# manhofer/Line3Dpp

Measured on AMD Instinct MI355X. Metric: M segment-pair scores/sec, higher is better.
Workload: dtype f64

## Files before the change

### include/l3dpp_hip.h

```cpp
#ifndef L3DPP_HIP_H_
#define L3DPP_HIP_H_

#include <stdint.h>

#ifdef __cplusplus
extern "C" {
#endif


typedef struct l3d_match {
    uint32_t src_camID_, src_segID_, tgt_camID_, tgt_segID_;
    float overlap_score_, score3D_;
    float depth_p1_, depth_p2_, depth_q1_, depth_q2_;
} l3d_match;

typedef struct l3d_segment2d { uint32_t camID_, segID_; } l3d_segment2d;

typedef struct l3d_segment3d {
    double P1[3], P2[3], dir[3];
    float length_;
    uint32_t valid_;
} l3d_segment3d;

typedef struct l3d_cledge { int32_t i_, j_; float w_; } l3d_cledge;

typedef struct l3d_float4 { float x, y, z, w; } l3d_float4;

typedef struct l3d_slot {
    uint32_t tgt_seg;
    float overlap;
    float depth_p1, depth_p2, depth_q1, depth_q2;
    float score3D;
    uint32_t flags;
} l3d_slot;

typedef enum l3d_status {
    L3D_OK = 0,
    L3D_ERR_ARG = -1,
    L3D_ERR_IMAGE_SMALL = -2,
    L3D_ERR_ID_IN_USE = -3,
    L3D_ERR_NO_NEIGHBORS = -4,
    L3D_ERR_NO_SEGMENTS = -5,
    L3D_ERR_NO_VIEWS = -6,
    L3D_ERR_STATE = -7,
    L3D_ERR_HIP = -8,
    L3D_ERR_LIMIT = -9,
    L3D_ERR_RETRY = -10,
    L3D_ERR_IO = -11
} l3d_status;

typedef struct l3d_ctx l3d_ctx;

typedef struct l3d_match_params {
    float sigma_position;
    float sigma_angle;
    uint32_t num_neighbors;
    float epipolar_overlap;
    int32_t kNN;
    float const_regularization_depth;
} l3d_match_params;

const char* l3d_last_error(void);
const char* l3d_build_info(void);
uint64_t l3d_trim_cache(void);


l3d_ctx* l3d_create(int device, void* stream);
void l3d_destroy(l3d_ctx*);

int l3d_add_view(l3d_ctx*, uint32_t camID, const float* segs4, uint32_t M, const double K[9],
                 const double R[9], const double t[3], uint32_t width, uint32_t height,
                 float median_depth, const uint32_t* neighbors, uint32_t n_neighbors);

int l3d_add_view_worldpoints(l3d_ctx*, uint32_t camID, const float* segs4, uint32_t M, const double K[9],
                             const double R[9], const double t[3], uint32_t width, uint32_t height,
                             float median_depth, const uint32_t* worldpoints, uint32_t n_worldpoints);
int l3d_get_visual_neighbors(l3d_ctx*, uint32_t camID, uint32_t* out, uint32_t cap, uint32_t* n);
int l3d_neighbors_from_worldpoints(uint32_t n_views, const uint32_t* cam_ids, const double* K9, const double* R9,
                                   const double* t3, const uint64_t* wp_offsets, const uint32_t* worldpoints,
                                   uint32_t num_neighbors, uint64_t* nb_offsets, uint32_t* neighbors, uint64_t cap);

typedef struct l3d_nvm l3d_nvm;
typedef struct l3d_nvm_camera {
    const char* filename;
    float focal, distortion;
    float median_depth;
    uint32_t n_worldpoints;
    double R[9], t[3], C[3];
} l3d_nvm_camera;
int l3d_nvm_open(const char* path, l3d_nvm** out);
uint32_t l3d_nvm_num_cameras(const l3d_nvm*);
int l3d_nvm_get_camera(const l3d_nvm*, uint32_t index, l3d_nvm_camera* out);
int l3d_nvm_get_worldpoints(const l3d_nvm*, uint32_t index, uint32_t* out, uint32_t cap);
void l3d_nvm_close(l3d_nvm*);
void l3d_nvm_intrinsics(float focal, uint32_t width, uint32_t height, double K[9]);
typedef struct l3d_sfm l3d_sfm;
typedef struct l3d_sfm_image {
    uint32_t id, camera;
    uint32_t width, height;
    const char* name;
    float focal;
    float median_depth;
    uint32_t n_worldpoints;
    double K[9];
    double R[9], t[3], C[3];
    double radial[3], tangential[2];
} l3d_sfm_image;
int l3d_sfm_open_colmap(const char* folder, l3d_sfm** out);
int l3d_sfm_open_bundler(const char* bundle_file, l3d_sfm** out);
uint32_t l3d_sfm_num_images(const l3d_sfm*);
int l3d_sfm_get_image(const l3d_sfm*, uint32_t index, l3d_sfm_image* out);
int l3d_sfm_get_worldpoints(const l3d_sfm*, uint32_t index, uint32_t* out, uint32_t cap);
void l3d_sfm_close(l3d_sfm*);
struct l3d_camera_model;
int l3d_sfm_get_camera_model(const l3d_sfm*, uint32_t index, struct l3d_camera_model* out);
const char* l3d_sfm_get_camera_params(const l3d_sfm*, uint32_t index, double* params, uint32_t cap, uint32_t* n);
int l3d_segment_cache_name(uint32_t camID, uint32_t width, uint32_t height, uint32_t max_segments, char* out, uint32_t cap);
int l3d_read_segment_cache(const char* path, float* segs4 , uint32_t cap, uint32_t* n);
int l3d_write_segment_cache(const char* path, const float* segs4, uint32_t n);

typedef struct l3d_image {
    const uint8_t* data;
    uint32_t cols, rows, channels, row_stride;
} l3d_image;
typedef struct l3d_detect_options {
    const char* output_folder;
    int32_t load_segments;
    int32_t max_image_width;
    uint32_t max_line_segments;
} l3d_detect_options;
typedef struct l3d_detect_stats {
    uint32_t width, height;
    uint32_t raw_segments;
    uint32_t segments;
    uint32_t from_cache;
    uint32_t seeds;
    uint32_t nfa_evals;
    uint32_t reserved;
    double max_grad;
} l3d_detect_stats;
int l3d_detect_segments(l3d_ctx*, uint32_t n_images, const l3d_image* images, int max_image_width,
                        uint32_t max_segments, uint32_t* counts);
int l3d_detect_view_segments(l3d_ctx*, uint32_t n_images, const uint32_t* camIDs, const l3d_image* images,
                             const l3d_detect_options* opts, uint32_t* counts);
int l3d_get_detected_segments(l3d_ctx*, float* segs4 , uint64_t cap, uint64_t* n);
int l3d_get_detect_stats(l3d_ctx*, l3d_detect_stats* out, uint32_t cap, uint32_t* n);
int l3d_add_view_image(l3d_ctx*, uint32_t camID, const l3d_image* image, const l3d_detect_options* opts,
                       const double K[9], const double R[9], const double t[3], float median_depth,
                       const uint32_t* neighbors, uint32_t n_neighbors, uint32_t* n_segments);
int l3d_add_view_image_worldpoints(l3d_ctx*, uint32_t camID, const l3d_image* image, const l3d_detect_options* opts,
                                   const double K[9], const double R[9], const double t[3], float median_depth,
                                   const uint32_t* worldpoints, uint32_t n_worldpoints, uint32_t* n_segments);

typedef struct l3d_distortion { double K[9]; double radial[3]; double tangential[2]; } l3d_distortion;
int l3d_undistort_images(l3d_ctx*, uint32_t n_images, const l3d_image* in, const l3d_distortion* dist,
                         uint8_t* const* out);
enum { L3D_CAM_NONE = 0, L3D_CAM_FULL_OPENCV = 1, L3D_CAM_OPENCV_FISHEYE = 2, L3D_CAM_SIMPLE_RADIAL_FISHEYE = 3,
       L3D_CAM_RADIAL_FISHEYE = 4, L3D_CAM_FOV = 5 };
typedef struct l3d_camera_model {
    uint32_t model;
    uint32_t reserved;
    double K[9];
    double params[8];
    double K_new[9];
} l3d_camera_model;
int l3d_undistort_images_model(l3d_ctx*, uint32_t n_images, const l3d_image* in, const l3d_camera_model* cams,
                               uint8_t* const* out);

int l3d_match_images(l3d_ctx*, const l3d_match_params*);

int l3d_match_begin(l3d_ctx*, const l3d_match_params*);
int l3d_num_pairs(l3d_ctx*, uint32_t* n);
int l3d_get_pairs(l3d_ctx*, uint32_t* src_cam, uint32_t* tgt_cam, uint64_t* slot_offset );
int l3d_match_pairs(l3d_ctx*, uint32_t first, uint32_t count);
int l3d_slot_buffer(l3d_ctx*, void** dev_ptr, uint64_t* n_slots);
int l3d_get_fresh_hyp(l3d_ctx*, float* out, uint64_t n);
int l3d_slots_exchanged(l3d_ctx*);
int l3d_slot_index_buffer(l3d_ctx*, void** dev_ptr, uint64_t* n_slots);
int l3d_pack_slot_indices(l3d_ctx*, uint32_t first, uint32_t count);
int l3d_expand_slot_indices(l3d_ctx*, uint32_t first, uint32_t count);
int l3d_match_finish(l3d_ctx*);
int l3d_lists_shard(l3d_ctx*, uint32_t rank, uint32_t world, void* slab_ptr[4], uint64_t slab_bytes[4], void* full_ptr[4]);
int l3d_lists_shard_views(l3d_ctx*, uint32_t rank, uint32_t world, uint32_t view0, uint32_t view1, void* slab_ptr[4],
                          uint64_t slab_bytes[4], void* full_ptr[4]);
int l3d_tail_shard_count(l3d_ctx*, uint32_t counts[2]);
int l3d_shard_options(l3d_ctx*, uint32_t first_needed_rank, int exchanges_stream_ordered);
int l3d_tail_shard_layout(l3d_ctx*, uint32_t world, const uint32_t* counts_all, const uint32_t* view_bounds, void* base_ptr[9],
                          uint64_t elt_bytes[9], uint64_t* first, uint64_t* count);
int l3d_tail_shard_commit(l3d_ctx*);
int l3d_affinity_shard_begin(l3d_ctx*, uint32_t rank, uint32_t world, void** simv, uint64_t* first, uint64_t* count);
int l3d_affinity_shard_finish(l3d_ctx*);
int l3d_affinity_shard_abort(l3d_ctx*);
int l3d_plan_shards(uint32_t n_views, uint32_t n_pairs, const uint32_t* pair_src_view, const uint64_t* pair_cost,
                    uint32_t world, uint32_t* view_bounds, uint32_t* pair_bounds);
int l3d_match_abort(l3d_ctx*);

int l3d_compute_affinity(l3d_ctx*);

int l3d_reconstruct_3d_lines(l3d_ctx*, uint32_t visibility_t, int perform_diffusion, float collinearity_t,
                             int use_CERES, uint32_t max_iter_CERES);
int l3d_num_3d_lines(l3d_ctx*, uint32_t* n_lines, uint32_t* n_segments, uint32_t* n_residuals);
typedef struct l3d_line_opt_summary {
    uint32_t lines_bundled;
    uint32_t lines_constant;
    uint32_t lines_dropped;
    uint32_t stop_gradient, stop_function, stop_parameter, stop_max_iter;
    uint32_t stop_other;
    uint32_t max_iterations;
    uint32_t residuals;
    uint32_t lines_wide;
    uint32_t max_residuals;
    double cost_before, cost_after;
    float kernel_ms;
    uint32_t reserved;
} l3d_line_opt_summary;
int l3d_line_opt_stats(l3d_ctx*, l3d_line_opt_summary* out);
int l3d_get_3d_lines(l3d_ctx*, uint32_t* seg_offsets, l3d_segment3d* segments, uint32_t* res_offsets,
                     l3d_segment2d* residuals, l3d_segment3d* cluster_lines, uint32_t* reference_views);

int l3d_synchronize(l3d_ctx*);


int l3d_pair_tests(l3d_ctx*, uint64_t* n);
int l3d_get_matches(l3d_ctx*, uint32_t camID, l3d_match* out, uint64_t cap, uint32_t* seg_offsets,
                    uint64_t* n);
int l3d_get_pair_slots(l3d_ctx*, uint32_t pair_index, l3d_slot* out, uint64_t cap, uint32_t* Ms,
                       uint32_t* K);
int l3d_num_best(l3d_ctx*, uint32_t* n);
int l3d_get_best(l3d_ctx*, l3d_segment2d* seg2d, l3d_segment3d* seg3d, l3d_match* best);
int l3d_view_info(l3d_ctx*, uint32_t camID, float* k, float* median_depth);
int l3d_translation(l3d_ctx*, double t[3]);
int l3d_num_affinity(l3d_ctx*, uint32_t* n_edges, uint32_t* n_rows);
int l3d_get_affinity(l3d_ctx*, l3d_cledge* edges, l3d_segment2d* local2global, float* med_scene_depth_lines);
int l3d_get_sparse_matrix(l3d_ctx*, int sort_by_row, l3d_float4* entries, int32_t* start_indices);

int l3d_principal_direction(const double S9[9], double dir3[3]);
int l3d_line_to_cayley(const double P1[3], const double P2[3], double x[4]);
int l3d_cayley_to_segment(const double x[4], const double P1_old[3], const double P2_old[3], double P1[3], double P2[3]);
int l3d_line_opt_eval(int device, uint32_t n, const double x[4], const double* obs, const double* cams, double* cost,
                      double* residuals, double* jacobians, int32_t* ok);

int l3d_triangulate_points(int device, uint32_t n_cameras, const double* P12, uint64_t n_points, const uint64_t* obs_offsets,
                           const uint32_t* obs_camera, const double* obs_xy, double* X3, uint8_t* valid);
int l3d_rotation_from_rpy(double roll, double pitch, double yaw, double R9[9]);
int l3d_rotation_from_q(double qw, double qx, double qy, double qz, double R9[9]);
int l3d_decompose_projection_matrix(const double P12[12], double K9[9], double R9[9], double t3[3]);

int l3d_selftest_arith(int device, uint64_t n, uint64_t seed, uint64_t counts[3]);

int l3d_selftest_scan(int device, uint32_t element_bytes, const void* in, uint32_t n_in, uint32_t n_calls, const uint32_t* n,
                      int in_place, int pass_total, void* out, void* totals, uint64_t* ws_nonzero, uint64_t* guard_changed);

int l3d_set_brute_force(l3d_ctx*, int on);

typedef struct l3d_timings {
    float begin_ms;
    float match_pairs_ms;
    float finish_ms;
    float affinity_ms;
    uint32_t match_kernel_launches;
    float match_kernel_ms;
    float cull_prepare_ms;
    uint32_t culled_pairs;
    uint32_t list_entries;
    uint32_t support_words;
    uint32_t tied_rows;
    uint32_t chain_sweeps;
    uint32_t chain_extra_rounds;
    uint32_t pool_retries;
    float lists_ms;
    uint32_t record_kbytes;
    uint32_t list_inverse;
    uint32_t list_candidates;
    uint32_t list_headers;
    uint32_t slots_lo, slots_hi;
} l3d_timings;
int l3d_get_timings(l3d_ctx*, l3d_timings*);
int l3d_set_timing_level(l3d_ctx*, int level);
unsigned long long l3d_debug_counter(const char* name);


int l3d_match_lines(int device, const float* lines_src4, uint32_t Ms, const float* lines_tgt4, uint32_t Mt,
                    const double F[9], const double RtKinv_src[9], const double RtKinv_tgt[9],
                    const double C_src[3], const double C_tgt[3], uint32_t width, uint32_t height,
                    float epi_overlap, int32_t kNN, l3d_slot* out_slots, uint64_t* num_matches);

int l3d_output_filename(l3d_ctx*, int max_image_width, char* buf, uint32_t cap);
int l3d_save_3d_lines_txt(l3d_ctx*, const char* output_folder, int max_image_width);
int l3d_save_3d_lines_bin(l3d_ctx*, const char* output_folder, int max_image_width);
int l3d_get_segment_coords2d(l3d_ctx*, uint32_t camID, uint32_t segID, float coords[4]);
int l3d_save_result_stl(l3d_ctx*, const char* output_folder, int max_image_width);
int l3d_save_result_obj(l3d_ctx*, const char* output_folder, int max_image_width);

int l3d_score_matches(int device, const float* lines4, uint32_t M, const float* matches4, const int32_t* ranges2,
                      const float* reg_tgt2, uint32_t n, const double RtKinv[9], const double C[3], float two_sigA_sqr,
                      float k, float* scores);

int l3d_find_collinear_segments(int device, const float* lines4, uint32_t M, float dist_t, uint32_t* offsets,
                                uint32_t* idx, uint64_t cap, uint64_t* n);

int l3d_diffuse_affinity(int device, const l3d_cledge* edges, uint32_t n_edges, uint32_t n_rows, uint32_t iterations,
                         l3d_cledge* out);

typedef struct l3d_camera {
    double K[9], R[9], t[3];
    uint32_t width, height;
} l3d_camera;
typedef struct l3d_projected_segment {
    float x1, y1, x2, y2;
    float inv_depth1, inv_depth2;
    uint32_t line;
    uint32_t segment;
} l3d_projected_segment;
#define L3D_PROJ_CLIPPED_NEAR 0x80000000u
#define L3D_PROJ_CLIPPED_RECT 0x40000000u
#define L3D_PROJ_SEGMENT_MASK 0x3FFFFFFFu
int l3d_project_segments(int device, uint32_t n_cams, const l3d_camera* cams, uint32_t n_segments,
                         const l3d_segment3d* segments, const uint32_t* line_of_segment, double near_plane,
                         uint32_t* counts, l3d_projected_segment* out, uint64_t cap, uint64_t* n);
int l3d_render_line_maps(int device, uint32_t n_cams, const l3d_camera* cams, const uint32_t* n_records_per_cam,
                         const l3d_projected_segment* records, uint32_t thickness, int32_t* const* line_id_planes,
                         float* const* inv_depth_planes);
int l3d_draw_line_maps(int device, uint32_t n_cams, const l3d_image* images, const int32_t* const* line_id_planes,
                       uint32_t n_lines, const uint8_t* colors, uint32_t alpha, uint8_t* const* out_rgb);
int l3d_view_camera(l3d_ctx*, uint32_t camID, l3d_camera* cam);
int l3d_project_lines(l3d_ctx*, uint32_t n_cams, const l3d_camera* cams, double near_plane, uint32_t* counts);
int l3d_get_projected_lines(l3d_ctx*, l3d_projected_segment* out, uint64_t cap, uint64_t* n);
int l3d_render_lines(l3d_ctx*, uint32_t n_cams, const l3d_camera* cams, double near_plane, uint32_t thickness,
                     int32_t* const* line_id_planes, float* const* inv_depth_planes);
int l3d_draw_lines(l3d_ctx*, uint32_t n_cams, const l3d_camera* cams, const l3d_image* images, double near_plane,
                   uint32_t thickness, uint32_t alpha, const uint8_t* colors, uint8_t* const* out_rgb);
int l3d_set_projection_budget(l3d_ctx*, uint64_t bytes);

#ifdef __cplusplus
}
#endif
#endif
```

### line3dpp_amd/_lib.py

```python
import ctypes as C
import os

import numpy as np

_HERE = os.path.dirname(os.path.abspath(__file__))
SO_PATH = os.path.join(_HERE, "csrc", "libl3dpp_hip.so")
SO_PATH = os.environ.get("L3D_LIB", SO_PATH)

MATCH_DTYPE = np.dtype([
    ("src_cam", "<u4"), ("src_seg", "<u4"), ("tgt_cam", "<u4"), ("tgt_seg", "<u4"),
    ("overlap", "<f4"), ("score3D", "<f4"),
    ("d_p1", "<f4"), ("d_p2", "<f4"), ("d_q1", "<f4"), ("d_q2", "<f4")])
SEGMENT2D_DTYPE = np.dtype([("cam", "<u4"), ("seg", "<u4")])
SEGMENT3D_DTYPE = np.dtype([("P1", "<f8", 3), ("P2", "<f8", 3), ("dir", "<f8", 3), ("length", "<f4"), ("valid", "<u4")])
CLEDGE_DTYPE = np.dtype([("i", "<i4"), ("j", "<i4"), ("w", "<f4")])
SLOT_DTYPE = np.dtype([
    ("tgt_seg", "<u4"), ("overlap", "<f4"), ("d_p1", "<f4"), ("d_p2", "<f4"), ("d_q1", "<f4"), ("d_q2", "<f4"),
    ("score3D", "<f4"), ("flags", "<u4")])
FLOAT4_DTYPE = np.dtype([("x", "<f4"), ("y", "<f4"), ("z", "<f4"), ("w", "<f4")])
PROJECTED_SEGMENT_DTYPE = np.dtype([("x1", "<f4"), ("y1", "<f4"), ("x2", "<f4"), ("y2", "<f4"), ("inv_depth1", "<f4"),
                                    ("inv_depth2", "<f4"), ("line", "<u4"), ("segment", "<u4")])
PROJ_CLIPPED_NEAR, PROJ_CLIPPED_RECT, PROJ_SEGMENT_MASK = 0x80000000, 0x40000000, 0x3FFFFFFF
assert MATCH_DTYPE.itemsize == 40 and SLOT_DTYPE.itemsize == 32 and SEGMENT3D_DTYPE.itemsize == 80
assert PROJECTED_SEGMENT_DTYPE.itemsize == 32
EMPTY = 0xFFFFFFFF
L3D_ERR_NO_SEGMENTS = -5
L3D_ERR_IO = -11


class MatchParams(C.Structure):
    _fields_ = [("sigma_position", C.c_float), ("sigma_angle", C.c_float), ("num_neighbors", C.c_uint32),
                ("epipolar_overlap", C.c_float), ("kNN", C.c_int32), ("const_regularization_depth", C.c_float)]


class NvmCamera(C.Structure):
    _fields_ = [("filename", C.c_char_p), ("focal", C.c_float), ("distortion", C.c_float), ("median_depth", C.c_float),
                ("n_worldpoints", C.c_uint32), ("R", C.c_double * 9), ("t", C.c_double * 3), ("C", C.c_double * 3)]


class SfmImage(C.Structure):
    _fields_ = [("id", C.c_uint32), ("camera", C.c_uint32), ("width", C.c_uint32), ("height", C.c_uint32),
                ("name", C.c_char_p), ("focal", C.c_float), ("median_depth", C.c_float), ("n_worldpoints", C.c_uint32),
                ("K", C.c_double * 9), ("R", C.c_double * 9), ("t", C.c_double * 3), ("C", C.c_double * 3),
                ("radial", C.c_double * 3), ("tangential", C.c_double * 2)]


class Timings(C.Structure):
    _fields_ = [("begin_ms", C.c_float), ("match_pairs_ms", C.c_float), ("finish_ms", C.c_float),
                ("affinity_ms", C.c_float), ("match_kernel_launches", C.c_uint32), ("match_kernel_ms", C.c_float),
                ("cull_prepare_ms", C.c_float), ("culled_pairs", C.c_uint32),
                ("list_entries", C.c_uint32), ("support_words", C.c_uint32), ("tied_rows", C.c_uint32), ("chain_sweeps", C.c_uint32),
                ("chain_extra_rounds", C.c_uint32), ("pool_retries", C.c_uint32),
                ("lists_ms", C.c_float), ("record_kbytes", C.c_uint32),
                ("list_inverse", C.c_uint32), ("list_candidates", C.c_uint32), ("list_headers", C.c_uint32),
                ("slots_lo", C.c_uint32), ("slots_hi", C.c_uint32)]


class LineOptStats(C.Structure):
    _fields_ = [("lines_bundled", C.c_uint32), ("lines_constant", C.c_uint32), ("lines_dropped", C.c_uint32),
                ("stop_gradient", C.c_uint32), ("stop_function", C.c_uint32), ("stop_parameter", C.c_uint32),
                ("stop_max_iter", C.c_uint32), ("stop_other", C.c_uint32), ("max_iterations", C.c_uint32),
                ("residuals", C.c_uint32), ("lines_wide", C.c_uint32), ("max_residuals", C.c_uint32),
                ("cost_before", C.c_double), ("cost_after", C.c_double), ("kernel_ms", C.c_float), ("reserved", C.c_uint32)]


class Image(C.Structure):
    _fields_ = [("data", C.c_void_p), ("cols", C.c_uint32), ("rows", C.c_uint32), ("channels", C.c_uint32),
                ("row_stride", C.c_uint32)]


class DetectOptions(C.Structure):
    _fields_ = [("output_folder", C.c_char_p), ("load_segments", C.c_int32), ("max_image_width", C.c_int32),
                ("max_line_segments", C.c_uint32)]


class Distortion(C.Structure):
    _fields_ = [("K", C.c_double * 9), ("radial", C.c_double * 3), ("tangential", C.c_double * 2)]


CAMERA_MODELS = {"FULL_OPENCV": 1, "OPENCV_FISHEYE": 2, "SIMPLE_RADIAL_FISHEYE": 3, "RADIAL_FISHEYE": 4, "FOV": 5}
CAMERA_MODEL_PARAMS = {"FULL_OPENCV": 8, "OPENCV_FISHEYE": 4, "SIMPLE_RADIAL_FISHEYE": 1, "RADIAL_FISHEYE": 2, "FOV": 1}


class CameraModel(C.Structure):
    _fields_ = [("model", C.c_uint32), ("reserved", C.c_uint32), ("K", C.c_double * 9), ("params", C.c_double * 8),
                ("K_new", C.c_double * 9)]


class Camera(C.Structure):
    _fields_ = [("K", C.c_double * 9), ("R", C.c_double * 9), ("t", C.c_double * 3), ("width", C.c_uint32),
                ("height", C.c_uint32)]


class ProjectedSegment(C.Structure):
    _fields_ = [("x1", C.c_float), ("y1", C.c_float), ("x2", C.c_float), ("y2", C.c_float), ("inv_depth1", C.c_float),
                ("inv_depth2", C.c_float), ("line", C.c_uint32), ("segment", C.c_uint32)]


class DetectStats(C.Structure):
    _fields_ = [("width", C.c_uint32), ("height", C.c_uint32), ("raw_segments", C.c_uint32), ("segments", C.c_uint32),
                ("from_cache", C.c_uint32), ("seeds", C.c_uint32), ("nfa_evals", C.c_uint32), ("reserved", C.c_uint32),
                ("max_grad", C.c_double)]


EXPORTS = [
    "l3d_last_error", "l3d_build_info", "l3d_create", "l3d_destroy", "l3d_add_view", "l3d_match_images",
    "l3d_match_begin", "l3d_num_pairs", "l3d_get_pairs", "l3d_match_pairs", "l3d_slot_buffer", "l3d_match_finish",
    "l3d_compute_affinity", "l3d_synchronize", "l3d_pair_tests", "l3d_get_matches", "l3d_get_pair_slots",
    "l3d_num_best", "l3d_get_best", "l3d_view_info", "l3d_translation", "l3d_num_affinity", "l3d_get_affinity",
    "l3d_get_sparse_matrix", "l3d_get_timings", "l3d_match_lines", "l3d_set_brute_force", "l3d_slots_exchanged",
    "l3d_reconstruct_3d_lines", "l3d_num_3d_lines", "l3d_get_3d_lines", "l3d_diffuse_affinity",
    "l3d_output_filename", "l3d_save_3d_lines_txt", "l3d_save_result_stl", "l3d_save_result_obj",
    "l3d_get_segment_coords2d", "l3d_find_collinear_segments", "l3d_score_matches",
    "l3d_slot_index_buffer", "l3d_pack_slot_indices", "l3d_expand_slot_indices", "l3d_match_abort", "l3d_save_3d_lines_bin", "l3d_lists_shard",
    "l3d_principal_direction", "l3d_selftest_arith", "l3d_lists_shard_views", "l3d_plan_shards",
    "l3d_add_view_worldpoints", "l3d_get_visual_neighbors", "l3d_neighbors_from_worldpoints",
    "l3d_nvm_open", "l3d_nvm_num_cameras", "l3d_nvm_get_camera", "l3d_nvm_get_worldpoints", "l3d_nvm_close",
    "l3d_nvm_intrinsics", "l3d_segment_cache_name", "l3d_read_segment_cache", "l3d_write_segment_cache",
    "l3d_trim_cache", "l3d_set_timing_level", "l3d_tail_shard_count", "l3d_tail_shard_layout", "l3d_tail_shard_commit",
    "l3d_sfm_open_colmap", "l3d_sfm_open_bundler", "l3d_sfm_num_images", "l3d_sfm_get_image", "l3d_sfm_get_worldpoints",
    "l3d_sfm_close", "l3d_debug_counter", "l3d_affinity_shard_begin", "l3d_affinity_shard_finish", "l3d_affinity_shard_abort", "l3d_shard_options",
    "l3d_line_opt_stats", "l3d_line_to_cayley", "l3d_cayley_to_segment", "l3d_line_opt_eval", "l3d_get_fresh_hyp",
    "l3d_detect_segments", "l3d_detect_view_segments", "l3d_get_detected_segments", "l3d_get_detect_stats",
    "l3d_add_view_image", "l3d_add_view_image_worldpoints", "l3d_undistort_images",
    "l3d_undistort_images_model", "l3d_sfm_get_camera_model", "l3d_sfm_get_camera_params",
    "l3d_triangulate_points", "l3d_rotation_from_rpy", "l3d_rotation_from_q", "l3d_decompose_projection_matrix",
    "l3d_project_segments", "l3d_render_line_maps", "l3d_draw_line_maps", "l3d_view_camera", "l3d_project_lines",
    "l3d_get_projected_lines", "l3d_render_lines", "l3d_draw_lines", "l3d_set_projection_budget", "l3d_selftest_scan",
]

_lib = None


def load():
    global _lib
    if _lib is not None:
        return _lib
    if not os.path.exists(SO_PATH):
        raise RuntimeError(
            f"{SO_PATH} is missing: the HIP extension has not been built (run `make -C line3dpp_amd/csrc` or "
            "`python -c 'import __graft_entry__ as g; g.build()'`). There is no CPU fallback.")
    L = C.CDLL(SO_PATH)
    vp, u32, u64, i32, f32 = C.c_void_p, C.c_uint32, C.c_uint64, C.c_int, C.c_float
    L.l3d_last_error.restype = C.c_char_p
    L.l3d_build_info.restype = C.c_char_p
    L.l3d_trim_cache.argtypes = []; L.l3d_trim_cache.restype = u64
    L.l3d_create.argtypes = [i32, vp]; L.l3d_create.restype = vp
    L.l3d_destroy.argtypes = [vp]; L.l3d_destroy.restype = None
    L.l3d_add_view.argtypes = [vp, u32, vp, u32, vp, vp, vp, u32, u32, f32, vp, u32]
    L.l3d_add_view_worldpoints.argtypes = [vp, u32, vp, u32, vp, vp, vp, u32, u32, f32, vp, u32]
    L.l3d_get_visual_neighbors.argtypes = [vp, u32, vp, u32, vp]
    L.l3d_neighbors_from_worldpoints.argtypes = [u32, vp, vp, vp, vp, vp, vp, u32, vp, vp, u64]
    L.l3d_sfm_open_colmap.argtypes = [C.c_char_p, vp]; L.l3d_sfm_open_bundler.argtypes = [C.c_char_p, vp]
    L.l3d_sfm_num_images.argtypes = [vp]; L.l3d_sfm_num_images.restype = u32
    L.l3d_sfm_get_image.argtypes = [vp, u32, vp]; L.l3d_sfm_get_worldpoints.argtypes = [vp, u32, vp, u32]
    L.l3d_sfm_close.argtypes = [vp]; L.l3d_sfm_close.restype = None
    L.l3d_nvm_open.argtypes = [C.c_char_p, vp]
    L.l3d_nvm_num_cameras.argtypes = [vp]; L.l3d_nvm_num_cameras.restype = u32
    L.l3d_nvm_get_camera.argtypes = [vp, u32, vp]
    L.l3d_nvm_get_worldpoints.argtypes = [vp, u32, vp, u32]
    L.l3d_nvm_close.argtypes = [vp]; L.l3d_nvm_close.restype = None
    L.l3d_nvm_intrinsics.argtypes = [f32, u32, u32, vp]; L.l3d_nvm_intrinsics.restype = None
    L.l3d_segment_cache_name.argtypes = [u32, u32, u32, u32, C.c_char_p, u32]
    L.l3d_read_segment_cache.argtypes = [C.c_char_p, vp, u32, vp]
    L.l3d_write_segment_cache.argtypes = [C.c_char_p, vp, u32]
    L.l3d_match_images.argtypes = [vp, C.POINTER(MatchParams)]
    L.l3d_match_begin.argtypes = [vp, C.POINTER(MatchParams)]
    L.l3d_num_pairs.argtypes = [vp, C.POINTER(u32)]
    L.l3d_get_pairs.argtypes = [vp, vp, vp, vp]
    L.l3d_match_pairs.argtypes = [vp, u32, u32]
    L.l3d_slot_buffer.argtypes = [vp, C.POINTER(vp), C.POINTER(u64)]
    L.l3d_get_fresh_hyp.argtypes = [vp, vp, u64]
    L.l3d_match_finish.argtypes = [vp]
    L.l3d_match_abort.argtypes = [vp]
    L.l3d_lists_shard.argtypes = [vp, u32, u32, vp, vp, vp]
    L.l3d_lists_shard_views.argtypes = [vp, u32, u32, u32, u32, vp, vp, vp]
    L.l3d_plan_shards.argtypes = [u32, u32, vp, vp, u32, vp, vp]
    L.l3d_compute_affinity.argtypes = [vp]
    L.l3d_synchronize.argtypes = [vp]
    L.l3d_pair_tests.argtypes = [vp, C.POINTER(u64)]
    L.l3d_get_matches.argtypes = [vp, u32, vp, u64, vp, C.POINTER(u64)]
    L.l3d_get_pair_slots.argtypes = [vp, u32, vp, u64, C.POINTER(u32), C.POINTER(u32)]
    L.l3d_num_best.argtypes = [vp, C.POINTER(u32)]
    L.l3d_get_best.argtypes = [vp, vp, vp, vp]
    L.l3d_view_info.argtypes = [vp, u32, C.POINTER(f32), C.POINTER(f32)]
    L.l3d_translation.argtypes = [vp, vp]
    L.l3d_num_affinity.argtypes = [vp, C.POINTER(u32), C.POINTER(u32)]
    L.l3d_get_affinity.argtypes = [vp, vp, vp, C.POINTER(f32)]
    L.l3d_get_sparse_matrix.argtypes = [vp, i32, vp, vp]
    L.l3d_get_timings.argtypes = [vp, C.POINTER(Timings)]
    L.l3d_set_timing_level.argtypes = [vp, C.c_int]
    L.l3d_debug_counter.argtypes = [C.c_char_p]
    L.l3d_debug_counter.restype = C.c_ulonglong
    L.l3d_tail_shard_count.argtypes = [vp, vp]
    L.l3d_tail_shard_layout.argtypes = [vp, u32, vp, vp, vp, vp, vp, vp]
    L.l3d_tail_shard_commit.argtypes = [vp]
    L.l3d_affinity_shard_begin.argtypes = [vp, u32, u32, vp, vp, vp]
    L.l3d_affinity_shard_finish.argtypes = [vp]
    L.l3d_affinity_shard_abort.argtypes = [vp]
    L.l3d_shard_options.argtypes = [vp, C.c_uint32, C.c_int]
    L.l3d_match_lines.argtypes = [i32, vp, u32, vp, u32, vp, vp, vp, vp, vp, u32, u32, f32, C.c_int32, vp,
                                  C.POINTER(u64)]
    L.l3d_set_brute_force.argtypes = [vp, i32]
    L.l3d_slots_exchanged.argtypes = [vp]
    L.l3d_slot_index_buffer.argtypes = [vp, C.POINTER(vp), C.POINTER(u64)]
    L.l3d_pack_slot_indices.argtypes = [vp, u32, u32]
    L.l3d_expand_slot_indices.argtypes = [vp, u32, u32]
    L.l3d_reconstruct_3d_lines.argtypes = [vp, u32, i32, f32, i32, u32]
    L.l3d_num_3d_lines.argtypes = [vp, C.POINTER(u32), C.POINTER(u32), C.POINTER(u32)]
    L.l3d_get_3d_lines.argtypes = [vp, vp, vp, vp, vp, vp, vp]
    L.l3d_diffuse_affinity.argtypes = [i32, vp, u32, u32, u32, vp]
    L.l3d_output_filename.argtypes = [vp, i32, C.c_char_p, u32]
    L.l3d_save_3d_lines_txt.argtypes = [vp, C.c_char_p, i32]
    L.l3d_save_result_stl.argtypes = [vp, C.c_char_p, i32]
    L.l3d_save_3d_lines_bin.argtypes = [vp, C.c_char_p, i32]
    L.l3d_save_result_obj.argtypes = [vp, C.c_char_p, i32]
    L.l3d_get_segment_coords2d.argtypes = [vp, u32, u32, vp]
    L.l3d_find_collinear_segments.argtypes = [i32, vp, u32, f32, vp, vp, u64, vp]
    L.l3d_principal_direction.argtypes = [vp, vp]
    L.l3d_line_opt_stats.argtypes = [vp, C.POINTER(LineOptStats)]
    L.l3d_line_to_cayley.argtypes = [vp, vp, vp]
    L.l3d_cayley_to_segment.argtypes = [vp, vp, vp, vp, vp]
    L.l3d_line_opt_eval.argtypes = [i32, u32, vp, vp, vp, vp, vp, vp, vp]
    L.l3d_selftest_arith.argtypes = [i32, u64, u64, vp]
    L.l3d_selftest_scan.argtypes = [i32, u32, vp, u32, u32, vp, i32, i32, vp, vp, C.POINTER(u64), C.POINTER(u64)]
    L.l3d_detect_segments.argtypes = [vp, u32, vp, i32, u32, vp]
    L.l3d_detect_view_segments.argtypes = [vp, u32, vp, vp, C.POINTER(DetectOptions), vp]
    L.l3d_get_detected_segments.argtypes = [vp, vp, u64, C.POINTER(u64)]
    L.l3d_get_detect_stats.argtypes = [vp, vp, u32, C.POINTER(u32)]
    L.l3d_add_view_image.argtypes = [vp, u32, C.POINTER(Image), C.POINTER(DetectOptions), vp, vp, vp, f32, vp, u32,
                                     C.POINTER(u32)]
    L.l3d_add_view_image_worldpoints.argtypes = [vp, u32, C.POINTER(Image), C.POINTER(DetectOptions), vp, vp, vp, f32,
                                                 vp, u32, C.POINTER(u32)]
    L.l3d_undistort_images.argtypes = [vp, u32, vp, vp, vp]
    L.l3d_undistort_images_model.argtypes = [vp, u32, vp, vp, vp]
    L.l3d_sfm_get_camera_model.argtypes = [vp, u32, vp]
    L.l3d_sfm_get_camera_params.argtypes = [vp, u32, vp, u32, vp]; L.l3d_sfm_get_camera_params.restype = C.c_char_p
    L.l3d_score_matches.argtypes = [i32, vp, u32, vp, vp, vp, u32, vp, vp, f32, f32, vp]
    L.l3d_triangulate_points.argtypes = [i32, u32, vp, u64, vp, vp, vp, vp, vp]
    f64 = C.c_double
    L.l3d_rotation_from_rpy.argtypes = [f64, f64, f64, vp]
    L.l3d_rotation_from_q.argtypes = [f64, f64, f64, f64, vp]
    L.l3d_decompose_projection_matrix.argtypes = [vp, vp, vp, vp]
    L.l3d_project_segments.argtypes = [i32, u32, vp, u32, vp, vp, f64, vp, vp, u64, C.POINTER(u64)]
    L.l3d_render_line_maps.argtypes = [i32, u32, vp, vp, vp, u32, vp, vp]
    L.l3d_draw_line_maps.argtypes = [i32, u32, vp, vp, u32, vp, u32, vp]
    L.l3d_view_camera.argtypes = [vp, u32, C.POINTER(Camera)]
    L.l3d_project_lines.argtypes = [vp, u32, vp, f64, vp]
    L.l3d_get_projected_lines.argtypes = [vp, vp, u64, C.POINTER(u64)]
    L.l3d_render_lines.argtypes = [vp, u32, vp, f64, u32, vp, vp]
    L.l3d_draw_lines.argtypes = [vp, u32, vp, vp, f64, u32, u32, vp, vp]
    L.l3d_set_projection_budget.argtypes = [vp, u64]
    for name in EXPORTS:
        fn = getattr(L, name)
        if fn.restype is C.c_int and name not in ("l3d_last_error", "l3d_build_info", "l3d_create", "l3d_destroy"):
            fn.restype = C.c_int
    _lib = L
    return L


def last_error():
    return load().l3d_last_error().decode()


def ptr(a):
    return a.ctypes.data_as(C.c_void_p) if a is not None else None
```

### line3dpp_amd/csrc/k_lists.hip

```cpp
#include <algorithm>
#include <cstdlib>
#include <type_traits>

#include "l3d_dev.h"
#include "l3d_kernels.h"
#include "l3d_lists.h"

constexpr uint32_t kLists4Grid = 512;

namespace l3d {

namespace {

#define L3D_LDS __attribute__((address_space(3)))

__device__ __forceinline__ uint32_t lane_id() { return threadIdx.x & 63u; }

template <int WPL>
__device__ __forceinline__ void group_barrier() {
    if (WPL == 1) {
        __builtin_amdgcn_fence(__ATOMIC_RELEASE, "wavefront");
        __builtin_amdgcn_wave_barrier();
        __builtin_amdgcn_fence(__ATOMIC_ACQUIRE, "wavefront");
    } else {
// ... 448 lines not shown
    const PairCsr pcs = pair_csr[pi];
    if (pcs.base == kEmpty) return;
    const PairDesc& pd = pairs[pi];
    if (pd.tgt < tgt_v0 || pd.tgt >= tgt_v1) return;
    const uint32_t Mt = pd.Mt, tid = threadIdx.x;
    if ((Mt <= lds_segs) != LDSCNT) return;
    const uint32_t S = row_start ? row_start[pd.row_off + pd.Ms] - row_start[pd.row_off] : pd.Ms * pd.K;
    if (!S) {
        for (uint32_t t = threadIdx.x; t <= pd.Mt; t += kCsrBlock) poff[pcs.base + pcs.q + (size_t)t * pcs.ni] = 0;
        return;
    }
    typedef typename std::conditional<TGT16, uint16_t, uint32_t>::type tgt_t;
    const tgt_t* __restrict__ it = (const tgt_t*)inv_tgt + pd.slot_off;
    uint32_t* __restrict__ offq = poff + pcs.base + pcs.q;
    const uint32_t ni = pcs.ni;
    L3D_LDS uint32_t* lcur = (L3D_LDS uint32_t*)smem;
    uint32_t* gdum = dummy + (size_t)blockIdx.x * 64;
    auto gcur = [&](uint32_t t) -> uint32_t* { return t < Mt ? offq + (size_t)(t + 1) * ni : gdum + (t - Mt); };
    auto cur_get = [&](uint32_t t) -> uint32_t { return LDSCNT ? lcur[t] : *gcur(t); };
    auto cur_set = [&](uint32_t t, uint32_t v) { if (LDSCNT) lcur[t] = v; else *gcur(t) = v; };
    for (uint32_t t = tid; t < Mt + 64; t += kCsrBlock) cur_set(t, 0u);
    __threadfence_block();
    __syncthreads();
    const uint32_t dum = Mt + (tid & 63u);
    for (uint32_t i0 = 0; i0 < S; i0 += kCsrChunk * kCsrBlock) {
        uint32_t tv[kCsrChunk];
#pragma unroll
        for (uint32_t k = 0; k < kCsrChunk; ++k) { const uint32_t i = i0 + k * kCsrBlock + tid; tv[k] = it[min(i, S - 1)]; tv[k] = (i < S && tv[k] < Mt) ? tv[k] : dum; }
#pragma unroll
        for (uint32_t k = 0; k < kCsrChunk; ++k) {
            if (LDSCNT) (void)__hip_atomic_fetch_add(&lcur[tv[k]], 1u, __ATOMIC_RELAXED, __HIP_MEMORY_SCOPE_WORKGROUP);
            else atomicAdd(gcur(tv[k]), 1u);
        }
    }
    __threadfence_block();
    __syncthreads();
    const uint32_t per = (Mt + kCsrBlock - 1) / kCsrBlock;
    const uint32_t t0 = min(tid * per, Mt), t1 = min(t0 + per, Mt);
    uint32_t sum = 0;
    for (uint32_t t = t0; t < t1; ++t) sum += cur_get(t);
    part[tid] = sum;
    __syncthreads();
    for (uint32_t d = 1; d < kCsrBlock; d <<= 1) {
        const uint32_t v = tid >= d ? part[tid - d] : 0u;
        __syncthreads();
        part[tid] += v;
        __syncthreads();
    }
    uint32_t run = part[tid] - sum;
    for (uint32_t t = t0; t < t1; ++t) { const uint32_t c = cur_get(t); cur_set(t, run); run += c; }
    if (tid == 0) offq[0] = 0;
    __threadfence_block();
    __syncthreads();
    uint32_t* __restrict__ out = refs + pd.slot_off;
    if (STAGED) {
        L3D_LDS uint32_t* stage = lcur + (lds_segs_round(Mt) + 64);
        const uint32_t total = part[kCsrBlock - 1];
        const uint32_t window = stage_cap - min(stage_cap / 8, 1024u);
        uint32_t t_lo = 0, base = 0;
        while (base < total) {
            uint32_t lo = t_lo + 1, hi = Mt;
            while (lo < hi) { const uint32_t mid = (lo + hi) >> 1; if (lcur[mid] < base + window) lo = mid + 1; else hi = mid; }
            const uint32_t t_hi = lo, end = t_hi < Mt ? lcur[t_hi] : total;
            __syncthreads();
            for (uint32_t i0 = 0; i0 < S; i0 += kCsrChunk * kCsrBlock) {
                uint32_t tv[kCsrChunk], at[kCsrChunk];
#pragma unroll
                for (uint32_t k = 0; k < kCsrChunk; ++k) { const uint32_t i = i0 + k * kCsrBlock + tid; tv[k] = it[min(i, S - 1)]; tv[k] = (i < S && tv[k] >= t_lo && tv[k] < t_hi) ? tv[k] : kEmpty; }
#pragma unroll
                for (uint32_t k = 0; k < kCsrChunk; ++k)
                    at[k] = tv[k] != kEmpty ? __hip_atomic_fetch_add(&lcur[tv[k]], 1u, __ATOMIC_RELAXED, __HIP_MEMORY_SCOPE_WORKGROUP) : 0u;
#pragma unroll
                for (uint32_t k = 0; k < kCsrChunk; ++k) {
                    if (tv[k] == kEmpty) continue;
                    const uint32_t i = i0 + k * kCsrBlock + tid, x = at[k] - base;
                    if (x < stage_cap) stage[x] = i;
                    else out[at[k]] = (uint32_t)pd.slot_off + i;
                }
            }
            __threadfence_block();
            __syncthreads();
            const uint32_t n_here = min(end - base, stage_cap);
            for (uint32_t x = tid; x < n_here; x += kCsrBlock) out[base + x] = (uint32_t)pd.slot_off + stage[x];
            __syncthreads();
            t_lo = t_hi; base = end;
        }
        for (uint32_t t = tid; t < Mt; t += kCsrBlock) *gcur(t) = lcur[t];
        return;
    }
    for (uint32_t i0 = 0; i0 < S; i0 += kCsrChunk * kCsrBlock) {
        uint32_t tv[kCsrChunk], at[kCsrChunk];
#pragma unroll
        for (uint32_t k = 0; k < kCsrChunk; ++k) { const uint32_t i = i0 + k * kCsrBlock + tid; tv[k] = it[min(i, S - 1)]; tv[k] = (i < S && tv[k] < Mt) ? tv[k] : dum; }
#pragma unroll
        for (uint32_t k = 0; k < kCsrChunk; ++k)
            at[k] = LDSCNT ? __hip_atomic_fetch_add(&lcur[tv[k]], 1u, __ATOMIC_RELAXED, __HIP_MEMORY_SCOPE_WORKGROUP)
                           : atomicAdd(gcur(tv[k]), 1u);
#pragma unroll
        for (uint32_t k = 0; k < kCsrChunk; ++k)
            if (tv[k] < Mt) out[at[k]] = (uint32_t)pd.slot_off + i0 + k * kCsrBlock + tid;
    }
    if (LDSCNT) {
        __syncthreads();
        for (uint32_t t = tid; t < Mt; t += kCsrBlock) *gcur(t) = lcur[t];
    }
}

template <int WPL, int BASE>
__global__ __launch_bounds__(64 * WPL) void k_lists(const ViewDev* __restrict__ views, const PairDesc* __restrict__ pairs,
                                               const ListView* __restrict__ lviews, const OutPair* __restrict__ opairs,
                                               const InPair* __restrict__ ipairs, const uint32_t* __restrict__ gseg_view,
                                               const uint32_t* __restrict__ poff,
                                               const uint32_t* __restrict__ inv, const float2* __restrict__ hyp_p,
                                               const float2* __restrict__ hyp_q, uint32_t uniform_K, const ListPools lp, uint32_t view0) {
    extern __shared__ __attribute__((aligned(16))) char smem[];
    if (WPL == 1) {
        const uint32_t vi = view0 + blockIdx.y, seg = blockIdx.x;
        if (seg >= lviews[vi].M) return;
        const uint32_t pool = lp.pool0 + ((blockIdx.y * gridDim.x + blockIdx.x) >> 2) % lp.npools;
        const uint32_t L = process_list<1, BASE>(vi, seg, pool, (L3D_LDS char*)smem, views, pairs, lviews, opairs,
                                                 ipairs, poff, inv, hyp_p, hyp_q, uniform_K, lp);
        if (L && lane_id() == 0) {
            const uint32_t g = lviews[vi].seg_base + seg;
            if (L > 65535u) atomicOr(&lp.flags[1], 1u);
            else if (L > ListCfg<4, BASE>::CAP) lp.listH[atomicAdd(&lp.flags[5], 1u)] = g;
            else if (L > ListCfg<2, BASE>::CAP) lp.list4[atomicAdd(&lp.flags[4], 1u)] = g;
            else lp.list2[atomicAdd(&lp.flags[7], 1u)] = g;
        }
    } else {
        const uint32_t n = WPL == 2 ? lp.flags[7] : lp.flags[4];
        const uint32_t* list = WPL == 2 ? lp.list2 : lp.list4;
        for (uint32_t idx = blockIdx.x; idx < n; idx += gridDim.x) {
            const uint32_t g = list[idx];
            const uint32_t vi = gseg_view[g];
            (void)process_list<WPL, BASE>(vi, g - lviews[vi].seg_base, lp.pool0 + blockIdx.x % lp.npools, (L3D_LDS char*)smem, views, pairs,
                                          lviews, opairs, ipairs, poff, inv, hyp_p, hyp_q, uniform_K, lp);
            __syncthreads();
        }
    }
}

struct HugeScratch {
    float* d1; float* d2; uint32_t* tv; uint32_t* ref; uint32_t* pf; uint64_t* key;
    uint32_t cap;
};
__global__ __launch_bounds__(256) void k_lists_huge(const ViewDev* __restrict__ views, const PairDesc* __restrict__ pairs,
                                                    const ListView* __restrict__ lviews,
                                                    const OutPair* __restrict__ opairs, const InPair* __restrict__ ipairs,
                                                    const uint32_t* __restrict__ gseg_view,
                                                    const uint32_t* __restrict__ poff,
                                                    const uint32_t* __restrict__ inv, const float2* __restrict__ hyp_p,
                                                    const float2* __restrict__ hyp_q, const ListPools lp, const HugeScratch hs) {
    __shared__ uint32_t red[16];
    __shared__ uint32_t s_base;
    constexpr uint32_t kRows = 256;
    __shared__ uint32_t s_row[4 * kRows];
    const uint32_t t = threadIdx.x;
    const uint32_t nH = lp.flags[5];
    for (uint32_t idx = blockIdx.x; idx < nH; idx += gridDim.x) {
        const uint32_t g = lp.listH[idx];
        const uint32_t vi = gseg_view[g];
        const ListView lv = lviews[vi];
        const uint32_t seg = g - lv.seg_base;
        const ViewDev& v = views[vi];
        uint32_t mine_n = 0;
        for (uint32_t q = t; q < lv.ni; q += 256)
            mine_n += poff[lv.pbase + (seg + 1) * lv.ni + q] - poff[lv.pbase + seg * lv.ni + q];
        uint32_t n_inv;
        (void)group_scan<4>(mine_n, n_inv, red);
        mine_n = 0;
        for (uint32_t q = lv.q0; q < lv.q0 + lv.nq; ++q) {
            const OutPair op = opairs[q];
            uint64_t row0; uint32_t Kr;
            out_row_slots(op, seg, lp, row0, Kr);
            for (uint32_t j = t; j < Kr; j += 256) {
                const float2 s = hyp_p[row0 + j];
                mine_n += s.x == s.x ? 1u : 0u;
            }
        }
        uint32_t n_fresh;
        (void)group_scan<4>(mine_n, n_fresh, red);
        const uint32_t L = n_inv + n_fresh;
        __syncthreads();
        if (t == 0) {
            s_base = atomicAdd(&lp.flags[6], L);
            atomicAdd(&lp.cnt[(lp.pool0 + blockIdx.x % lp.npools) * 16 + 5], L); atomicAdd(&lp.cnt[(lp.pool0 + blockIdx.x % lp.npools) * 16 + 6], n_inv);
        }
        __syncthreads();
        const uint32_t base = s_base;
        if ((uint64_t)base + L > hs.cap) { if (t == 0) atomicOr(&lp.flags[2], 1u); continue; }
        float* e_d1 = hs.d1 + base; float* e_d2 = hs.d2 + base;
        uint32_t* e_tv = hs.tv + base; uint32_t* e_ref = hs.ref + base; uint32_t* e_pf = hs.pf + base;
        uint64_t* keys = hs.key + base;
        uint32_t pos = 0;
        for (uint32_t qb = 0; qb < lv.ni; qb += kRows) {
            const uint32_t q = qb + t, nq_here = min(kRows, lv.ni - qb);
            uint32_t c = 0, a = 0;
            if (q < lv.ni) {
                const uint32_t e0 = poff[lv.pbase + seg * lv.ni + q], e1 = poff[lv.pbase + (seg + 1) * lv.ni + q];
                const InPair ip = ipairs[lv.i0 + q];
                a = ip.rec_base + e0; c = e1 - e0;
                s_row[4 * t + 2] = ip.src; s_row[4 * t + 3] = ip.pair;
            }
            uint32_t total;
            const uint32_t ex = group_scan<4>(c, total, red);
            if (q < lv.ni) { s_row[4 * t] = a; s_row[4 * t + 1] = ex; }
            __syncthreads();
            for (uint32_t x = t; x < total; x += 256) {
                uint32_t lo = 0, hi = nq_here;
                while (hi - lo > 1) { const uint32_t mid = (lo + hi) / 2; if (s_row[4 * mid + 1] <= x) lo = mid; else hi = mid; }
                const uint32_t* rowp = inv + s_row[4 * lo];
                const uint32_t r0 = s_row[4 * lo + 1], r1 = lo + 1 < nq_here ? s_row[4 * lo + 5] : total;
                const uint32_t ref = rowp[x - r0];
                uint32_t rank = r0;
                for (uint32_t y = 0; y < r1 - r0; ++y) rank += rowp[y] < ref ? 1u : 0u;
                const float2 dq = hyp_q[ref];
                const uint32_t at = pos + rank;
                e_d1[at] = dq.x; e_d2[at] = dq.y; e_tv[at] = s_row[4 * lo + 2]; e_ref[at] = ref; e_pf[at] = s_row[4 * lo + 3] | kHypInv;
            }
            pos += total;
            __syncthreads();
        }
        for (uint32_t q = lv.q0; q < lv.q0 + lv.nq; ++q) {
            const OutPair op = opairs[q];
            uint64_t row0; uint32_t Kr;
            out_row_slots(op, seg, lp, row0, Kr);
            for (uint32_t j0 = 0; j0 < Kr; j0 += 256) {
                bool alive = false;
                float2 s = make_float2(0.0f, 0.0f);
                if (j0 + t < Kr) { s = hyp_p[row0 + j0 + t]; alive = s.x == s.x; }
                uint32_t total;
                const uint32_t at = pos + group_scan<4>(alive ? 1u : 0u, total, red);
                if (alive && at < L) { e_d1[at] = s.x; e_d2[at] = s.y; e_tv[at] = op.tgt; e_ref[at] = (uint32_t)(row0 + j0 + t); e_pf[at] = op.pair; }
                pos += total;
            }
        }
        __threadfence_block();
        __syncthreads();
        if (pos != L) { if (t == 0) atomicOr(&lp.flags[3], 1u); continue; }
        auto for_candidates = [&](uint32_t i, auto&& emit) {
            const float a1 = e_d1[i], a2 = e_d2[i];
            const uint32_t tvi = e_tv[i];
            const float kt = views[tvi].k, D = pairs[e_pf[i] & 0x7FFFFFFFu].cc_dist;
            const float R1 = window_sq(a1, v.k, kt, D), R2 = window_sq(a2, v.k, kt, D);
            for (uint32_t j = 0; j < L; ++j) {
                if (j == i || e_tv[j] == tvi) continue;
                const float d1 = a1 - e_d1[j], d2 = a2 - e_d2[j];
                if ((d1 * d1 <= R1) && (d2 * d2 <= R2)) emit(j);
            }
        };
        uint32_t mine = 0;
        for (uint32_t i = t; i < L; i += 256) {
            uint32_t c = 0;
            for_candidates(i, [&](uint32_t) { ++c; });
            keys[i] = c;
            mine += c;
        }
        uint32_t H;
        (void)group_scan<4>(mine, H, red);
        __threadfence_block();
        __syncthreads();
        if (H == 0) continue;
        const uint32_t pool = lp.pool0 + blockIdx.x % lp.npools;
        if (t == 0) {
            red[8] = atomicAdd(&lp.cnt[pool * 16 + 3], H);
            red[9] = atomicAdd(&lp.cnt[pool * 16 + 4], 1u);
        }
        __syncthreads();
        const uint32_t cb = red[8], hb = red[9];
        if (cb + H > lp.ccap || hb + 1 > lp.scap) { if (t == 0) atomicOr(&lp.flags[0], 1u); continue; }
        const uint32_t c0 = pool * lp.ccap + cb;
        for (uint32_t i = t; i < L; i += 256) {
            if (!keys[i]) continue;
            uint32_t w = c0;
            for (uint32_t y = 0; y < i; ++y) w += (uint32_t)keys[y];
            for_candidates(i, [&](uint32_t j) {
                CandRec r;
                r.ij = (i << 16) | j; r.ref_i = e_ref[i]; r.ref_j = e_ref[j]; r.pf_i = e_pf[i];
                r.tvj = e_tv[j] | (e_pf[j] & kHypInv);
                r.a1 = e_d1[i]; r.a2 = e_d2[i]; r.b1 = e_d1[j]; r.b2 = e_d2[j]; r.sim = __uint_as_float(g);
                lp.cands[w++] = r;
            });
        }
        if (t == 0) lp.chdrs[pool * lp.scap + hb] = CandHdr{g, c0, H, 0u};
    }
}

__global__ __launch_bounds__(256) __attribute__((amdgpu_waves_per_eu(4))) void k_cand_exact(
        const ViewDev* __restrict__ views, const PairDesc* __restrict__ pairs, const uint32_t* __restrict__ gseg_view,
        const SimConst sc, const ListPools lp) {
    if (lp.flags[0] | lp.flags[2]) return;
    const uint32_t pool = lp.pool0 + blockIdx.y, x = blockIdx.x * 256 + threadIdx.x;
    if (x >= min(lp.cnt[pool * 16 + 3], lp.ccap)) return;
    CandRec* cr = lp.cands + (size_t)pool * lp.ccap + x;
    const CandRec r = *cr;
    const uint32_t g = __float_as_uint(r.sim);
    const PairDesc& pd = pairs[r.pf_i & 0x7FFFFFFFu];
    const uint32_t tvi = (r.pf_i & kHypInv) ? pd.src : pd.tgt;
    float sim = -1.0f;
    const bool ok = exact_support(views[gseg_view[g]], views, views[0].segx[g], r.a1, r.a2, tvi, r.b1, r.b2, sc, sim);
    cr->sim = ok ? sim : -1.0f;
}

constexpr uint32_t kEdgeLds = 512;
__device__ __forceinline__ void edges_of_segment(const PairDesc* __restrict__ pairs, const Slot* __restrict__ slots,
                                                 const ListPools& lp, uint32_t* __restrict__ seg_of_g, const CandHdr ch,
                                                 uint32_t opool, L3D_LDS uint32_t* s_ij_w, L3D_LDS float* s_sim_w,
                                                 uint32_t lane) {
    const uint32_t g = ch.g, n = ch.cnt;
    CandRec* cand = lp.cands + ch.begin;
    const uint64_t lt_mask = (1ull << lane) - 1ull;
    const bool in_lds = n <= kEdgeLds;
    uint32_t n_acc = 0;
    for (uint32_t x0 = 0; x0 < n; x0 += 64) {
        const uint32_t x = x0 + lane;
        bool ok = false;
        if (x < n) {
            const float sim = cand[x].sim;
            ok = sim >= 0.0f;
            if (in_lds) { s_ij_w[x] = cand[x].ij; s_sim_w[x] = sim; }
        }
        n_acc += (uint32_t)__popcll(__builtin_amdgcn_ballot_w64(ok));
    }
    if (n_acc == 0) return;
    if (in_lds) {
        __builtin_amdgcn_fence(__ATOMIC_RELEASE, "workgroup");
        __builtin_amdgcn_wave_barrier();
        __builtin_amdgcn_fence(__ATOMIC_ACQUIRE, "workgroup");
    }
    auto ij_of = [&](uint32_t y) -> uint32_t { return in_lds ? s_ij_w[y] : cand[y].ij; };
    auto sim_of = [&](uint32_t y) -> float { return in_lds ? s_sim_w[y] : cand[y].sim; };
    auto in_run = [&](uint32_t x, uint32_t& rank, uint32_t& earlier, uint32_t& mine) {
        const uint32_t ij = ij_of(x), i = ij >> 16;
        rank = 0; earlier = 0; mine = 1;
        for (uint32_t y = x; y-- > 0;) {
            const uint32_t o = ij_of(y);
            if ((o >> 16) != i) break;
            if (sim_of(y) >= 0.0f) { ++earlier; ++mine; rank += o < ij ? 1u : 0u; }
        }
        for (uint32_t y = x + 1; y < n; ++y) {
            const uint32_t o = ij_of(y);
            if ((o >> 16) != i) break;
            if (sim_of(y) >= 0.0f) { ++mine; rank += o < ij ? 1u : 0u; }
        }
    };
    uint32_t n_h = 0;
    for (uint32_t x0 = 0; x0 < n; x0 += 64) {
        const uint32_t x = x0 + lane;
        bool first = false;
        if (x < n && sim_of(x) >= 0.0f) {
            const uint32_t i = ij_of(x) >> 16;
            first = true;
            for (uint32_t y = x; y-- > 0;) {
                if ((ij_of(y) >> 16) != i) break;
                if (sim_of(y) >= 0.0f) { first = false; break; }
            }
        }
        n_h += (uint32_t)__popcll(__builtin_amdgcn_ballot_w64(first));
    }
    uint32_t eb = 0, hb = 0, sb = 0;
    if (lane == 0) {
        eb = atomicAdd(&lp.cnt[opool * 16 + 0], n_acc);
        hb = atomicAdd(&lp.cnt[opool * 16 + 1], n_h);
        sb = atomicAdd(&lp.cnt[opool * 16 + 2], 1u);
    }
    eb = __shfl(eb, 0); hb = __shfl(hb, 0); sb = __shfl(sb, 0);
    if (eb + n_acc > lp.ecap || hb + n_h > lp.hcap || sb + 1 > lp.scap) {
        if (lane == 0) atomicOr(&lp.flags[0], 1u);
        return;
    }
    const uint32_t e0 = opool * lp.ecap + eb, h0 = opool * lp.hcap + hb;
    uint32_t acc_before = 0, first_before = 0;
    for (uint32_t x0 = 0; x0 < n; x0 += 64) {
        const uint32_t x = x0 + lane;
        bool acc = false, first = false;
        uint32_t rank = 0, earlier = 0, mine = 0;
        float sim = -1.0f;
        if (x < n) {
            sim = sim_of(x);
            acc = sim >= 0.0f;
            if (acc) { in_run(x, rank, earlier, mine); first = earlier == 0; }
        }
        const uint64_t ma = __builtin_amdgcn_ballot_w64(acc), mf = __builtin_amdgcn_ballot_w64(first);
        if (acc) {
            const CandRec r = cand[x];
            const uint32_t run0 = acc_before + (uint32_t)__popcll(ma & lt_mask) - earlier;
            EdgeRec e;
            e.ref_j = r.ref_j; e.sim = sim;
            e.j_cam = (r.ij & 0xFFFFu) | ((r.tvj & kHypInv) ? kEdgeInv : 0u);
            e.tv_j = r.tvj & 0x7FFFFFFFu;
            lp.edges[e0 + run0 + rank] = e;
            if (first) {
                HypHdr hdr;
                hdr.g = g; hdr.ref = r.ref_i; hdr.pair_flags = r.pf_i; hdr.canon = r.ij >> 16;
                hdr.dp1 = r.a1; hdr.dp2 = r.a2;
                hdr.edge_begin = e0 + run0; hdr.edge_cnt = mine; hdr.score3D = 0.0f; hdr.state = 0;
                {
                    const Slot hs = slots[r.ref_i];
                    const bool hinv = (r.pf_i & kHypInv) != 0;
                    const PairDesc& hp = pairs[r.pf_i & 0x7FFFFFFFu];
                    hdr.tgt_seg = !hinv ? hs.tgt_seg : lp.slot_row ? lp.slot_row[r.ref_i] : (uint32_t)((r.ref_i - hp.slot_off) / hp.K);
                    hdr.overlap = hs.overlap;
                    hdr.oq1 = hinv ? hs.dp1 : hs.dq1; hdr.oq2 = hinv ? hs.dp2 : hs.dq2;
                }
                hdr.pad[0] = hdr.pad[1] = 0;
                lp.hyps[h0 + first_before + (uint32_t)__popcll(mf & lt_mask)] = hdr;
            }
        }
        acc_before += (uint32_t)__popcll(ma); first_before += (uint32_t)__popcll(mf);
    }
    if (lane == 0) {
        const uint32_t si = opool * lp.scap + sb;
        lp.segs[si] = SegHdr{g, h0, n_h, 0u};
        seg_of_g[g] = si;
    }
}

constexpr uint32_t kEdgesSplit = 4;
__global__ __launch_bounds__(64) void k_edges(const ViewDev* __restrict__ views, const PairDesc* __restrict__ pairs,
                                               const uint32_t* __restrict__ gseg_view, const Slot* __restrict__ slots,
                                               const ListPools lp, uint32_t* __restrict__ seg_of_g) {
    const uint32_t pool = lp.pool0 + blockIdx.y, lane = lane_id();
    if (lp.flags[0] | lp.flags[2]) return;
    __shared__ uint32_t s_ij[kEdgeLds];
    __shared__ float s_sim[kEdgeLds];
    const uint32_t n_hdr = min(lp.cnt[pool * 16 + 4], lp.scap);
    for (uint32_t k = blockIdx.x; k < n_hdr; k += gridDim.x) {
        const uint32_t opool = lp.pool0 + (k + 61u * blockIdx.y) % lp.npools;
        edges_of_segment(pairs, slots, lp, seg_of_g, lp.chdrs[pool * lp.scap + k], opool, (L3D_LDS uint32_t*)s_ij, (L3D_LDS float*)s_sim, lane);
        __builtin_amdgcn_fence(__ATOMIC_RELEASE, "workgroup");
        __builtin_amdgcn_wave_barrier();
    }
}

__global__ void k_chain_sweep(const ListPools lp, uint8_t* __restrict__ positive, uint32_t* __restrict__ changed,
                              uint32_t* __restrict__ undecided) {
    if (lp.flags[0] | lp.flags[2]) return;
    const uint32_t pool = lp.pool0 + blockIdx.y, k = blockIdx.x * blockDim.x + threadIdx.x;
    bool later = false;
    if (k < min(lp.cnt[pool * 16 + 1], lp.hcap)) {
        const HypHdr& h = lp.hyps[pool * lp.hcap + k];
        if (!(h.pair_flags & kHypInv) && !__hip_atomic_load(&positive[h.ref], __ATOMIC_RELAXED, __HIP_MEMORY_SCOPE_AGENT)) {
            const uint32_t n = h.edge_cnt, e0 = h.edge_begin;
            bool done = false, any_inverse = false;
            for (uint32_t e = 0; e < n && !done; ++e) {
                const EdgeRec& ed = lp.edges[e0 + e];
                const bool inv = (ed.j_cam & kEdgeInv) != 0;
                any_inverse |= inv;
                if (!inv || __hip_atomic_load(&positive[ed.ref_j], __ATOMIC_RELAXED, __HIP_MEMORY_SCOPE_AGENT)) {
                    __hip_atomic_store(&positive[h.ref], (uint8_t)1, __ATOMIC_RELAXED, __HIP_MEMORY_SCOPE_AGENT);
                    changed[0] = 1;
                    done = true;
                }
            }
            later = !done && any_inverse;
        }
    }
    const uint64_t m = __builtin_amdgcn_ballot_w64(later);
    if (m) {
        uint32_t base = 0;
        if ((threadIdx.x & 63u) == (uint32_t)__builtin_ctzll(m)) base = atomicAdd(&lp.cnt[pool * 16 + 7], (uint32_t)__popcll(m));
        base = __shfl(base, __builtin_ctzll(m));
        if (later) undecided[pool * lp.hcap + base + (uint32_t)__popcll(m & ((1ull << (threadIdx.x & 63u)) - 1ull))] = pool * lp.hcap + k;
    }
}
constexpr uint32_t kChainListBlocks = 4;
__global__ void k_chain_sweep_list(const ListPools lp, uint8_t* __restrict__ positive, uint32_t* __restrict__ changed,
                                   uint32_t sweep, const uint32_t* __restrict__ undecided) {
    if (lp.flags[0] | lp.flags[2]) return;
    if (!changed[sweep - 1]) return;
    const uint32_t pool = lp.pool0 + blockIdx.y;
    const uint32_t n_u = min(lp.cnt[pool * 16 + 7], lp.hcap);
    for (uint32_t idx = blockIdx.x * blockDim.x + threadIdx.x; idx < n_u; idx += gridDim.x * blockDim.x) {
        const HypHdr& h = lp.hyps[undecided[pool * lp.hcap + idx]];
        if (__hip_atomic_load(&positive[h.ref], __ATOMIC_RELAXED, __HIP_MEMORY_SCOPE_AGENT)) continue;
        const uint32_t n = h.edge_cnt, e0 = h.edge_begin;
        for (uint32_t e = 0; e < n; ++e) {
            const EdgeRec& ed = lp.edges[e0 + e];
            if ((ed.j_cam & kEdgeInv) && __hip_atomic_load(&positive[ed.ref_j], __ATOMIC_RELAXED, __HIP_MEMORY_SCOPE_AGENT)) {
                __hip_atomic_store(&positive[h.ref], (uint8_t)1, __ATOMIC_RELAXED, __HIP_MEMORY_SCOPE_AGENT);
                changed[sweep] = 1;
                break;
            }
        }
    }
}

constexpr uint32_t kMaxReplicas = 16;
__global__ void k_hyp_scores(const ListPools lp, const uint8_t* __restrict__ positive,
                             const uint32_t* __restrict__ gseg_view, Slot* __restrict__ slots,
                             const uint8_t* __restrict__ pair_present, uint32_t* __restrict__ max_score_bits) {
    const uint32_t pool = lp.pool0 + blockIdx.y, k = blockIdx.x * blockDim.x + threadIdx.x;
    const bool active = !(lp.flags[0] | lp.flags[2]) && k < min(lp.cnt[pool * 16 + 1], lp.hcap);
    float score3D = 0.0f;
    uint32_t view = kEmpty;
    if (active) {
        HypHdr& h = lp.hyps[pool * lp.hcap + k];
        const bool inv = (h.pair_flags & kHypInv) != 0;
        const bool exists = !inv || positive[h.ref] != 0;
        float cur = 0.0f;
        uint32_t cur_cam = kEmpty;
        if (exists) {
            const uint32_t n = h.edge_cnt, e0 = h.edge_begin;
            for (uint32_t e = 0; e < n; e += 4) {
                EdgeRec ed[4]; bool ok[4];
#pragma unroll
                for (uint32_t i = 0; i < 4; ++i) ed[i] = lp.edges[e0 + min(e + i, n - 1)];
#pragma unroll
                for (uint32_t i = 0; i < 4; ++i) ok[i] = e + i < n && (!(ed[i].j_cam & kEdgeInv) || positive[ed[i].ref_j] != 0);
#pragma unroll
                for (uint32_t i = 0; i < 4; ++i) {
                    if (!ok[i]) continue;
                    if (ed[i].tv_j == cur_cam) {
                        if (ed[i].sim > cur) { score3D -= cur; score3D += ed[i].sim; cur = ed[i].sim; }
                    } else {
                        score3D += ed[i].sim; cur = ed[i].sim; cur_cam = ed[i].tv_j;
                    }
                }
            }
        }
        h.score3D = score3D;
        h.state = exists ? kHypExists : 0u;
        if (exists && !inv && (!pair_present || pair_present[h.pair_flags & 0x7FFFFFFFu])) slots[h.ref].score3D = score3D;
        view = gseg_view[h.g];
    }
    uint64_t todo = __builtin_amdgcn_ballot_w64(score3D > 0.0f);
    while (todo) {
        const uint32_t leader = (uint32_t)__builtin_ctzll(todo);
        const uint32_t lv = __builtin_amdgcn_readlane(view, leader);
        const bool mine = score3D > 0.0f && view == lv;
        float mx = mine ? score3D : 0.0f;
#pragma unroll
        for (int d = 32; d > 0; d >>= 1) mx = fmaxf(mx, __shfl_xor(mx, d));
        if (lane_id() == leader) {
            uint32_t* p = &max_score_bits[lv * kMaxReplicas + (pool & (kMaxReplicas - 1))];
            if (__float_as_uint(mx) > *(volatile uint32_t*)p) atomicMax(p, __float_as_uint(mx));
        }
        todo &= ~__builtin_amdgcn_ballot_w64(mine);
    }
}

__global__ void k_hyp_filter(const ListPools lp, const uint32_t* __restrict__ gseg_view,
                             const uint32_t* __restrict__ max_score_bits, uint32_t* __restrict__ kept_cnt,
                             unsigned long long* __restrict__ best_pack) {
    const uint32_t pool = lp.pool0 + blockIdx.y, k = blockIdx.x * blockDim.x + threadIdx.x;
    if ((lp.flags[0] | lp.flags[2]) || k >= min(lp.cnt[pool * 16 + 1], lp.hcap)) return;
    HypHdr& h = lp.hyps[pool * lp.hcap + k];
    uint32_t mx = 0;
    {
        const uint32_t* p = max_score_bits + (size_t)gseg_view[h.g] * kMaxReplicas;
#pragma unroll
        for (uint32_t r = 0; r < kMaxReplicas; ++r) mx = max(mx, p[r]);
    }
    const float lim = kMinBestScorePerc * __uint_as_float(mx);
    const float s = h.score3D;
    if ((h.state & kHypExists) && s > 0.0f && s > lim) {
        h.state |= kHypKeep;
        atomicAdd(&kept_cnt[h.g], 1u);
        atomicMax(&best_pack[h.g], ((unsigned long long)__float_as_uint(s) << 32) | (0xFFFFFFFFu - h.canon));
    }
}

__global__ void k_seg_filter(uint32_t g0, uint32_t g1, const uint32_t* __restrict__ kept_cnt,
                             const unsigned long long* __restrict__ best_pack, unsigned long long* __restrict__ cnt64) {
    const uint32_t g = g0 + blockIdx.x * blockDim.x + threadIdx.x;
    if (g >= g1) return;
    const bool ok = __uint_as_float((uint32_t)(best_pack[g] >> 32)) > kMinBestScore3D;
    cnt64[g] = ok ? ((1ull << 32) | kept_cnt[g]) : 0ull;
}

__device__ __forceinline__ void make_match(const ViewDev* views, const PairDesc* pairs, uint32_t view, uint32_t seg,
                                           const HypHdr& h, Match& m, uint32_t& tgt_view, uint32_t& tgt_seg) {
    const bool inv = (h.pair_flags & kHypInv) != 0;
    const PairDesc& pd = pairs[h.pair_flags & 0x7FFFFFFFu];
    tgt_view = inv ? pd.src : pd.tgt;
    tgt_seg = h.tgt_seg;
    m.src_cam = views[view].cam; m.src_seg = seg;
    m.tgt_cam = views[tgt_view].cam; m.tgt_seg = tgt_seg;
    m.overlap = h.overlap; m.score3D = h.score3D;
    m.dp1 = h.dp1; m.dp2 = h.dp2;
    m.dq1 = h.oq1; m.dq2 = h.oq2;
}

__global__ void k_seg_write(uint32_t g0, uint32_t g1, unsigned long long base64, const ViewDev* __restrict__ views, const PairDesc* __restrict__ pairs,
                            const uint32_t* __restrict__ seg_base, const uint32_t* __restrict__ gseg_view,
                            const unsigned long long* __restrict__ off64s, const unsigned long long* __restrict__ best_pack,
                            const uint32_t* __restrict__ seg_of_g, const ListPools lp, const Slot* __restrict__ slots,
                            uint32_t* __restrict__ surv_off, uint32_t* __restrict__ hyp_off, Match* __restrict__ surv,
                            uint32_t* __restrict__ surv_tg, uint32_t* __restrict__ surv_sg,
                            int32_t* __restrict__ hyp_of_seg, HypRec* __restrict__ hyps, float* __restrict__ depths) {
    const uint32_t t = blockIdx.x * blockDim.x + threadIdx.x;
    const bool pass_ok = !(lp.flags[0] | lp.flags[2]);
    if (t <= g1 - g0) {
        const uint32_t gs = g0 + t;
        const unsigned long long o = off64s[gs] + base64;
        surv_off[gs] = (uint32_t)o; hyp_off[gs] = (uint32_t)(o >> 32);
        if (gs < g1) hyp_of_seg[gs] = ((off64s[gs + 1] >> 32) != (off64s[gs] >> 32) && pass_ok) ? (int32_t)(uint32_t)(o >> 32) : -1;
    }
    if (!pass_ok) return;
    const uint32_t pq = t / lp.hcap, k = t - pq * lp.hcap, pool = lp.pool0 + pq;
    if (pq >= lp.npools || k >= min(lp.cnt[pool * 16 + 1], lp.hcap)) return;
    const uint32_t hi = pool * lp.hcap + k;
    const HypHdr& h = lp.hyps[hi];
    if (!(h.state & kHypKeep)) return;
    const uint32_t g = h.g;
    if ((off64s[g + 1] >> 32) == (off64s[g] >> 32)) return;
    const unsigned long long o = off64s[g] + base64;
    const uint32_t view = gseg_view[g], seg = g - seg_base[view];
    const SegHdr sh = lp.segs[seg_of_g[g]];
    uint32_t w = (uint32_t)o;
    for (uint32_t y = sh.hyp_begin; y < hi; ++y) w += (lp.hyps[y].state & kHypKeep) ? 1u : 0u;
    Match m; uint32_t tv, tseg;
    make_match(views, pairs, view, seg, h, m, tv, tseg);
    surv_tg[w] = seg_base[tv] + tseg;
    surv_sg[w] = g;
    surv[w] = m;
    if (h.canon == 0xFFFFFFFFu - (uint32_t)best_pack[g]) {
        const uint32_t hx = (uint32_t)(o >> 32);
        const ViewDev& v = views[view];
        HypRec r;
        const SegX& sx = v.segx[seg];
        const Seg3 s3 = unproject(v.C, sx.r1, sx.r2, h.dp1, h.dp2);
        r.P1[0] = s3.P1.x; r.P1[1] = s3.P1.y; r.P1[2] = s3.P1.z;
        r.P2[0] = s3.P2.x; r.P2[1] = s3.P2.y; r.P2[2] = s3.P2.z;
        r.dir[0] = s3.dir.x; r.dir[1] = s3.dir.y; r.dir[2] = s3.dir.z;
        r.length = s3.length;
        r.valid = s3.length > 0.0f ? 1u : 0u;
        r.m = m;
        r.view = view; r.pad = 0;
        hyps[hx] = r;
        depths[2 * hx] = h.dp1;
        depths[2 * hx + 1] = h.dp2;
    }
}

std::atomic<uint64_t> g_csr_global_launches{0};

hipError_t launch_pair_csr(const PairDesc* pairs, uint32_t n_pairs, uint32_t max_Mt, const PairCsr* pair_poff,
                           const uint32_t* inv_tgt, uint32_t tgt16, uint32_t* poff, uint32_t* refs,
                           uint32_t* dummy, uint32_t tgt_v0, uint32_t tgt_v1, uint64_t max_pair_slots,
                           const uint32_t* row_start, hipStream_t st) {
    if (!n_pairs) return hipSuccess;
    const bool force_global = std::getenv("L3D_CSR_GLOBAL") != nullptr;
    const uint32_t lds_segs = force_global ? 0u : kCsrLdsSegs;
    const size_t lds = ((size_t)std::min(max_Mt, lds_segs) + 64) * 4;
    static const hipError_t attr_rc = [] {
        const int mx = (int)(((size_t)kCsrLdsSegs + 64) * 4);
        hipError_t e = hipFuncSetAttribute((const void*)k_pair_csr<true, true, false>, hipFuncAttributeMaxDynamicSharedMemorySize, mx);
        if (e == hipSuccess) e = hipFuncSetAttribute((const void*)k_pair_csr<true, false, false>, hipFuncAttributeMaxDynamicSharedMemorySize, mx);
        return e;
    }();
    if (attr_rc != hipSuccess) return attr_rc;
    if (tgt16 && !force_global && max_Mt <= lds_segs) {
        const size_t cur_bytes = ((size_t)lds_segs_round(max_Mt) + 64) * 4;
        const size_t two = 78 * 1024, one = 156 * 1024 - 4096;
        const size_t want = (size_t)(0.6 * (double)max_pair_slots) * 4 + 4096;
        const size_t budget = cur_bytes + want <= two ? two : one;
        size_t cap = (budget - cur_bytes) / 4;
        cap = std::min<size_t>(cap, (size_t)std::max<uint64_t>(max_pair_slots, 1024));
        static const hipError_t attr2 = hipFuncSetAttribute((const void*)k_pair_csr<true, true, true>, hipFuncAttributeMaxDynamicSharedMemorySize, 156 * 1024);
        if (attr2 != hipSuccess) return attr2;
        hipLaunchKernelGGL((k_pair_csr<true, true, true>), dim3(n_pairs), dim3(kCsrBlock), cur_bytes + cap * 4, st, pairs, 0u, pair_poff, inv_tgt,
                           poff, refs, dummy, tgt_v0, tgt_v1, lds_segs, (uint32_t)cap, row_start);
        return hipGetLastError();
    }
#define L3D_CSR(T16)                                                                                                      \
    do {                                                                                                                  \
        hipLaunchKernelGGL((k_pair_csr<true, T16, false>), dim3(n_pairs), dim3(kCsrBlock), lds, st, pairs, 0u, pair_poff, inv_tgt, \
                           poff, refs, dummy, tgt_v0, tgt_v1, lds_segs, 0u, row_start);                                   \
        if (max_Mt > lds_segs) {  \
            hipLaunchKernelGGL((k_pair_csr<false, T16, false>), dim3(n_pairs), dim3(kCsrBlock), 0, st, pairs, 0u, pair_poff, inv_tgt, \
                               poff, refs, dummy, tgt_v0, tgt_v1, lds_segs, 0u, row_start);                               \
            g_csr_global_launches.fetch_add(1, std::memory_order_relaxed);                                                \
        }                                                                                                                 \
    } while (0)
    if (tgt16) L3D_CSR(true); else L3D_CSR(false);
#undef L3D_CSR
    return hipGetLastError();
}

__global__ void k_publish_flags(const ListPools lp) {
    if (threadIdx.x < 4) lp.cnt[lp.pool0 * 16 + 8 + threadIdx.x] = lp.flags[threadIdx.x];
    if (threadIdx.x == 4) lp.cnt[lp.pool0 * 16 + 12] = lp.flags[6];
}

__global__ void k_merge_flags(const ListPools lp, uint32_t world) {
    const uint32_t ppr = kListPools / world;
    uint32_t f0 = 0, f2 = 0;
    for (uint32_t r = 0; r < world; ++r) { f0 |= lp.cnt[(size_t)r * ppr * 16 + 8]; f2 |= lp.cnt[(size_t)r * ppr * 16 + 10]; }
    if (f0) lp.flags[0] = 1;
    if (f2) lp.flags[2] = 1;
}

__global__ void k_seg_index(const ListPools lp, uint32_t* __restrict__ seg_of_g) {
    if (lp.flags[0] | lp.flags[2]) return;
    const uint32_t pool = lp.pool0 + blockIdx.y, k = blockIdx.x * blockDim.x + threadIdx.x;
    if (k >= min(lp.cnt[pool * 16 + 2], lp.scap)) return;
    seg_of_g[lp.segs[pool * lp.scap + k].g] = pool * lp.scap + k;
}
hipError_t launch_seg_index(ListPools lp, uint32_t* seg_of_g, uint32_t G, uint32_t world, hipStream_t st) {
    hipLaunchKernelGGL(k_merge_flags, dim3(1), dim3(1), 0, st, lp, world ? world : 1u);
    hipLaunchKernelGGL(k_seg_index, dim3((lp.scap + 255) / 256, lp.npools), dim3(256), 0, st, lp, seg_of_g);
    return hipGetLastError();
}

constexpr uint32_t kLists2Grid = 16384;
hipError_t launch_lists(uint32_t v0, uint32_t nv, uint32_t max_M, const ViewDev* views, const PairDesc* pairs,
                        const ListView* lviews, const OutPair* opairs, const InPair* ipairs, const uint32_t* gseg_view,
                        const uint32_t* poff, const uint32_t* inv, const float2* hyp_p, const float2* hyp_q, const Slot* slots, uint32_t uniform_K,
                        SimConst sc, ListPools lp, uint32_t* seg_of_g, HugeScratchArgs hsa, hipStream_t st) {
    if (!nv || !max_M) return hipSuccess;
    const bool wide = hsa.mean_list > 96;
#define L3D_LISTS(B)                                                                                                       \
    do {                                                                                                                   \
        const size_t lds1 = ListCfg<1, B>::BYTES, lds2 = ListCfg<2, B>::BYTES, lds4 = ListCfg<4, B>::BYTES;                \
        hipError_t e = hipFuncSetAttribute((const void*)k_lists<1, B>, hipFuncAttributeMaxDynamicSharedMemorySize, (int)lds1); \
        if (e != hipSuccess) return e;                                                                                     \
        e = hipFuncSetAttribute((const void*)k_lists<2, B>, hipFuncAttributeMaxDynamicSharedMemorySize, (int)lds2);        \
        if (e != hipSuccess) return e;                                                                                     \
        e = hipFuncSetAttribute((const void*)k_lists<4, B>, hipFuncAttributeMaxDynamicSharedMemorySize, (int)lds4);        \
        if (e != hipSuccess) return e;                                                                                     \
        for (uint32_t a = 0; a < nv; a += 65535u) {                                                      \
            const uint32_t n = nv - a < 65535u ? nv - a : 65535u;                                                          \
            hipLaunchKernelGGL((k_lists<1, B>), dim3(max_M, n), dim3(64), lds1, st, views, pairs, lviews, opairs, ipairs,  \
                               gseg_view, poff, inv, hyp_p, hyp_q, uniform_K, lp, v0 + a);                                        \
        }                                                                                                                  \
           \
        hipLaunchKernelGGL((k_lists<2, B>), dim3(kLists2Grid), dim3(128), lds2, st, views, pairs, lviews, opairs, ipairs, \
                           gseg_view, poff, inv, hyp_p, hyp_q, uniform_K, lp, 0u);                                                \
            \
            \
        if (hsa.run_tier4)                                                                                                 \
        hipLaunchKernelGGL((k_lists<4, B>), dim3(kLists4Grid), dim3(256), lds4, st, views, pairs, lviews, opairs, ipairs, \
                           gseg_view, poff, inv, hyp_p, hyp_q, uniform_K, lp, 0u);                                                \
    } while (0)
    if (wide) L3D_LISTS(256); else L3D_LISTS(128);
#undef L3D_LISTS
    HugeScratch hs;
    hs.d1 = hsa.f32; hs.d2 = hsa.f32 + hsa.cap;
    hs.tv = hsa.u32; hs.ref = hsa.u32 + hsa.cap; hs.pf = hsa.u32 + 2 * (size_t)hsa.cap;
    hs.key = hsa.u64; hs.cap = hsa.cap;
    if (hsa.run_huge)
        hipLaunchKernelGGL(k_lists_huge, dim3(256), dim3(256), 0, st, views, pairs, lviews, opairs, ipairs, gseg_view, poff,
                           inv, hyp_p, hyp_q, lp, hs);
    hipLaunchKernelGGL(k_cand_exact, dim3((lp.ccap + 255) / 256, lp.npools), dim3(256), 0, st, views, pairs, gseg_view, sc, lp);
    hipLaunchKernelGGL(k_edges, dim3((lp.scap + kEdgesSplit - 1) / kEdgesSplit, lp.npools), dim3(64), 0, st, views, pairs,
                       gseg_view, slots, lp, seg_of_g);
    if (lp.npools < kListPools) hipLaunchKernelGGL(k_publish_flags, dim3(1), dim3(64), 0, st, lp);
    return hipGetLastError();
}

static dim3 hyp_grid(const ListPools& lp) { return dim3((lp.hcap + 255) / 256, lp.npools); }

hipError_t launch_chain_sweep(ListPools lp, uint8_t* positive, uint32_t* changed, uint32_t sweep, uint32_t* undecided, hipStream_t st) {
    if (sweep == 0) hipLaunchKernelGGL(k_chain_sweep, hyp_grid(lp), dim3(256), 0, st, lp, positive, changed, undecided);
    else hipLaunchKernelGGL(k_chain_sweep_list, dim3(kChainListBlocks, lp.npools), dim3(256), 0, st, lp, positive, changed, sweep, undecided);
    return hipGetLastError();
}
hipError_t launch_hyp_scores(ListPools lp, const uint8_t* positive, const uint32_t* gseg_view, Slot* slots,
                             const uint8_t* pair_present, uint32_t* max_score_bits, hipStream_t st) {
    hipLaunchKernelGGL(k_hyp_scores, hyp_grid(lp), dim3(256), 0, st, lp, positive, gseg_view, slots, pair_present, max_score_bits);
    return hipGetLastError();
}
hipError_t launch_hyp_filter(ListPools lp, uint32_t g0, uint32_t g1, const uint32_t* gseg_view, const uint32_t* max_score_bits,
                             uint32_t* kept_cnt, unsigned long long* best_pack, unsigned long long* cnt64,
                             hipStream_t st) {
    hipLaunchKernelGGL(k_hyp_filter, hyp_grid(lp), dim3(256), 0, st, lp, gseg_view, max_score_bits, kept_cnt, best_pack);
    if (g1 > g0) hipLaunchKernelGGL(k_seg_filter, dim3((g1 - g0 + 255) / 256), dim3(256), 0, st, g0, g1, kept_cnt, best_pack, cnt64);
    return hipGetLastError();
}
hipError_t launch_seg_write(uint32_t g0, uint32_t g1, unsigned long long base64, const ViewDev* views, const PairDesc* pairs, const uint32_t* seg_base,
                            const uint32_t* gseg_view, const unsigned long long* off64s,
                            const unsigned long long* best_pack, const uint32_t* seg_of_g, ListPools lp,
                            const Slot* slots, uint32_t* surv_off, uint32_t* hyp_off, Match* surv, uint32_t* surv_tg,
                            uint32_t* surv_sg, int32_t* hyp_of_seg, HypRec* hyps, float* depths, hipStream_t st) {
    const uint64_t n_thr = std::max<uint64_t>((uint64_t)(g1 - g0) + 1, (uint64_t)lp.npools * lp.hcap);
    hipLaunchKernelGGL(k_seg_write, dim3((uint32_t)((n_thr + 255) / 256)), dim3(256), 0, st, g0, g1, base64, views, pairs, seg_base, gseg_view,
                       off64s, best_pack, seg_of_g, lp, slots, surv_off, hyp_off, surv, surv_tg, surv_sg, hyp_of_seg,
                       hyps, depths);
    return hipGetLastError();
}

}


namespace l3d {
namespace { __global__ void k_warm_lists() {} }
hipError_t warm_lists(hipStream_t st) {
    hipLaunchKernelGGL(k_warm_lists, dim3(1), dim3(64), 0, st);
    return hipGetLastError();
}
}
```

### line3dpp_amd/csrc/k_selftest.hip

```cpp
#include "l3d_ctx.h"

namespace l3d {
namespace {

__device__ __forceinline__ uint64_t mix64(uint64_t z) {
    z += 0x9E3779B97F4A7C15ull; z = (z ^ (z >> 30)) * 0xBF58476D1CE4E5B9ull; z = (z ^ (z >> 27)) * 0x94D049BB133111EBull;
    return z ^ (z >> 31);
}
__device__ __forceinline__ double draw(uint64_t& st, int lo10, int hi10) {
    st = mix64(st);
    const double m = 1.0 + (double)(st >> 12) * (1.0 / 4503599627370496.0);
    st = mix64(st);
    const int e10 = lo10 + (int)(st % (uint64_t)(hi10 - lo10 + 1));
    const double v = m * pow(10.0, (double)e10);
    return (st >> 40) & 1 ? -v : v;
}

__global__ void k_selftest_arith(uint64_t n, uint64_t seed, unsigned long long* out) {
    const uint64_t i0 = (uint64_t)blockIdx.x * blockDim.x + threadIdx.x, stride = (uint64_t)gridDim.x * blockDim.x;
    unsigned long long bad_div = 0, bad_sqrt = 0, bad_div2 = 0;
    for (uint64_t i = i0; i < n; i += stride) {
        uint64_t st = seed ^ (i * 0xD1342543DE82EF95ull);
        const int kind = (int)(i % 4);
        double a = kind == 3 ? 0.0 : draw(st, kind == 0 ? -3 : -72, kind == 0 ? 8 : 60);
        double a2 = draw(st, -20, 20);
        const double b = draw(st, kind == 0 ? -3 : -12, kind == 0 ? 8 : 52);
        if (kind == 2) a = b * (1.0 + (double)((int)(st % 9) - 4) * 2.220446049250313e-16);
        const double q_ref = a / b, q2_ref = a2 / b;
        double q1, q2;
        L3D_DIV2(true, a, a2, b, q1, q2);
        const double qs = L3D_DIV(true, a, b);
        bad_div2 += (__double_as_longlong(q1) != __double_as_longlong(q_ref)) + (__double_as_longlong(q2) != __double_as_longlong(q2_ref));
        bad_div += __double_as_longlong(qs) != __double_as_longlong(q_ref);
        const double x = kind == 3 ? 0.0 : fabs(draw(st, kind == 0 ? -2 : -180, kind == 0 ? 14 : 140));
        bad_sqrt += __double_as_longlong(L3D_SQRT(true, x)) != __double_as_longlong(sqrt(x));
        const double r = floor(fabs(draw(st, 0, 7))), sq = r * r;
        bad_sqrt += __double_as_longlong(L3D_SQRT(true, sq)) != __double_as_longlong(sqrt(sq));
    }
    atomicAdd(&out[0], bad_div); atomicAdd(&out[1], bad_div2); atomicAdd(&out[2], bad_sqrt);
}

}
}

extern "C" int l3d_selftest_arith(int device, uint64_t n, uint64_t seed, uint64_t counts[3]) {
    if (!counts) return fail(L3D_ERR_ARG, "null argument");
    if (int rc = set_device(device)) return rc;
    l3d::DevBuf<unsigned long long> buf;
    L3D_HIP_CHECK(buf.reserve(3));
    unsigned long long* d = buf.p;
    L3D_HIP_CHECK(hipMemset(d, 0, 24));
    hipLaunchKernelGGL(l3d::k_selftest_arith, dim3(2048), dim3(256), 0, 0, n, seed, d);
    L3D_HIP_CHECK(hipGetLastError());
    unsigned long long h[3];
    L3D_HIP_CHECK(hipMemcpy(h, d, 24, hipMemcpyDeviceToHost));
    counts[0] = h[0]; counts[1] = h[1]; counts[2] = h[2];
    return L3D_OK;
}

extern "C" int l3d_selftest_scan(int device, uint32_t element_bytes, const void* in, uint32_t n_in, uint32_t n_calls,
                                 const uint32_t* n, int in_place, int pass_total, void* out, void* totals,
                                 uint64_t* ws_nonzero, uint64_t* guard_changed) {
    constexpr size_t kGuard = 8;
    constexpr unsigned long long kPattern = 0xA5C3965A5AC3A569ull;
    if (element_bytes != 4 && element_bytes != 8) return fail(L3D_ERR_ARG, "l3d_selftest_scan: elements of 4 or 8 bytes");
    if ((!in && n_in) || (!n && n_calls) || !out || !ws_nonzero || !guard_changed || (pass_total && !totals))
        return fail(L3D_ERR_ARG, "null argument");
    size_t n_out = 0; uint32_t n_max = 0;
    for (uint32_t k = 0; k < n_calls; ++k) {
        if (n[k] > n_in) return fail(L3D_ERR_ARG, "l3d_selftest_scan: call " + std::to_string(k) + " is longer than the input");
        n_out += (size_t)n[k] + 1; n_max = std::max(n_max, n[k]);
    }
    *ws_nonzero = 0; *guard_changed = 0;
    if (!n_calls) return L3D_OK;
    if (int rc = set_device(device)) return rc;
    const size_t eb = element_bytes, words = l3d::scan_ws_words(n_max, element_bytes);
    l3d::DevBuf<char> d_in, d_out, d_tot; l3d::DevBuf<unsigned long long> ws;
    std::vector<unsigned long long> h_ws(words + kGuard, kPattern);
    L3D_HIP_CHECK(d_in.reserve(std::max<size_t>(1, n_in) * eb)); L3D_HIP_CHECK(d_out.reserve(n_out * eb));
    L3D_HIP_CHECK(d_tot.reserve((size_t)n_calls * eb));
    L3D_HIP_CHECK(ws.reserve_zeroed(words + kGuard, 0));
    L3D_HIP_CHECK(hipMemcpy(ws.p + words, h_ws.data(), kGuard * 8, hipMemcpyHostToDevice));
    if (n_in) L3D_HIP_CHECK(hipMemcpy(d_in.p, in, (size_t)n_in * eb, hipMemcpyHostToDevice));
    L3D_HIP_CHECK(hipMemset(d_out.p, 0xEE, n_out * eb)); L3D_HIP_CHECK(hipMemset(d_tot.p, 0xEE, (size_t)n_calls * eb));
    size_t at = 0;
    for (uint32_t k = 0; k < n_calls; at += (size_t)n[k] + 1, ++k) {
        char* o = d_out.p + at * eb; char* t = pass_total ? d_tot.p + (size_t)k * eb : nullptr;
        const char* src = d_in.p;
        if (in_place) {
            if (n[k]) L3D_HIP_CHECK(hipMemcpyAsync(o, d_in.p, (size_t)n[k] * eb, hipMemcpyDeviceToDevice, 0));
            src = o;
        }
        if (element_bytes == 4)
            L3D_HIP_CHECK(l3d::launch_scan((const uint32_t*)src, n[k], (uint32_t*)o, ws.p, (uint32_t*)t, 0));
        else
            L3D_HIP_CHECK(l3d::launch_scan64((const unsigned long long*)src, n[k], (unsigned long long*)o, ws.p, (unsigned long long*)t, 0));
    }
    L3D_HIP_CHECK(hipDeviceSynchronize());
    L3D_HIP_CHECK(hipMemcpy(out, d_out.p, n_out * eb, hipMemcpyDeviceToHost));
    if (pass_total) L3D_HIP_CHECK(hipMemcpy(totals, d_tot.p, (size_t)n_calls * eb, hipMemcpyDeviceToHost));
    L3D_HIP_CHECK(hipMemcpy(h_ws.data(), ws.p, (words + kGuard) * 8, hipMemcpyDeviceToHost));
    for (size_t i = 0; i < words; ++i) *ws_nonzero += h_ws[i] != 0;
    for (size_t i = 0; i < kGuard; ++i) *guard_changed += h_ws[words + i] != kPattern;
    return L3D_OK;
}
```

### line3dpp_amd/csrc/l3d_ctx.h

```cpp
#pragma once
#include <algorithm>
#include <chrono>
#include <cstdio>
#include <cstdlib>
#include <fstream>
#include <memory>
#include <mutex>
#include <sstream>
#include <unordered_set>

#include "l3d_host.h"
#include "l3d_lists.h"
#include "l3d_recon.h"

struct l3d_ctx;

namespace l3d {

size_t scan_ws_words(size_t n, uint32_t bytes_per_element);
hipError_t launch_scan(const uint32_t* in, uint32_t n, uint32_t* out, unsigned long long* ws, uint32_t* total, hipStream_t);
hipError_t launch_collin(int pass, const ViewDev* views, uint32_t n_views, uint32_t max_M, const uint32_t* seg_base,
                         float collin_t, uint32_t* cnt, const uint32_t* coll_off, uint32_t* coll_idx, hipStream_t);
hipError_t launch_aff_coll_count(int mode, uint32_t n_items, const uint32_t* surv_tg, const float* simv, const HypRec*,
                                 const uint32_t* seg_base, const uint32_t* coll_off, uint32_t* cnt, hipStream_t);
hipError_t launch_aff_coll_sim(int mode, uint32_t n_items, const uint32_t* surv_sg, const uint32_t* surv_tg,
                               const int32_t* hyp_of_seg, const HypRec*, const ViewDev*, const uint32_t* seg_base,
                               const uint32_t* gseg_view, const uint32_t* coll_off, const uint32_t* coll_idx,
                               const uint32_t* item_off, const ViewAff*, const float* medians, const float* msdl,
                               float two_sigA_sqr, uint32_t* out_seg, float* out_sim, hipStream_t);
hipError_t launch_seam_entries(uint32_t n, const float4* m4, const float2* rt, const ViewDev*, float k, DEntry*, hipStream_t);
hipError_t launch_seam_all_present(uint32_t G, const uint32_t* off, const uint32_t* boff, uint64_t* bits, hipStream_t);
hipError_t launch_seam_scores_out(uint32_t n, const DEntry*, float* scores, hipStream_t);
hipError_t launch_fill_gseg_view(const uint32_t* seg_base, uint32_t V, uint32_t max_M, uint32_t* gseg_view, hipStream_t);
hipError_t launch_orient_pairs(const ViewDev*, const PairDesc*, uint32_t n_pairs, uint64_t max_slots, Slot* slots,
                               uint32_t* inv_tgt, uint32_t tgt16, float2* hyp_p, float2* hyp_q, double thr_lo, double thr_hi, hipStream_t);
hipError_t launch_bits_len(uint32_t G, const uint32_t* off, uint32_t* len, uint32_t* long_list, uint32_t* n_long,
                           hipStream_t);
hipError_t launch_support_long(uint32_t n_long, const uint32_t* long_list, const uint32_t* off, const uint32_t* boff,
                               const DEntry*, uint64_t* bits, const ViewDev*, const uint32_t* gseg_view, SimConst,
                               hipStream_t);
hipError_t launch_support_all(uint32_t g0, uint32_t G, const uint32_t* off, const uint32_t* boff, const DEntry*, uint64_t* bits,
                              const ViewDev*, const uint32_t* seg_base, const uint32_t* gseg_view, SimConst, hipStream_t);
hipError_t launch_score_all(uint32_t g0, uint32_t G, const uint32_t* off, const uint32_t* boff, const uint32_t* gseg_view, DEntry*,
                            const uint64_t* bits, Slot*, uint32_t* max_score_bits, const ViewDev*, const uint32_t* seg_base,
                            SimConst, hipStream_t);
hipError_t launch_median_all(uint32_t V, const float* depths, const uint32_t* hyp_off, const uint32_t* seg_base,
                             const uint32_t* tie_total, uint32_t* tie_out, float* out, const uint32_t* rb_src,
                             uint32_t* rb_host, uint32_t rb_words, uint32_t* rb_count, hipStream_t, uint32_t v0 = 0);
hipError_t launch_aff_sim(uint32_t N, uint32_t lo, uint32_t hi, const uint32_t* surv_sg, const uint32_t* surv_tg, const int32_t* hyp_of_seg,
                          const HypRec*, const ViewAff*, const float* medians, const float* msdl, float two_sigA_sqr,
                          float* simv, int32_t* ca, int32_t* cb, hipStream_t);
hipError_t launch_aff_flag(uint32_t N, const uint32_t* surv_off, const uint32_t* surv_sg, const uint32_t* surv_tg,
                           const float* simv, const int32_t* ca, const int32_t* cb, uint32_t* flag,
                           uint32_t* first_touch, uint32_t H, uint32_t* touch_flag, hipStream_t);
hipError_t launch_fill_u32(uint32_t*, uint32_t n, uint32_t val, hipStream_t);
hipError_t launch_aff_touch(uint32_t N, const uint32_t* flag, const uint32_t* epos, const int32_t* ca,
                            const int32_t* cb, uint32_t* first_touch, hipStream_t);
hipError_t launch_aff_mark(uint32_t H, const uint32_t* first_touch, uint32_t* touch_flag, hipStream_t);
hipError_t launch_aff_emit(uint32_t N, const uint32_t* flag, const uint32_t* epos, const int32_t* ca,
                           const int32_t* cb, const float* simv, const uint32_t* first_touch,
                           const uint32_t* touch_rank, const HypRec*, void* edges, void* local2global, hipStream_t);

hipError_t warm_affinity(hipStream_t); hipError_t warm_lists(hipStream_t); hipError_t warm_match(hipStream_t);
hipError_t warm_rdd(hipStream_t); hipError_t warm_scan(hipStream_t); hipError_t warm_views(hipStream_t);

int fail(int code, const std::string& msg);
int set_device(int device);
const char* last_error_cstr();
void init_view(HostView& v, const double K[9], const double R[9], const double t[3]);
void translate_view(HostView& v, const d3& d);
d3 scene_translation(const std::vector<HostView*>& order);
void neighbors_from_worldpoints(const std::map<uint32_t, HostView*>& views, uint32_t num_neighbors);
void translate(::l3d_ctx& c);
void untranslate(::l3d_ctx& c);
struct Translated {
    ::l3d_ctx& c;
    bool on = true;
    explicit Translated(::l3d_ctx& ctx, bool adopt = false) : c(ctx) { if (!adopt) translate(c); }
    Translated(const Translated&) = delete;
    Translated& operator=(const Translated&) = delete;
    ~Translated() { if (on) untranslate(c); }
    void keep() { on = false; }
};
void make_cull(const double F[9], double ws, double hs, double wt, double ht, PairCull& pc);
void pair_baseline(const d3& Cs, const d3& Ct, PairDesc& pd);
void orientation_thresholds(double& lo, double& hi);
SimConst sim_thresholds(float two_sigA_sqr);
struct HostTrace {
    bool on = std::getenv("L3D_TRACE") != nullptr;
    std::chrono::steady_clock::time_point t0 = std::chrono::steady_clock::now();
    std::vector<std::pair<double, const char*>> marks;
    void mark(const char* what) {
        if (!on) return;
        marks.emplace_back(std::chrono::duration<double, std::micro>(std::chrono::steady_clock::now() - t0).count(), what);
    }
    void flush() {
        for (auto& m : marks) std::fprintf(stderr, "[l3d trace] %9.1f us  %s\n", m.first, m.second);
        marks.clear();
    }
};
extern HostTrace g_trace;

float ev_ms(hipEvent_t a, hipEvent_t b);
float ev_ms(const ::l3d_ctx* c, int a, int b);
int affinity_core(::l3d_ctx* c);
int ensure_affinity_host(::l3d_ctx* c);
std::string output_filename(::l3d_ctx* c, int max_image_width);
int line_opt(::l3d_ctx* c, const std::map<uint32_t, const HostView*>& views, std::vector<ReconCluster>& clusters, uint32_t max_iter);
bool line_to_cayley(const d3& P1, const d3& P2, double x[4]);
bool cayley_to_segment(const double x[4], const d3& P1_old, const d3& P2_old, d3& P1, d3& P2);

struct ProjWork {
    PinnedBuf<char> h;
    DevBuf<char> d;
    DevBuf<unsigned long long> keys, scan_ws;
    size_t budget = 0;
};

}

extern "C" void abort_match(::l3d_ctx* c);
extern "C" void collect_match_timing(::l3d_ctx* c);

using namespace l3d;

struct l3d_ctx {
    int device = 0;
    hipStream_t stream = nullptr;
    std::recursive_mutex mu;
    std::map<uint32_t, std::unique_ptr<HostView>> views;
    std::vector<HostView*> order;
    std::vector<float> views_avg_depths;
    float sigma_p = 2.5f, sigma_a = 10.0f, two_sigA_sqr = 200.0f, epipolar_overlap = 0.25f;
    float const_regularization_depth = -1.0f, med_scene_depth = (float)kEps, med_scene_depth_lines = 0.0f;
    int kNN = 10, num_neighbors = 10;
    bool fixed3Dregularizer = false;
    bool brute = false;
    bool knn_replay = false;
    double orient_lo = -1.0, orient_hi = 1.0;
    d3 translation{0, 0, 0};
    enum { IDLE, BEGUN, MATCHED } state = IDLE;
    bool affinity_done = false;
    std::vector<PairDesc> pairs;
    std::vector<uint32_t> pair_src_cam, pair_tgt_cam;
    std::vector<char> pair_done;
    DevBuf<uint8_t> d_pair_present;
    uint64_t n_slots = 0, pair_tests = 0;
    uint32_t n_rows_total = 0;
    DevBuf<ViewDev> d_views;
    DevBuf<PairDesc> d_pairs;
    DevBuf<WorkItem> d_work;
    DevBuf<Slot> d_slots;
    DevBuf<uint32_t> d_slot_idx;
    std::vector<PairCull> cull;
    DevBuf<PairCull> d_cull;
    DevBuf<uint32_t> d_src_perm, d_tgt_perm;
    DevBuf<float2> d_src_band, d_chunk_band, d_tgt_band;
    DevBuf<float4> d_tgt_sf, d_tgt_s4;
    DevBuf<SegD32> d_tgt_sd;
    DevBuf<uint32_t> d_item_bucket, d_item_order, d_order_done;
    DevBuf<uint64_t> d_cull_keys;
    bool use_cull = true;
    unsigned visibility_t = 3;
    bool perform_rdd = false;
    uint32_t aff_n_edges = 0, aff_n_rows = 0;
    bool aff_host_valid = true;
    PinnedBuf<uint32_t> h_cnt;
    std::vector<uint8_t> pair_counted;
    DevBuf<SegX> d_gsegx;
    DevBuf<SegD32> d_gsegd32;
    float collinearity_t = -1.0f;
    DevBuf<uint32_t> d_coll_cnt, d_coll_off, d_coll_idx, d_item_cnt, d_item_off, d_item_seg;
    DevBuf<float> d_item_sim;
    PinnedBuf<ViewDev> h_views;
    PinnedBuf<PairDesc> h_pairs;
    PinnedBuf<PairCull> h_cull;
    PinnedBuf<WorkItem> h_work;
    UploadTag up_views, up_pairs, up_cull, up_seg_base, up_ltab;
    std::vector<unsigned char> begin_sig; bool begin_sig_valid = false;
    uint64_t cull_tot[4] = {0, 0, 0, 0};
    uint32_t layout_rows = 0;
    uint32_t tile_rows = 0;
    uint64_t pairs_version = 0;
    struct { uint64_t version = ~0ull; uint32_t first = 0, count = 0, rows = 0; size_t items = 0; const void* dev = nullptr; } work_key;
    PinnedBuf<uint32_t> h_segb;
    const void* gseg_view_for = nullptr;
    bool timing_pending = false;
    uint32_t pending_launches = 0;
    DevBuf<uint32_t> d_row_counts;
    bool ragged = false;
    uint32_t keep_cap = 0;
    DevBuf<Slot> d_keep_rec;
    DevBuf<uint32_t> d_row_pair, d_blk_row;
    DevBuf<uint32_t> d_row_start, d_slot_row;
    DevBuf<uint4> d_keep_info;
    std::vector<uint64_t> pair_nslots;
    uint64_t keep_last_total = 0;
    PinnedBuf<uint4> h_keep_info;
    uint64_t pair_slots(uint32_t p) const { return ragged ? pair_nslots[p] : (uint64_t)pairs[p].Ms * pairs[p].K; }
    DevBuf<uint32_t> d_tie_count;
    uint32_t tie_seq = 0;
    DevBuf<uint2> d_tie_list;
    DevBuf<uint64_t> d_tie_heap;
    uint32_t G = 0, n_ents = 0, n_surv = 0, n_hyps = 0;
    std::vector<uint32_t> seg_base;
    DevBuf<uint32_t> d_seg_base, d_gseg_view, d_scal;
    DevBuf<uint32_t> d_surv_off, d_hyp_off, d_surv_tg, d_surv_sg;
    DevBuf<uint32_t> d_inv_tgt;
    DevBuf<float2> d_hyp_p, d_hyp_q;
    uint32_t tgt16 = 0;
    DevBuf<uint32_t> d_poff, d_csr_dummy;
    uint32_t poff_total = 0, n_in_pairs = 0;
    DevBuf<Match> d_surv;
    DevBuf<int32_t> d_hyp_of_seg;
    DevBuf<float> d_depths;
    float* d_med = nullptr;
    DevBuf<HypRec> d_hyps;
    DevBuf<unsigned long long> d_cnt64, d_off64s, d_scan_ws, d_huge_u64;
    DevBuf<uint32_t> d_inv_refs;
    DevBuf<uint32_t> d_lzero, d_list2, d_list4, d_listH, d_seg_of_g, d_huge_u32;
    DevBuf<float> d_huge_f32;
    DevBuf<EdgeRec> d_ledges;
    DevBuf<HypHdr> d_lhyps;
    DevBuf<SegHdr> d_lsegs;
    DevBuf<CandRec> d_lcands;
    DevBuf<CandHdr> d_lchdrs;
    uint32_t lp_ecap = 0, lp_hcap = 0, lp_scap = 0, lp_ccap = 0, huge_cap = 0;
    uint32_t lp_attempts = 0;
    bool huge_skip = false, huge_ran = true;
    bool list4_skip = false, list4_ran = true;
    struct PoolCaps { uint32_t e = 0, h = 0, s = 0, c = 0, huge = 0; bool huge_skip = false, list4_skip = false; } caps_saved[2];
    int caps_mode = 0;
    uint32_t chain_need = 8, chain_enqueued = 10;
    uint32_t chain_hist[4] = {6, 6, 6, 6}, chain_hist_at = 0;
    uint32_t shard_world = 0;
    uint32_t shard_rank = 0, shard_v0 = 0, shard_v1 = 0, shard_pool0 = 0, shard_ppr = 0;
    std::vector<uint32_t> tail_base_n, tail_base_h;
    bool tail_counted = false, tail_written = false;
    uint32_t shard_dep_rank0 = 0;
    bool exch_ordered = false;
    uint32_t aff_parts_world = 0;
    bool aff_shard_open = false;
    bool lists_ready = false, lists_prepared = false;
    PinnedBuf<uint32_t> h_fin;
    PinnedBuf<char> h_ltab;
    DevBuf<char> d_ltab;
    std::vector<uint32_t> h_surv_off, h_hyp_off;
    bool host_offsets_valid = false;
    DevBuf<ViewAff> d_vaff;
    DevBuf<float> d_simv;
    PinnedBuf<ViewAff> h_vaff; UploadTag up_vaff;
    DevBuf<int32_t> d_ca, d_cb;
    DevBuf<uint32_t> d_flag, d_epos, d_first_touch, d_touch_flag, d_touch_rank;
    DevBuf<l3d_cledge> d_edges;
    DevBuf<l3d_segment2d> d_l2g;
    std::vector<l3d_cledge> edges;
    std::vector<l3d_segment2d> l2g;
    std::vector<ReconLine> lines3D;
    bool lines_done = false;
    bool use_ceres = false;
    l3d_line_opt_summary lo_stats{};
    PinnedBuf<char> h_lopt;
    DevBuf<char> d_lopt;
    hipEvent_t lo_ev[2] = {};
    hipEvent_t ev[10] = {};
    int timing_level = 1;
    bool ev_on(int k) const { return timing_level >= 2 || (timing_level == 1 && (k == 4 || k == 5)); }
    l3d_timings tm{};
    std::vector<float> det_segs;
    std::vector<uint32_t> det_counts;
    std::vector<l3d_detect_stats> det_stats;
    ProjWork proj;
    std::vector<l3d_projected_segment> proj_records;
    ~l3d_ctx() {
        order.clear();
        for (auto& kv : views) kv.second.reset();
        for (auto& e : ev) if (e) (void)hipEventDestroy(e);
        for (auto& e : lo_ev) if (e) (void)hipEventDestroy(e);
    }
};
```

### line3dpp_amd/csrc/l3d_kernels.h

```cpp
#pragma once
#include <atomic>

#include "l3d_dev.h"

struct l3d_cledge;

namespace l3d {

extern std::atomic<uint64_t> g_knn_replay_calls;
extern std::atomic<uint64_t> g_keep_all_repeats;
extern std::atomic<uint64_t> g_live_blocks[2];
extern std::atomic<uint64_t> g_csr_global_launches;
extern std::atomic<uint64_t> g_seam_support_lists[4];
extern std::atomic<uint64_t> g_seam_score_unstaged_lists;
enum SupportTier : uint32_t { kSupportNone = 0, kSupportWave, kSupportGroupStaged, kSupportSortOnly, kSupportAllPairs };
struct ListTier { SupportTier support; bool score_unstaged; };
ListTier list_tier(uint32_t L);

constexpr int kMatchRows = 64;
constexpr uint32_t kTileClasses = 5;
constexpr uint32_t kTileMinItems = 24;
__host__ __device__ constexpr uint32_t tile_classes(uint32_t Ms, uint32_t R) { return Ms / R < kTileMinItems ? 2u : kTileClasses; }
__host__ __device__ constexpr uint32_t tile_src_cap(uint32_t Ms, uint32_t R) {
    return ((Ms + tile_classes(Ms, R) * (R - 1) + R - 1) / R) * R;
}
constexpr uint64_t kMatchTileMaxItems = 2048;
uint32_t match_tile_rows(int mode, bool brute, uint64_t est_row_items);
uint32_t match_layout_rows(int mode, bool brute, uint32_t tile_rows);
struct WorkItem {
    uint32_t pair;
    uint32_t src0;
};

struct PairCull {
    double As[3], Bs[3];
    double At[3], Bt[3];
    uint64_t s_off;
    uint64_t t_off;
    uint32_t c_off;
    uint32_t enabled;
    uint64_t k_off;
    uint32_t w_item0;
    uint32_t sorted_copy;
};
constexpr uint32_t kSortedCopyMinSegs = 4096;
struct CullPools {
    const PairCull* cull;
    uint32_t* src_perm;
    float2* src_band;
    uint32_t* tgt_perm;
    float4* tgt_sf;
    float2* tgt_band;
    float2* chunk_band;
    uint64_t* big_keys;
    uint32_t* item_bucket;
    uint32_t* item_order;
    uint32_t* order_done;
    uint32_t w_base;
    uint32_t cost_max;
    float4* tgt_s4;
    SegD32* tgt_sd;
    uint32_t row_cache;
    uint32_t padded_rows;
};
constexpr uint32_t kOrderBuckets = 1024;
constexpr uint32_t kCullLdsSegs = 16384;
constexpr uint32_t kCullBandCacheSegs = 4096;
constexpr uint32_t kCullMaxSegs = 1u << 20;

struct OrientFuse {
    uint32_t* inv_tgt;
    uint32_t tgt16;
    OrientThr thr;
    uint32_t* tie_count;
    uint2* tie_list;
    uint32_t tie_cap;
    uint32_t* tie_next;
    uint32_t* tie_total;
    float2* hyp_p;
    float2* hyp_q;
    Slot* keep_rec;
    uint32_t keep_cap;
    uint32_t* slot_row;
};

size_t match_lds_bytes(int mode, uint32_t K, bool ix16 = false, uint32_t waves = 1, bool brute = false, uint32_t tile_rows = 0,
                       bool row_cache = false);
bool match_row_cache(int mode, bool brute, uint32_t nwork, uint32_t tile_rows);
constexpr uint32_t kMatchOrderMaxItems = 16384;
constexpr uint32_t kMatchOrderMinItems = 3584;
uint32_t match_waves_per_group(int mode, bool brute, uint32_t nwork);
hipError_t launch_cull_prepare(const ViewDev* views, const PairDesc* pairs, uint32_t first, uint32_t count,
                               uint32_t max_M, CullPools pools, uint32_t tile_rows, hipStream_t stream);
hipError_t launch_order_items(const PairDesc* pairs, uint32_t first, uint32_t count, uint32_t max_Mt, CullPools pools,
                              uint32_t nwork, hipStream_t stream);
hipError_t launch_match_pairs(int mode, bool brute, const ViewDev* views, const PairDesc* pairs,
                              const WorkItem* work, uint32_t nwork, uint32_t maxK, Slot* slots,
                              uint32_t* row_counts, float thr, CullPools pools, OrientFuse of, bool ix16,
                              uint32_t tile_rows, hipStream_t stream);
uint32_t match_tied_grid(uint32_t scratch_stride);
hipError_t launch_queue_all_rows(const PairDesc* pairs, uint32_t first, uint32_t count, uint32_t max_Ms, uint32_t list_base,
                                 OrientFuse of, hipStream_t stream);
hipError_t launch_match_tied_rows(const ViewDev* views, const PairDesc* pairs, Slot* slots, uint32_t maxK, float thr,
                                  OrientFuse of, CullPools cp, uint64_t* scratch, uint32_t scratch_stride,
                                  hipStream_t stream);
hipError_t launch_pack_slot_idx(const Slot* slots, uint32_t* idx, uint64_t lo, uint64_t hi, hipStream_t stream);
hipError_t launch_expand_slot_idx(const ViewDev* views, const PairDesc* pairs, uint32_t first, uint32_t count,
                                  uint32_t max_row_slots, const uint32_t* idx, Slot* slots, OrientFuse of,
                                  hipStream_t stream);
constexpr uint32_t kKeepBlock = 1024;
hipError_t launch_keep_pair_info(const PairDesc* pairs, uint32_t n_pairs, const uint32_t* row_counts, const uint32_t* row_start,
                                 uint4* info, uint32_t* row_pair, uint32_t* blk_row, uint32_t n_blk, uint32_t* longest, hipStream_t stream);
hipError_t launch_keep_assemble(const ViewDev* views, const PairDesc* pairs, uint32_t n_rows, uint64_t slot_cap, const uint32_t* row_start,
                                const uint32_t* row_pair, const uint32_t* blk_row, const uint32_t* longest, Slot* slots, OrientFuse of,
                                hipStream_t stream);
hipError_t launch_prep_views(const ViewDev* views, uint32_t n_views, uint32_t max_M, hipStream_t stream);

struct InvRec; struct ListPools; struct PairCsr;
struct HugeScratchArgs { float* f32; uint32_t* u32; uint64_t* u64; uint32_t cap; uint32_t mean_list; uint32_t run_huge; uint32_t run_tier4; };
hipError_t launch_scan64(const unsigned long long* in, uint32_t n, unsigned long long* out, unsigned long long* tmp,
                         unsigned long long* total, hipStream_t st);
hipError_t launch_pair_csr(const PairDesc* pairs, uint32_t n_pairs, uint32_t max_Mt, const PairCsr* pair_csr,
                           const uint32_t* inv_tgt, uint32_t tgt16, uint32_t* poff, uint32_t* refs,
                           uint32_t* dummy, uint32_t tgt_v0, uint32_t tgt_v1, uint64_t max_pair_slots,
                           const uint32_t* row_start, hipStream_t st);
hipError_t launch_seg_index(ListPools lp, uint32_t* seg_of_g, uint32_t G, uint32_t world, hipStream_t st);
struct ListView; struct OutPair; struct InPair;
hipError_t launch_lists(uint32_t v0, uint32_t nv, uint32_t max_M, const ViewDev* views, const PairDesc* pairs,
                        const ListView* lviews, const OutPair* opairs, const InPair* ipairs, const uint32_t* gseg_view,
                        const uint32_t* poff, const uint32_t* inv_refs, const float2* hyp_p, const float2* hyp_q,
                        const Slot* slots, uint32_t uniform_K,
                        SimConst sc, ListPools lp, uint32_t* seg_of_g, HugeScratchArgs hsa, hipStream_t st);
hipError_t launch_chain_sweep(ListPools lp, uint8_t* positive, uint32_t* changed, uint32_t sweep, uint32_t* undecided,
                              hipStream_t st);
hipError_t launch_hyp_scores(ListPools lp, const uint8_t* positive, const uint32_t* gseg_view, Slot* slots,
                             const uint8_t* pair_present, uint32_t* max_score_bits, hipStream_t st);
hipError_t launch_hyp_filter(ListPools lp, uint32_t g0, uint32_t g1, const uint32_t* gseg_view, const uint32_t* max_score_bits,
                             uint32_t* kept_cnt, unsigned long long* best_pack, unsigned long long* cnt64,
                             hipStream_t st);
hipError_t launch_seg_write(uint32_t g0, uint32_t g1, unsigned long long base64, const ViewDev* views, const PairDesc* pairs, const uint32_t* seg_base,
                            const uint32_t* gseg_view, const unsigned long long* off64s,
                            const unsigned long long* best_pack, const uint32_t* seg_of_g, ListPools lp,
                            const Slot* slots, uint32_t* surv_off, uint32_t* hyp_off, Match* surv, uint32_t* surv_tg,
                            uint32_t* surv_sg, int32_t* hyp_of_seg, HypRec* hyps, float* depths, hipStream_t st);

size_t rdd_workspace_bytes(uint32_t nnz, uint32_t n_rows);
hipError_t launch_rdd(const struct ::l3d_cledge* edges_in, uint32_t nnz, uint32_t n_rows, uint32_t iterations,
                      struct ::l3d_cledge* edges_out, void* workspace, size_t workspace_bytes, hipStream_t stream);

struct TriArgs {
    const double* P;
    uint32_t n_cameras;
    uint64_t n_points;
    const uint64_t* off;
    const uint32_t* cam;
    const double* xy;
    double* X;
    uint8_t* valid;
};
constexpr size_t kTriLdsBytes = 32 * 1024;
hipError_t launch_triangulate(const TriArgs& t, hipStream_t st);

struct ProjRecord { float x1, y1, x2, y2, iz1, iz2; uint32_t line, segment; };
constexpr uint32_t kProjNear = 0x80000000u, kProjRect = 0x40000000u;
struct ProjCam { double K[9], R[9], t[3], xmax, ymax; };
struct ProjArgs {
    const ProjCam* cams;
    uint32_t n_cams, n_seg;
    const double* P;
    const uint32_t* line;
    double near_plane;
    ProjRecord* rec;
    uint32_t* vis;
    ProjRecord* out;
    uint32_t* bounds;
};
hipError_t launch_project_lines(const ProjArgs& a, hipStream_t st);
hipError_t launch_project_compact(const ProjArgs& a, hipStream_t st);
struct MapCam {
    uint32_t width, height;
    uint32_t rec0;
    uint32_t img_stride, img_channels, pad;
    uint64_t pix0;
    uint64_t img_off;
    uint64_t rgb_off;
};
struct MapArgs {
    const MapCam* cams; uint32_t n_cams;
    const ProjRecord* rec; uint32_t n_rec;
    uint32_t* steps;
    uint32_t thickness;
    unsigned long long* keys;
    uint64_t n_pix; uint32_t max_pix;
    int32_t* line_id; float* inv_depth;
    const uint8_t* img; uint8_t* rgb;
    const uint8_t* colors; uint32_t n_lines, alpha;
};
hipError_t launch_raster_count(const MapArgs& a, hipStream_t st);
hipError_t launch_raster_lines(const MapArgs& a, uint32_t blocks, hipStream_t st);
hipError_t launch_map_decode(const MapArgs& a, hipStream_t st);
hipError_t launch_overlay(const MapArgs& a, hipStream_t st);

}
```

### line3dpp_amd/csrc/l3d_phase_b.hip

```cpp
#include "l3d_ctx.h"

extern "C" {

static int match_finish_impl(l3d_ctx* c);
static int lists_prepare(l3d_ctx* c, int caps_mode);
static int lists_reserve(l3d_ctx* c);
static int lists_run(l3d_ctx* c, uint32_t v0, uint32_t nv, uint32_t pool0, uint32_t npools);

static int lists_shard_impl(l3d_ctx* c, uint32_t rank, uint32_t world, int64_t view0, int64_t view1, void* slab_ptr[4],
                            uint64_t slab_bytes[4], void* full_ptr[4]) {
    if (!c || !slab_ptr || !slab_bytes || !full_ptr) return fail(L3D_ERR_ARG, "null argument");
    std::lock_guard<std::recursive_mutex> lk(c->mu);
    if (c->state != l3d_ctx::BEGUN) return fail(L3D_ERR_STATE, "l3d_match_begin must precede l3d_lists_shard");
    (void)hipSetDevice(c->device);
    const int rc = [&]() -> int {
        if (world == 0 || world > kListPools || rank >= world) return fail(L3D_ERR_ARG, "rank / world out of range");
        const uint32_t V = (uint32_t)c->order.size();
        uint32_t v0, v1;
        if (view0 >= 0) {
            if (view1 < view0 || (uint64_t)view1 > V) return fail(L3D_ERR_ARG, "view range out of bounds");
            v0 = (uint32_t)view0; v1 = (uint32_t)view1;
        } else {
            uint64_t G = 0;
            std::vector<uint64_t> base(V + 1, 0);
            for (uint32_t vi = 0; vi < V; ++vi) base[vi + 1] = base[vi] + c->order[vi]->M;
            G = base[V];
            auto bound = [&](uint32_t r) -> uint32_t {
                if (r >= world) return V;
                const uint64_t target = G * r / world;
                uint32_t v = 0;
                while (v < V && base[v] < target) ++v;
                return v;
            };
            v0 = bound(rank); v1 = bound(rank + 1);
        }
        for (size_t p = 0; p < c->pairs.size(); ++p) {
            const PairDesc& pd = c->pairs[p];
            const bool touches = (pd.src >= v0 && pd.src < v1) || (pd.tgt >= v0 && pd.tgt < v1);
            if (touches && !c->pair_done[p])
                return fail(L3D_ERR_STATE, "l3d_lists_shard: the slots of a pair that touches this rank's views are not present");
        }
        int r2;
        if (!c->lists_prepared) {
            r2 = lists_prepare(c, 1);
            if (r2) return r2;
            c->lists_prepared = true; c->lp_attempts = 0;
        }
        r2 = lists_reserve(c);
        if (r2) return r2;
        const uint32_t ppr = kListPools / world, pool0 = rank * ppr;
        r2 = lists_run(c, v0, v1 - v0, pool0, ppr);
        if (r2) return r2;
        c->shard_rank = rank; c->shard_v0 = v0; c->shard_v1 = v1; c->shard_pool0 = pool0; c->shard_ppr = ppr;
        c->tail_counted = false; c->tail_written = false;
        if (!c->exch_ordered) L3D_HIP_CHECK(hipStreamSynchronize(c->stream));
        c->shard_world = world; c->lists_ready = true;
        slab_ptr[0] = c->d_ledges.p + (size_t)pool0 * c->lp_ecap; slab_bytes[0] = (uint64_t)ppr * c->lp_ecap * sizeof(EdgeRec); full_ptr[0] = c->d_ledges.p;
        slab_ptr[1] = c->d_lhyps.p + (size_t)pool0 * c->lp_hcap; slab_bytes[1] = (uint64_t)ppr * c->lp_hcap * sizeof(HypHdr); full_ptr[1] = c->d_lhyps.p;
        slab_ptr[2] = c->d_lsegs.p + (size_t)pool0 * c->lp_scap; slab_bytes[2] = (uint64_t)ppr * c->lp_scap * sizeof(SegHdr); full_ptr[2] = c->d_lsegs.p;
        slab_ptr[3] = c->d_lzero.p + (size_t)pool0 * 16; slab_bytes[3] = (uint64_t)ppr * 16 * 4; full_ptr[3] = c->d_lzero.p;
        return L3D_OK;
    }();
    if (rc != L3D_OK) {
        const std::string why = l3d_last_error();
        abort_match(c);
        set_error(why);
    }
    return rc;
}

int l3d_lists_shard(l3d_ctx* c, uint32_t rank, uint32_t world, void* slab_ptr[4], uint64_t slab_bytes[4], void* full_ptr[4]) {
    return lists_shard_impl(c, rank, world, -1, -1, slab_ptr, slab_bytes, full_ptr);
}
int l3d_lists_shard_views(l3d_ctx* c, uint32_t rank, uint32_t world, uint32_t view0, uint32_t view1, void* slab_ptr[4],
                          uint64_t slab_bytes[4], void* full_ptr[4]) {
    return lists_shard_impl(c, rank, world, (int64_t)view0, (int64_t)view1, slab_ptr, slab_bytes, full_ptr);
}

int l3d_plan_shards(uint32_t n_views, uint32_t n_pairs, const uint32_t* pair_src_view, const uint64_t* pair_cost,
                    uint32_t world, uint32_t* view_bounds, uint32_t* pair_bounds) {
    if (!world || !view_bounds || !pair_bounds || (n_pairs && (!pair_src_view || !pair_cost))) return fail(L3D_ERR_ARG, "null argument");
    std::vector<double> vcost(n_views + 1, 0.0);
    for (uint32_t p = 0; p < n_pairs; ++p) {
        if (pair_src_view[p] >= n_views || (p && pair_src_view[p] < pair_src_view[p - 1]))
            return fail(L3D_ERR_ARG, "pair list is not ordered by source view");
        vcost[pair_src_view[p]] += (double)pair_cost[p];
    }
    double total = 0.0;
    for (uint32_t v = 0; v < n_views; ++v) total += vcost[v];
    view_bounds[0] = 0;
    uint32_t v = 0; double acc = 0.0;
    for (uint32_t r = 1; r < world; ++r) {
        const double target = total * r / world;
        while (v < n_views && std::fabs(acc + vcost[v] - target) <= std::fabs(acc - target)) { acc += vcost[v]; ++v; }
        view_bounds[r] = v;
    }
    view_bounds[world] = n_views;
    uint32_t p = 0;
    for (uint32_t r = 0; r <= world; ++r) {
        while (p < n_pairs && pair_src_view[p] < view_bounds[r]) ++p;
        pair_bounds[r] = p;
    }
    pair_bounds[world] = n_pairs;
    return L3D_OK;
}

int l3d_match_finish(l3d_ctx* c) {
    if (!c) return fail(L3D_ERR_ARG, "null argument");
    std::lock_guard<std::recursive_mutex> lk(c->mu);
    if (c->state != l3d_ctx::BEGUN) return fail(L3D_ERR_STATE, "l3d_match_begin must precede l3d_match_finish");
    (void)hipSetDevice(c->device);
    const int rc = match_finish_impl(c);
    if (rc == L3D_ERR_RETRY) return rc;
    if (rc != L3D_OK) {
        const std::string why = l3d_last_error();
        abort_match(c);
        set_error(why);
    }
    return rc;
}

static constexpr uint32_t kChainSweeps = 16;

static ListPools list_pools(l3d_ctx* c, uint32_t pool0 = 0, uint32_t npools = kListPools) {
    ListPools lp;
    lp.cnt = c->d_lzero.p; lp.edges = c->d_ledges.p; lp.hyps = c->d_lhyps.p; lp.segs = c->d_lsegs.p;
    lp.cands = c->d_lcands.p; lp.chdrs = c->d_lchdrs.p;
    lp.ecap = c->lp_ecap; lp.hcap = c->lp_hcap; lp.scap = c->lp_scap; lp.ccap = c->lp_ccap;
    lp.flags = c->d_lzero.p + kListPools * 16;
    lp.list2 = c->d_list2.p; lp.list4 = c->d_list4.p; lp.listH = c->d_listH.p;
    lp.pool0 = pool0; lp.npools = npools;
    lp.row_start = c->ragged ? c->d_row_start.p : nullptr; lp.slot_row = c->ragged ? c->d_slot_row.p : nullptr;
    static const bool no_stat = std::getenv("L3D_NO_LIST_STAT") != nullptr;
    lp.count_entries = no_stat ? 0u : 1u;
    return lp;
}

static unsigned long long* tot64_of(l3d_ctx* c) { return (unsigned long long*)c->d_med; }
static float* medians_of(l3d_ctx* c) { return c->d_med + 8; }
static size_t fin_med(uint32_t V) { return ((size_t)8 + V + 3) & ~(size_t)3; }
static constexpr size_t kFinHead = (size_t)kListPools * 16 + 96;

struct ZeroLayout { size_t flags, changed, med, max_score, kept, best, words; };
static ZeroLayout zero_layout(uint32_t V, uint32_t G);
static uint8_t* positive_of(l3d_ctx* c) {
    return (uint8_t*)(c->d_lzero.p + zero_layout((uint32_t)c->order.size(), c->G).words);
}
static ZeroLayout zero_layout(uint32_t V, uint32_t G) {
    ZeroLayout z;
    z.flags = (size_t)kListPools * 16; z.changed = z.flags + 32; z.med = z.changed + 64; z.max_score = z.med + fin_med(V);
    z.kept = z.max_score + ((size_t)V + 1) * 16;
    z.best = (z.kept + G + 1) & ~(size_t)1;
    z.words = z.best + 2 * (size_t)G + 2;
    return z;
}

static int lists_prepare(l3d_ctx* c, int caps_mode) {
    if (caps_mode != c->caps_mode) {
        c->caps_saved[c->caps_mode] = l3d_ctx::PoolCaps{c->lp_ecap, c->lp_hcap, c->lp_scap, c->lp_ccap, c->huge_cap, c->huge_skip, c->list4_skip};
        const l3d_ctx::PoolCaps& pc = c->caps_saved[caps_mode];
        c->lp_ecap = pc.e; c->lp_hcap = pc.h; c->lp_scap = pc.s; c->lp_ccap = pc.c; c->huge_cap = pc.huge; c->huge_skip = pc.huge_skip;
        c->list4_skip = pc.list4_skip;
        c->caps_mode = caps_mode;
    }
    if (caps_mode == 1) { c->huge_skip = false; c->list4_skip = false; }
    hipStream_t st = c->stream;
    const uint32_t V = (uint32_t)c->order.size(), P = (uint32_t)c->pairs.size();
    c->seg_base.assign(V + 1, 0);
    for (uint32_t vi = 0; vi < V; ++vi) c->seg_base[vi + 1] = c->seg_base[vi] + c->order[vi]->M;
    const uint32_t G = c->G = c->seg_base[V];
    uint64_t max_slots = 0;
    for (uint32_t p = 0; p < P; ++p) max_slots = std::max<uint64_t>(max_slots, c->pair_slots(p));
    if (2 * c->n_slots >= (1ull << 32)) return fail(L3D_ERR_LIMIT, "more than 2^32 hypotheses");
    L3D_HIP_CHECK(c->d_seg_base.reserve(V + 1)); L3D_HIP_CHECK(c->d_gseg_view.reserve(G + 1));
    L3D_HIP_CHECK(c->d_surv_off.reserve(G + 2)); L3D_HIP_CHECK(c->d_hyp_off.reserve(G + 2));
    L3D_HIP_CHECK(c->d_hyp_of_seg.reserve(G + 1));
    L3D_HIP_CHECK(c->d_cnt64.reserve(G + 2)); L3D_HIP_CHECK(c->d_off64s.reserve(G + 2));
    L3D_HIP_CHECK(c->d_scan_ws.reserve_zeroed(scan_ws_words(G, 8), st));
    L3D_HIP_CHECK(c->d_seg_of_g.reserve(G + 1)); L3D_HIP_CHECK(c->d_list2.reserve(G + 1)); L3D_HIP_CHECK(c->d_list4.reserve(G + 1)); L3D_HIP_CHECK(c->d_listH.reserve(G + 1));
    L3D_HIP_CHECK(c->d_hyps.reserve(std::max<uint32_t>(G, 1))); L3D_HIP_CHECK(c->d_depths.reserve(2 * (size_t)G + 2));
    L3D_HIP_CHECK(c->d_inv_refs.reserve(std::max<uint64_t>(c->n_slots, 1)));
    L3D_HIP_CHECK(c->d_inv_tgt.reserve(std::max<uint64_t>(c->n_slots, 1)));
    L3D_HIP_CHECK(c->d_hyp_p.reserve(std::max<uint64_t>(c->n_slots, 1))); L3D_HIP_CHECK(c->d_hyp_q.reserve(std::max<uint64_t>(c->n_slots, 1)));
    L3D_HIP_CHECK(c->h_fin.reserve(kFinHead + fin_med(V)));
    if (c->ev_on(6)) L3D_HIP_CHECK(hipEventRecord(c->ev[6], st));
    g_trace.mark("finish: reserves done");
    {
        bool sent = false;
        L3D_HIP_CHECK(upload_table(c->d_seg_base, c->h_segb, c->seg_base.data(), ((size_t)V + 1) * 4, c->up_seg_base, st, &sent));
        if (sent || c->gseg_view_for != (const void*)c->d_gseg_view.p) {
            uint32_t max_M = 0;
            for (auto* v : c->order) max_M = std::max(max_M, v->M);
            L3D_HIP_CHECK(launch_fill_gseg_view(c->d_seg_base.p, V, max_M, c->d_gseg_view.p, st));
            c->gseg_view_for = c->d_gseg_view.p;
        }
    }
    {
        static_assert(sizeof(ListView) == 32 && sizeof(OutPair) == 32 && sizeof(InPair) == 16 && sizeof(PairCsr) == 16, "table layout");
        uint32_t n_in = 0;
        for (uint32_t vi = 0; vi < V; ++vi) n_in += (uint32_t)c->order[vi]->in_pairs.size();
        const size_t o_in = ((size_t)V + P) * 32, o_pp = o_in + (size_t)n_in * 16;
        std::vector<char> table(o_pp + ((size_t)P + 1) * 16 + 32, 0);
        ListView* hv = (ListView*)table.data();
        OutPair* hp = (OutPair*)(table.data() + (size_t)V * 32);
        InPair* hi = (InPair*)(table.data() + o_in);
        PairCsr* hpp = (PairCsr*)(table.data() + o_pp);
        for (uint32_t p = 0; p < P; ++p) hpp[p] = PairCsr{kEmpty, 0u, 0u, 0u};
        uint32_t n = 0, ni = 0;
        uint64_t poff_total = 0;
        for (uint32_t vi = 0; vi < V; ++vi) {
            ListView& lv = hv[vi];
            lv = ListView{};
            lv.seg_base = c->seg_base[vi]; lv.M = c->order[vi]->M; lv.q0 = n; lv.k = c->order[vi]->k;
            for (uint32_t p : c->order[vi]->out_pairs) {
                const PairDesc& pd = c->pairs[p];
                OutPair op{};
                op.slot_off = pd.slot_off; op.tgt = pd.tgt; op.pair = p; op.K = pd.K; op.row_off = pd.row_off;
                hp[n++] = op;
            }
            lv.nq = n - lv.q0;
            lv.i0 = ni; lv.ni = (uint32_t)c->order[vi]->in_pairs.size(); lv.pbase = (uint32_t)poff_total;
            uint32_t q = 0;
            for (uint32_t p : c->order[vi]->in_pairs) {
                const PairDesc& pd = c->pairs[p];
                InPair ip{};
                ip.rec_base = (uint32_t)pd.slot_off; ip.src = pd.src; ip.pair = p;
                hpp[p] = PairCsr{(uint32_t)poff_total, lv.ni, q++, 0u};
                hi[ni++] = ip;
            }
            poff_total += ((uint64_t)lv.M + 1) * lv.ni;
            if (poff_total >= (1ull << 32)) return fail(L3D_ERR_LIMIT, "more than 2^32 per-pair CSR offsets in phase B");
        }
        c->poff_total = (uint32_t)poff_total; c->n_in_pairs = ni;
        L3D_HIP_CHECK(c->d_poff.reserve(std::max<uint64_t>(poff_total, 1)));
        L3D_HIP_CHECK(c->d_ltab.reserve(table.size()));
        L3D_HIP_CHECK(upload_table(c->d_ltab, c->h_ltab, table.data(), o_pp + (size_t)P * 16, c->up_ltab, st));
    }
    for (uint32_t p0 = 0; p0 < P;) {
        if (c->pair_counted[p0] || !c->pair_done[p0]) { ++p0; continue; }
        uint32_t p1 = p0;
        while (p1 < P && !c->pair_counted[p1] && c->pair_done[p1]) ++p1;
        L3D_HIP_CHECK(launch_orient_pairs(c->d_views.p, c->d_pairs.p + p0, p1 - p0, max_slots, c->d_slots.p, c->d_inv_tgt.p,
                                          c->tgt16, c->d_hyp_p.p, c->d_hyp_q.p, c->orient_lo, c->orient_hi, st));
        for (uint32_t p = p0; p < p1; ++p) c->pair_counted[p] = 1;
        p0 = p1;
    }
    if (!c->lp_ecap) {
        const double scale = [] { const char* e = std::getenv("L3D_POOL_SCALE"); const double v = e ? std::atof(e) : 1.0; return v > 0.0 ? v : 1.0; }();
        const double ns = scale * (double)c->n_slots;
        const double bytes1 = ns * (sizeof(EdgeRec) / 4.0 + sizeof(HypHdr) / 8.0 + sizeof(CandRec) / 2.0);
        const double gen = scale < 1.0 ? 1.0 : std::min(4.0, std::max(1.0, 4.0e9 / std::max(bytes1, 1.0)));
        c->lp_ecap = (uint32_t)std::max<double>(gen * ns / 4 / kListPools, scale < 1.0 ? 16 : 512);
        c->lp_hcap = (uint32_t)std::max<double>(gen * ns / 8 / kListPools, scale < 1.0 ? 16 : 256);
        c->lp_ccap = (uint32_t)std::max<double>(gen * ns / 2 / kListPools, scale < 1.0 ? 32 : 1024);
    }
    c->lp_scap = std::max<uint32_t>(c->lp_scap, G / kListPools + 64);
    if (!c->huge_cap) c->huge_cap = (uint32_t)std::min<uint64_t>(std::max<uint64_t>(c->n_slots / 16, 1u << 20), 1u << 30);
    return L3D_OK;
}

static int lists_reserve(l3d_ctx* c) {
    g_trace.mark("lists_reserve enter");
    const uint32_t V = (uint32_t)c->order.size();
    const ZeroLayout z = zero_layout(V, c->G);
    L3D_HIP_CHECK(c->d_lzero.reserve(z.words + 2 + (c->n_slots + 3) / 4));
    c->d_med = (float*)(c->d_lzero.p + z.med);
    L3D_HIP_CHECK(c->d_ledges.reserve((size_t)kListPools * c->lp_ecap));
    L3D_HIP_CHECK(c->d_lhyps.reserve((size_t)kListPools * c->lp_hcap));
    L3D_HIP_CHECK(c->d_lsegs.reserve((size_t)kListPools * c->lp_scap));
    L3D_HIP_CHECK(c->d_lchdrs.reserve((size_t)kListPools * c->lp_scap));
    L3D_HIP_CHECK(c->d_lcands.reserve((size_t)kListPools * c->lp_ccap));
    L3D_HIP_CHECK(c->d_huge_f32.reserve(2 * (size_t)c->huge_cap)); L3D_HIP_CHECK(c->d_huge_u32.reserve(3 * (size_t)c->huge_cap));
    L3D_HIP_CHECK(c->d_huge_u64.reserve(c->huge_cap));
    const size_t surv_cap = (size_t)kListPools * c->lp_hcap;
    L3D_HIP_CHECK(c->d_surv.reserve(surv_cap)); L3D_HIP_CHECK(c->d_surv_tg.reserve(surv_cap));
    L3D_HIP_CHECK(c->d_surv_sg.reserve(surv_cap));
    return L3D_OK;
}

static int lists_run(l3d_ctx* c, uint32_t v0, uint32_t nv, uint32_t pool0, uint32_t npools) {
    g_trace.mark("lists_run enter");
    hipStream_t st = c->stream;
    const uint32_t V = (uint32_t)c->order.size(), P = (uint32_t)c->pairs.size(), G = c->G;
    const ZeroLayout z = zero_layout(V, G);
    const ListPools lp = list_pools(c, pool0, npools);
    const SimConst simc = sim_thresholds(c->two_sigA_sqr);
    uint64_t max_slots = 0;
    for (uint32_t p = 0; p < P; ++p) max_slots = std::max<uint64_t>(max_slots, c->pair_slots(p));
    L3D_HIP_CHECK(hipMemsetAsync(c->d_lzero.p, 0, z.words * 4 + std::max<uint64_t>(c->n_slots, 1), st));
    g_trace.mark("zero block memset enqueued");
    const ListView* lviews = (const ListView*)c->d_ltab.p;
    const OutPair* opairs = (const OutPair*)(c->d_ltab.p + (size_t)V * 32);
    const InPair* ipairs = (const InPair*)(c->d_ltab.p + ((size_t)V + P) * 32);
    const PairCsr* pair_poff = (const PairCsr*)(c->d_ltab.p + ((size_t)V + P) * 32 + (size_t)c->n_in_pairs * 16);
    {
        uint32_t max_Mt = 0;
        for (auto& pd : c->pairs) if (pd.tgt > pd.src && pd.tgt >= v0 && pd.tgt < v0 + nv) max_Mt = std::max(max_Mt, pd.Mt);
        if (max_Mt) {
            if (max_Mt > 32768 || std::getenv("L3D_CSR_GLOBAL")) L3D_HIP_CHECK(c->d_csr_dummy.reserve((size_t)P * 64));
            L3D_HIP_CHECK(launch_pair_csr(c->d_pairs.p, P, max_Mt, pair_poff, c->d_inv_tgt.p, c->tgt16, c->d_poff.p, c->d_inv_refs.p,
                                          c->d_csr_dummy.p, v0, v0 + nv, max_slots, c->ragged ? c->d_row_start.p : nullptr, st));
        }
    }
    g_trace.mark("pair CSRs enqueued");
    const uint32_t mean_list = c->n_ents ? (uint32_t)(c->n_ents / std::max<uint32_t>(G, 1))
                                         : (uint32_t)(1.5 * (double)c->n_slots / std::max<uint32_t>(G, 1));
    const HugeScratchArgs hsa{c->d_huge_f32.p, c->d_huge_u32.p, (uint64_t*)c->d_huge_u64.p, c->huge_cap, mean_list,
                              c->huge_skip ? 0u : 1u, c->list4_skip ? 0u : 1u};
    c->huge_ran = !c->huge_skip; c->list4_ran = !c->list4_skip;
    uint32_t max_M = 0;
    for (uint32_t vi = v0; vi < v0 + nv; ++vi) max_M = std::max(max_M, c->order[vi]->M);
    L3D_HIP_CHECK(launch_lists(v0, nv, max_M, c->d_views.p, c->d_pairs.p, lviews, opairs, ipairs, c->d_gseg_view.p,
                               c->d_poff.p, c->d_inv_refs.p, c->d_hyp_p.p, c->d_hyp_q.p, c->d_slots.p, c->kNN > 0 ? (uint32_t)c->kNN : 0u, simc, lp,
                               c->d_seg_of_g.p, hsa, st));
    if (c->ev_on(9)) L3D_HIP_CHECK(hipEventRecord(c->ev[9], st));
    g_trace.mark("list pass enqueued");
    return L3D_OK;
}

struct TailShard { uint32_t v0, v1, g0, g1, pool0, npools; };
static TailShard whole_tail(const l3d_ctx* c) { return TailShard{0u, (uint32_t)c->order.size(), 0u, c->G, 0u, kListPools}; }

static int tail_count_run(l3d_ctx* c, bool fresh, const TailShard& ts) {
    g_trace.mark("tail_run enter");
    hipStream_t st = c->stream;
    const uint32_t V = (uint32_t)c->order.size(), G = c->G;
    const ZeroLayout z = zero_layout(V, G);
    const bool dep = ts.npools < kListPools && c->shard_world > 1 && c->shard_dep_rank0 <= c->shard_rank;
    const uint32_t cp0 = dep ? c->shard_dep_rank0 * c->shard_ppr : 0u, cp1 = dep ? (c->shard_rank + 1) * c->shard_ppr : kListPools;
    const ListPools lp = list_pools(c, cp0, cp1 - cp0), lps = list_pools(c, ts.pool0, ts.npools);
    uint32_t* changed = c->d_lzero.p + z.changed;
    uint32_t* max_score = c->d_lzero.p + z.max_score;
    uint32_t* kept = c->d_lzero.p + z.kept;
    unsigned long long* best = (unsigned long long*)(c->d_lzero.p + z.best);
    if (!fresh) L3D_HIP_CHECK(hipMemsetAsync(changed, 0, (z.words - z.changed) * 4, st));
    const uint32_t need = std::max(std::max(c->chain_hist[0], c->chain_hist[1]), std::max(c->chain_hist[2], c->chain_hist[3]));
    const uint32_t n_sweeps = std::min(kChainSweeps, std::max(4u, need + 3));
    c->chain_enqueued = n_sweeps;
    if (!fresh) L3D_HIP_CHECK(hipMemset2DAsync(c->d_lzero.p + 7, 64, 0, 4, kListPools, st));
    for (uint32_t s2 = 0; s2 < n_sweeps; ++s2)
        L3D_HIP_CHECK(launch_chain_sweep(lp, positive_of(c), changed, s2, c->d_surv_tg.p, st));
    g_trace.mark("chain sweeps enqueued");
    const uint8_t* present = nullptr;
    if (c->shard_world > 1) {
        L3D_HIP_CHECK(c->d_pair_present.reserve(std::max<size_t>(c->pair_done.size(), 1)));
        L3D_HIP_CHECK(hipMemcpyAsync(c->d_pair_present.p, c->pair_done.data(), c->pair_done.size(), hipMemcpyHostToDevice, st));
        present = c->d_pair_present.p;
    }
    L3D_HIP_CHECK(launch_hyp_scores(lps, positive_of(c), c->d_gseg_view.p, c->d_slots.p, present, max_score, st));
    g_trace.mark("hyp_scores enqueued");
    L3D_HIP_CHECK(launch_hyp_filter(lps, ts.g0, ts.g1, c->d_gseg_view.p, max_score, kept, best, c->d_cnt64.p, st));
    g_trace.mark("hyp_filter enqueued");
    L3D_HIP_CHECK(launch_scan64(c->d_cnt64.p + ts.g0, ts.g1 - ts.g0, c->d_off64s.p + ts.g0, c->d_scan_ws.p, tot64_of(c) + 1, st));
    g_trace.mark("scan enqueued");
    return L3D_OK;
}

static int tail_write_run(l3d_ctx* c, const TailShard& ts, unsigned long long base64, bool publish) {
    hipStream_t st = c->stream;
    const uint32_t V = (uint32_t)c->order.size(), G = c->G;
    const ZeroLayout z = zero_layout(V, G);
    const ListPools lps = list_pools(c, ts.pool0, ts.npools);
    unsigned long long* best = (unsigned long long*)(c->d_lzero.p + z.best);
    L3D_HIP_CHECK(launch_seg_write(ts.g0, ts.g1, base64, c->d_views.p, c->d_pairs.p, c->d_seg_base.p, c->d_gseg_view.p,
                                   c->d_off64s.p, best, c->d_seg_of_g.p, lps, c->d_slots.p, c->d_surv_off.p, c->d_hyp_off.p,
                                   c->d_surv.p, c->d_surv_tg.p, c->d_surv_sg.p, c->d_hyp_of_seg.p, c->d_hyps.p, c->d_depths.p, st));
    g_trace.mark("seg_write enqueued");
    void* h_dev = nullptr;
    L3D_HIP_CHECK(hipHostGetDevicePointer(&h_dev, c->h_fin.p, 0));
    L3D_HIP_CHECK(launch_median_all(ts.v1 - ts.v0, c->d_depths.p, c->d_hyp_off.p, c->d_seg_base.p,
                                    c->d_tie_count.p ? c->d_tie_count.p + 2 : nullptr, (uint32_t*)tot64_of(c), medians_of(c),
                                    c->d_lzero.p, publish ? (uint32_t*)h_dev : nullptr, (uint32_t)(kFinHead + fin_med(V)),
                                    c->d_lzero.p + z.flags + 16, st, ts.v0));
    g_trace.mark("median + read-back enqueued");
    return L3D_OK;
}

static int tail_run(l3d_ctx* c, bool fresh) {
    const TailShard ts = whole_tail(c);
    int rc = tail_count_run(c, fresh, ts);
    if (rc) return rc;
    rc = tail_write_run(c, ts, 0ull, true);
    if (rc) return rc;
    if (c->ev_on(7)) L3D_HIP_CHECK(hipEventRecord(c->ev[7], c->stream));
    g_trace.mark("tail enqueued");
    return L3D_OK;
}

static constexpr int kRetry = 1;
static int check_pass(l3d_ctx* c) {
    const uint32_t* h = c->h_fin.p;
    const uint32_t* hf = h + kListPools * 16;
    uint32_t fl[8];
    for (int k = 0; k < 8; ++k) fl[k] = hf[k];
    if (c->shard_world > 1) {
        const uint32_t ppr = kListPools / c->shard_world;
        for (uint32_t r = 0; r < c->shard_world; ++r)
            for (int k = 0; k < 4; ++k) fl[k] |= h[(size_t)r * ppr * 16 + 8 + k];
        fl[6] = 0;
        for (uint32_t r = 0; r < c->shard_world; ++r) fl[6] = std::max(fl[6], h[(size_t)r * ppr * 16 + 12]);
    }
    if (fl[1]) return fail(L3D_ERR_LIMIT, "a 2D segment has more than 65535 match hypotheses");
    const bool huge_missed = (fl[5] && !c->huge_ran) || (fl[4] && !c->list4_ran);
    c->huge_skip = fl[5] == 0 && c->shard_world <= 1;
    c->list4_skip = fl[4] == 0 && c->shard_world <= 1;
    if (huge_missed) { ++c->tm.pool_retries; return kRetry; }
    if (fl[3]) return fail(L3D_ERR_HIP, "internal error: hypothesis counters and slot flags disagree");
    if (fl[0] || fl[2]) {
        ++c->tm.pool_retries;
        if (++c->lp_attempts > 6) return fail(L3D_ERR_LIMIT, "phase-B pools keep overflowing");
        if (fl[0]) {
            uint32_t me = 0, mh = 0, ms = 0, mc = 0;
            for (uint32_t q = 0; q < kListPools; ++q) {
                me = std::max(me, h[q * 16]); mh = std::max(mh, h[q * 16 + 1]);
                ms = std::max(ms, std::max(h[q * 16 + 2], h[q * 16 + 4])); mc = std::max(mc, h[q * 16 + 3]);
            }
            const bool cands_over = mc > c->lp_ccap || ms > c->lp_scap;
            c->lp_ccap = std::max(c->lp_ccap, mc + mc / 2 + 64); c->lp_scap = std::max(c->lp_scap, ms + ms / 2 + 64);
            c->lp_ecap = std::max(cands_over ? 2 * c->lp_ecap : c->lp_ecap, me + me / 2 + 64);
            c->lp_hcap = std::max(cands_over ? 2 * c->lp_hcap : c->lp_hcap, mh + mh / 2 + 64);
        }
        if (fl[2]) c->huge_cap = (uint32_t)std::min<uint64_t>(std::max<uint64_t>(2ull * c->huge_cap, fl[6] + 1024ull), 1u << 31);
        return kRetry;
    }
    return L3D_OK;
}

static int finish_commit(l3d_ctx* c) {
    const uint32_t V = (uint32_t)c->order.size();
    const uint32_t* h = c->h_fin.p;
    const uint32_t* h0 = h + kFinHead;
    const uint32_t* changed = h + kListPools * 16 + 32;
    c->n_surv = h0[2]; c->n_hyps = h0[3];
    c->tm.tied_rows = h0[0];
    {
        uint64_t ents = 0, inv = 0, cands = 0, hdrs = 0;
        for (uint32_t q = 0; q < kListPools; ++q) { ents += h[q * 16 + 5]; inv += h[q * 16 + 6]; cands += h[q * 16 + 3]; hdrs += h[q * 16 + 1]; }
        c->n_ents = (uint32_t)std::min<uint64_t>(ents, 0xFFFFFFFFu);
        c->tm.list_entries = c->n_ents;
        c->tm.list_inverse = (uint32_t)std::min<uint64_t>(inv, 0xFFFFFFFFu);
        c->tm.list_candidates = (uint32_t)std::min<uint64_t>(cands, 0xFFFFFFFFu);
        c->tm.list_headers = (uint32_t)std::min<uint64_t>(hdrs, 0xFFFFFFFFu);
        c->tm.slots_lo = (uint32_t)c->n_slots; c->tm.slots_hi = (uint32_t)(c->n_slots >> 32);
    }
    for (uint32_t s2 = 0; s2 < c->chain_enqueued; ++s2) c->tm.chain_sweeps += changed[s2] ? 1u : 0u;
    c->chain_need = c->tm.chain_extra_rounds ? kChainSweeps : c->tm.chain_sweeps;
    c->chain_hist[c->chain_hist_at++ & 3u] = c->chain_need;
    {
        uint64_t ne = 0;
        uint32_t me = 0, mh = 0, ms = 0, mc = 0;
        for (uint32_t q = 0; q < kListPools; ++q) {
            ne += h[q * 16];
            me = std::max(me, h[q * 16]); mh = std::max(mh, h[q * 16 + 1]);
            ms = std::max(ms, std::max(h[q * 16 + 2], h[q * 16 + 4])); mc = std::max(mc, h[q * 16 + 3]);
        }
        c->tm.support_words = (uint32_t)ne;
        auto fit = [](uint32_t cap, uint32_t need, uint32_t lowest) {
            const uint32_t want = std::max(need + need / 4 + 64, lowest);
            return cap > want + want / 2 ? want : cap;
        };
        c->lp_ecap = fit(c->lp_ecap, me, 256); c->lp_hcap = fit(c->lp_hcap, mh, 128);
        c->lp_scap = fit(c->lp_scap, ms, 64); c->lp_ccap = fit(c->lp_ccap, mc, 512);
    }
    for (uint32_t vi = 0; vi < V; ++vi) c->order[vi]->median_depth = ((const float*)h0)[8 + vi];
    c->host_offsets_valid = false;
    if (c->timing_pending) {
        collect_match_timing(c);
        c->tm.match_pairs_ms += ev_ms(c, 2, 3);
    }
    c->tm.finish_ms = ev_ms(c, 6, 7);
    c->tm.lists_ms = ev_ms(c, 6, 9);
    c->tm.record_kbytes = (uint32_t)(((uint64_t)kListPools * ((uint64_t)c->lp_ecap * sizeof(EdgeRec) + (uint64_t)c->lp_hcap * sizeof(HypHdr) +
                                                              (uint64_t)c->lp_scap * sizeof(SegHdr) + 64)) >> 10);
    c->tm.begin_ms = ev_ms(c, 0, 1);
    untranslate(*c);
    c->state = l3d_ctx::MATCHED;
    c->shard_world = 0; c->lists_ready = false; c->lists_prepared = false;
    return L3D_OK;
}

static int tail_until_converged(l3d_ctx* c) {
    hipStream_t st = c->stream;
    int rc = tail_run(c, true);
    if (rc) return rc;
    g_trace.mark("phase B enqueued, waiting");
    L3D_HIP_CHECK(hipStreamSynchronize(st));
    g_trace.mark("phase B done");
    rc = check_pass(c);
    if (rc) return rc;
    while (c->h_fin.p[kListPools * 16 + 32 + c->chain_enqueued - 1]) {
        rc = tail_run(c, false);
        if (rc) return rc;
        L3D_HIP_CHECK(hipStreamSynchronize(st));
        ++c->tm.chain_extra_rounds;
    }
    return L3D_OK;
}

static int match_finish_impl(l3d_ctx* c) {
    int rc;
    if (c->lists_ready) {
        const ListPools lp = list_pools(c);
        L3D_HIP_CHECK(launch_seg_index(lp, c->d_seg_of_g.p, c->G, c->shard_world, c->stream));
        rc = tail_until_converged(c);
        if (rc == kRetry) { c->lists_ready = false; return fail(L3D_ERR_RETRY, "phase-B pools enlarged: repeat l3d_lists_shard and the exchange"); }
        if (rc) return rc;
        return finish_commit(c);
    }
    rc = lists_prepare(c, 0);
    if (rc) return rc;
    c->lp_attempts = 0;
    const uint32_t V = (uint32_t)c->order.size();
    for (;;) {
        rc = lists_reserve(c);
        if (rc) return rc;
        rc = lists_run(c, 0, V, 0, kListPools);
        if (rc) return rc;
        rc = tail_until_converged(c);
        if (rc == kRetry) continue;
        if (rc) return rc;
        break;
    }
    return finish_commit(c);
}

static int tail_count_until_converged(l3d_ctx* c, const TailShard& ts) {
    hipStream_t st = c->stream;
    const uint32_t V = (uint32_t)c->order.size();
    auto run = [&](bool fresh) -> int {
        const int rc = tail_count_run(c, fresh, ts);
        if (rc) return rc;
        L3D_HIP_CHECK(hipMemcpyAsync(c->h_fin.p, c->d_lzero.p, (kFinHead + fin_med(V)) * 4, hipMemcpyDeviceToHost, st));
        L3D_HIP_CHECK(hipStreamSynchronize(st));
        return L3D_OK;
    };
    int rc = run(true);
    if (rc) return rc;
    rc = check_pass(c);
    if (rc) return rc;
    while (c->h_fin.p[kListPools * 16 + 32 + c->chain_enqueued - 1]) {
        rc = run(false);
        if (rc) return rc;
        ++c->tm.chain_extra_rounds;
    }
    return L3D_OK;
}

static int close_failed_call(l3d_ctx* c, int rc) {
    if (rc != L3D_OK && rc != L3D_ERR_RETRY) {
        const std::string why = l3d_last_error();
        abort_match(c);
        set_error(why);
    }
    return rc;
}

int l3d_shard_options(l3d_ctx* c, uint32_t first_needed_rank, int exchanges_stream_ordered) {
    if (!c) return fail(L3D_ERR_ARG, "null argument");
    std::lock_guard<std::recursive_mutex> lk(c->mu);
    c->shard_dep_rank0 = first_needed_rank;
    c->exch_ordered = exchanges_stream_ordered != 0;
    return L3D_OK;
}

int l3d_tail_shard_count(l3d_ctx* c, uint32_t counts[2]) {
    if (!c || !counts) return fail(L3D_ERR_ARG, "null argument");
    std::lock_guard<std::recursive_mutex> lk(c->mu);
    if (c->state != l3d_ctx::BEGUN || !c->lists_ready || c->shard_world < 2)
        return fail(L3D_ERR_STATE, "l3d_tail_shard_count follows l3d_lists_shard* and the exchange of its slabs (world > 1)");
    (void)hipSetDevice(c->device);
    const int rc = [&]() -> int {
        if (c->shard_dep_rank0 > c->shard_rank) return fail(L3D_ERR_ARG, "l3d_shard_options: first_needed_rank lies above this rank");
        const ListPools lp = list_pools(c, c->shard_dep_rank0 * c->shard_ppr, (c->shard_rank + 1 - c->shard_dep_rank0) * c->shard_ppr);
        L3D_HIP_CHECK(launch_seg_index(lp, c->d_seg_of_g.p, c->G, c->shard_world, c->stream));
        const TailShard ts{c->shard_v0, c->shard_v1, c->seg_base[c->shard_v0], c->seg_base[c->shard_v1], c->shard_pool0, c->shard_ppr};
        const int r = tail_count_until_converged(c, ts);
        if (r == kRetry) { c->lists_ready = false; return fail(L3D_ERR_RETRY, "phase-B pools enlarged: repeat l3d_lists_shard and the exchange"); }
        if (r) return r;
        const uint32_t* med = c->h_fin.p + kFinHead;
        counts[0] = med[2]; counts[1] = med[3];
        c->tail_counted = true; c->tail_written = false;
        return L3D_OK;
    }();
    return close_failed_call(c, rc);
}

int l3d_tail_shard_layout(l3d_ctx* c, uint32_t world, const uint32_t* counts_all, const uint32_t* view_bounds, void* base_ptr[9],
                          uint64_t elt_bytes[9], uint64_t* first, uint64_t* count) {
    if (!c || !counts_all || !view_bounds || !base_ptr || !elt_bytes || !first || !count) return fail(L3D_ERR_ARG, "null argument");
    std::lock_guard<std::recursive_mutex> lk(c->mu);
    if (c->state != l3d_ctx::BEGUN || !c->tail_counted || world != c->shard_world)
        return fail(L3D_ERR_STATE, "l3d_tail_shard_layout follows l3d_tail_shard_count (same world size)");
    (void)hipSetDevice(c->device);
    const int rc = [&]() -> int {
        const uint32_t V = (uint32_t)c->order.size();
        if (view_bounds[0] != 0 || view_bounds[world] != V || view_bounds[c->shard_rank] != c->shard_v0 ||
            view_bounds[c->shard_rank + 1] != c->shard_v1)
            return fail(L3D_ERR_ARG, "view bounds do not match the list pass of this rank");
        c->tail_base_n.assign(world + 1, 0); c->tail_base_h.assign(world + 1, 0);
        uint64_t n = 0, h = 0;
        for (uint32_t r = 0; r < world; ++r) {
            if (view_bounds[r + 1] < view_bounds[r]) return fail(L3D_ERR_ARG, "view bounds are not ascending");
            c->tail_base_n[r] = (uint32_t)n; c->tail_base_h[r] = (uint32_t)h;
            n += counts_all[2 * r]; h += counts_all[2 * r + 1];
        }
        if (n >= (1ull << 32) || n > (uint64_t)kListPools * c->lp_hcap || h > c->G)
            return fail(L3D_ERR_LIMIT, "the ranks' counts exceed the output arrays");
        c->tail_base_n[world] = (uint32_t)n; c->tail_base_h[world] = (uint32_t)h;
        const uint32_t me = c->shard_rank;
        const TailShard ts{c->shard_v0, c->shard_v1, c->seg_base[c->shard_v0], c->seg_base[c->shard_v1], c->shard_pool0, c->shard_ppr};
        const int r2 = tail_write_run(c, ts, (unsigned long long)c->tail_base_n[me] | ((unsigned long long)c->tail_base_h[me] << 32), false);
        if (r2) return r2;
        if (!c->exch_ordered) L3D_HIP_CHECK(hipStreamSynchronize(c->stream));
        void* bp[9] = {c->d_surv.p, c->d_surv_tg.p, c->d_surv_sg.p, c->d_hyps.p, c->d_depths.p, c->d_surv_off.p, c->d_hyp_off.p,
                       c->d_hyp_of_seg.p, medians_of(c)};
        const uint64_t eb[9] = {sizeof(Match), 4, 4, sizeof(HypRec), 8, 4, 4, 4, 4};
        for (int k = 0; k < 9; ++k) { base_ptr[k] = bp[k]; elt_bytes[k] = eb[k]; }
        for (uint32_t r = 0; r < world; ++r) {
            const uint64_t g0 = c->seg_base[view_bounds[r]], g1 = c->seg_base[view_bounds[r + 1]], end = r + 1 == world ? 1 : 0;
            const uint64_t f[9] = {c->tail_base_n[r], c->tail_base_n[r], c->tail_base_n[r], c->tail_base_h[r], c->tail_base_h[r],
                                   g0, g0, g0, view_bounds[r]};
            const uint64_t m[9] = {counts_all[2 * r], counts_all[2 * r], counts_all[2 * r], counts_all[2 * r + 1], counts_all[2 * r + 1],
                                   g1 - g0 + end, g1 - g0 + end, g1 - g0, (uint64_t)view_bounds[r + 1] - view_bounds[r]};
            for (int k = 0; k < 9; ++k) { first[9 * r + k] = f[k]; count[9 * r + k] = m[k]; }
        }
        c->tail_written = true;
        return L3D_OK;
    }();
    return close_failed_call(c, rc);
}

int l3d_tail_shard_commit(l3d_ctx* c) {
    if (!c) return fail(L3D_ERR_ARG, "null argument");
    std::lock_guard<std::recursive_mutex> lk(c->mu);
    if (c->state != l3d_ctx::BEGUN || !c->tail_written)
        return fail(L3D_ERR_STATE, "l3d_tail_shard_commit follows l3d_tail_shard_layout and the exchange of the parts");
    (void)hipSetDevice(c->device);
    const int rc = [&]() -> int {
        const uint32_t V = (uint32_t)c->order.size(), world = c->shard_world;
        uint32_t* med = c->h_fin.p + kFinHead;
        if (c->ev_on(7)) L3D_HIP_CHECK(hipEventRecord(c->ev[7], c->stream));
        L3D_HIP_CHECK(hipMemcpyAsync(med, c->d_med, (8 + (size_t)V) * 4, hipMemcpyDeviceToHost, c->stream));
        L3D_HIP_CHECK(hipStreamSynchronize(c->stream));
        med[2] = c->tail_base_n[world]; med[3] = c->tail_base_h[world];
        c->tail_counted = false; c->tail_written = false;
        const int fr = finish_commit(c);
        if (fr == L3D_OK) c->aff_parts_world = world;
        return fr;
    }();
    return close_failed_call(c, rc);
}

}
```

Measured before the change: 975,300.

## Batch segments per block in k_edges and fold first chain sweep into it

k_edges changes from one 64-lane wave per segment to a 256-thread block that handles a batch of up to 32 segment headers at once. Candidates are staged in LDS with block-wide scans, and pool counters are reserved with one atomic set per batch. In the non-sharded path the kernel also takes positive/changed/undecided buffers so the first chain sweep is done inside it, and the tail then skips sweep 0. The aim is better occupancy, fewer atomics and one fewer kernel launch, at the cost of more block barriers, a binary search per staged element, and more complex correctness logic.

After: 1.007 million, median of 6. 1.03x the previous value.

```diff
diff --git a/include/l3dpp_hip.h b/include/l3dpp_hip.h
--- a/include/l3dpp_hip.h
+++ b/include/l3dpp_hip.h
@@ -251,6 +251,12 @@
 int l3d_selftest_scan(int device, uint32_t element_bytes, const void* in, uint32_t n_in, uint32_t n_calls, const uint32_t* n,
                       int in_place, int pass_total, void* out, void* totals, uint64_t* ws_nonzero, uint64_t* guard_changed);
 
+int l3d_selftest_edges_constants(uint32_t out[3]);
+int l3d_selftest_edges(int device, uint32_t npools, uint32_t scap, uint32_t ccap, uint32_t ecap, uint32_t hcap, const void* cands,
+                       const void* chdrs, const uint32_t* n_cands, const uint32_t* n_chdrs, const void* slots, uint32_t n_slots,
+                       uint32_t slots_per_row, const uint32_t* slot_row, uint32_t n_segments, int fold_sweep0, uint32_t* counters,
+                       void* edges, void* hyps, void* segs, uint32_t* seg_of_g, uint8_t* positive, uint32_t* undecided);
+
 int l3d_set_brute_force(l3d_ctx*, int on);
 
 typedef struct l3d_timings {
diff --git a/line3dpp_amd/_lib.py b/line3dpp_amd/_lib.py
--- a/line3dpp_amd/_lib.py
+++ b/line3dpp_amd/_lib.py
@@ -127,6 +127,7 @@
     "l3d_triangulate_points", "l3d_rotation_from_rpy", "l3d_rotation_from_q", "l3d_decompose_projection_matrix",
     "l3d_project_segments", "l3d_render_line_maps", "l3d_draw_line_maps", "l3d_view_camera", "l3d_project_lines",
     "l3d_get_projected_lines", "l3d_render_lines", "l3d_draw_lines", "l3d_set_projection_budget", "l3d_selftest_scan",
+    "l3d_selftest_edges_constants", "l3d_selftest_edges",
 ]
 
 _lib = None
@@ -224,6 +225,8 @@
     L.l3d_line_opt_eval.argtypes = [i32, u32, vp, vp, vp, vp, vp, vp, vp]
     L.l3d_selftest_arith.argtypes = [i32, u64, u64, vp]
     L.l3d_selftest_scan.argtypes = [i32, u32, vp, u32, u32, vp, i32, i32, vp, vp, C.POINTER(u64), C.POINTER(u64)]
+    L.l3d_selftest_edges_constants.argtypes = [vp]
+    L.l3d_selftest_edges.argtypes = [i32, u32, u32, u32, u32, u32, vp, vp, vp, vp, vp, u32, u32, vp, u32, i32, vp, vp, vp, vp, vp, vp, vp]
     L.l3d_detect_segments.argtypes = [vp, u32, vp, i32, u32, vp]
     L.l3d_detect_view_segments.argtypes = [vp, u32, vp, vp, C.POINTER(DetectOptions), vp]
     L.l3d_get_detected_segments.argtypes = [vp, vp, u64, C.POINTER(u64)]
diff --git a/line3dpp_amd/csrc/k_lists.hip b/line3dpp_amd/csrc/k_lists.hip
--- a/line3dpp_amd/csrc/k_lists.hip
+++ b/line3dpp_amd/csrc/k_lists.hip
@@ -774,134 +774,201 @@
     cr->sim = ok ? sim : -1.0f;
 }
 
-constexpr uint32_t kEdgeLds = 512;
-__device__ __forceinline__ void edges_of_segment(const PairDesc* __restrict__ pairs, const Slot* __restrict__ slots,
-                                                 const ListPools& lp, uint32_t* __restrict__ seg_of_g, const CandHdr ch,
-                                                 uint32_t opool, L3D_LDS uint32_t* s_ij_w, L3D_LDS float* s_sim_w,
-                                                 uint32_t lane) {
-    const uint32_t g = ch.g, n = ch.cnt;
-    CandRec* cand = lp.cands + ch.begin;
-    const uint64_t lt_mask = (1ull << lane) - 1ull;
-    const bool in_lds = n <= kEdgeLds;
-    uint32_t n_acc = 0;
-    for (uint32_t x0 = 0; x0 < n; x0 += 64) {
-        const uint32_t x = x0 + lane;
-        bool ok = false;
-        if (x < n) {
-            const float sim = cand[x].sim;
-            ok = sim >= 0.0f;
-            if (in_lds) { s_ij_w[x] = cand[x].ij; s_sim_w[x] = sim; }
-        }
-        n_acc += (uint32_t)__popcll(__builtin_amdgcn_ballot_w64(ok));
-    }
-    if (n_acc == 0) return;
-    if (in_lds) {
-        __builtin_amdgcn_fence(__ATOMIC_RELEASE, "workgroup");
-        __builtin_amdgcn_wave_barrier();
-        __builtin_amdgcn_fence(__ATOMIC_ACQUIRE, "workgroup");
-    }
-    auto ij_of = [&](uint32_t y) -> uint32_t { return in_lds ? s_ij_w[y] : cand[y].ij; };
-    auto sim_of = [&](uint32_t y) -> float { return in_lds ? s_sim_w[y] : cand[y].sim; };
-    auto in_run = [&](uint32_t x, uint32_t& rank, uint32_t& earlier, uint32_t& mine) {
-        const uint32_t ij = ij_of(x), i = ij >> 16;
-        rank = 0; earlier = 0; mine = 1;
-        for (uint32_t y = x; y-- > 0;) {
-            const uint32_t o = ij_of(y);
-            if ((o >> 16) != i) break;
-            if (sim_of(y) >= 0.0f) { ++earlier; ++mine; rank += o < ij ? 1u : 0u; }
-        }
-        for (uint32_t y = x + 1; y < n; ++y) {
-            const uint32_t o = ij_of(y);
-            if ((o >> 16) != i) break;
-            if (sim_of(y) >= 0.0f) { ++mine; rank += o < ij ? 1u : 0u; }
-        }
-    };
-    uint32_t n_h = 0;
-    for (uint32_t x0 = 0; x0 < n; x0 += 64) {
-        const uint32_t x = x0 + lane;
-        bool first = false;
-        if (x < n && sim_of(x) >= 0.0f) {
-            const uint32_t i = ij_of(x) >> 16;
-            first = true;
-            for (uint32_t y = x; y-- > 0;) {
-                if ((ij_of(y) >> 16) != i) break;
-                if (sim_of(y) >= 0.0f) { first = false; break; }
-            }
-        }
-        n_h += (uint32_t)__popcll(__builtin_amdgcn_ballot_w64(first));
-    }
-    uint32_t eb = 0, hb = 0, sb = 0;
-    if (lane == 0) {
-        eb = atomicAdd(&lp.cnt[opool * 16 + 0], n_acc);
-        hb = atomicAdd(&lp.cnt[opool * 16 + 1], n_h);
-        sb = atomicAdd(&lp.cnt[opool * 16 + 2], 1u);
-    }
-    eb = __shfl(eb, 0); hb = __shfl(hb, 0); sb = __shfl(sb, 0);
-    if (eb + n_acc > lp.ecap || hb + n_h > lp.hcap || sb + 1 > lp.scap) {
-        if (lane == 0) atomicOr(&lp.flags[0], 1u);
-        return;
-    }
-    const uint32_t e0 = opool * lp.ecap + eb, h0 = opool * lp.hcap + hb;
-    uint32_t acc_before = 0, first_before = 0;
-    for (uint32_t x0 = 0; x0 < n; x0 += 64) {
-        const uint32_t x = x0 + lane;
-        bool acc = false, first = false;
-        uint32_t rank = 0, earlier = 0, mine = 0;
-        float sim = -1.0f;
-        if (x < n) {
-            sim = sim_of(x);
-            acc = sim >= 0.0f;
-            if (acc) { in_run(x, rank, earlier, mine); first = earlier == 0; }
-        }
-        const uint64_t ma = __builtin_amdgcn_ballot_w64(acc), mf = __builtin_amdgcn_ballot_w64(first);
-        if (acc) {
-            const CandRec r = cand[x];
-            const uint32_t run0 = acc_before + (uint32_t)__popcll(ma & lt_mask) - earlier;
-            EdgeRec e;
-            e.ref_j = r.ref_j; e.sim = sim;
-            e.j_cam = (r.ij & 0xFFFFu) | ((r.tvj & kHypInv) ? kEdgeInv : 0u);
-            e.tv_j = r.tvj & 0x7FFFFFFFu;
-            lp.edges[e0 + run0 + rank] = e;
-            if (first) {
-                HypHdr hdr;
-                hdr.g = g; hdr.ref = r.ref_i; hdr.pair_flags = r.pf_i; hdr.canon = r.ij >> 16;
-                hdr.dp1 = r.a1; hdr.dp2 = r.a2;
-                hdr.edge_begin = e0 + run0; hdr.edge_cnt = mine; hdr.score3D = 0.0f; hdr.state = 0;
-                {
-                    const Slot hs = slots[r.ref_i];
-                    const bool hinv = (r.pf_i & kHypInv) != 0;
-                    const PairDesc& hp = pairs[r.pf_i & 0x7FFFFFFFu];
-                    hdr.tgt_seg = !hinv ? hs.tgt_seg : lp.slot_row ? lp.slot_row[r.ref_i] : (uint32_t)((r.ref_i - hp.slot_off) / hp.K);
-                    hdr.overlap = hs.overlap;
-                    hdr.oq1 = hinv ? hs.dp1 : hs.dq1; hdr.oq2 = hinv ? hs.dp2 : hs.dq2;
-                }
-                hdr.pad[0] = hdr.pad[1] = 0;
-                lp.hyps[h0 + first_before + (uint32_t)__popcll(mf & lt_mask)] = hdr;
-            }
-        }
-        acc_before += (uint32_t)__popcll(ma); first_before += (uint32_t)__popcll(mf);
-    }
-    if (lane == 0) {
-        const uint32_t si = opool * lp.scap + sb;
-        lp.segs[si] = SegHdr{g, h0, n_h, 0u};
-        seg_of_g[g] = si;
-    }
-}
-
-constexpr uint32_t kEdgesSplit = 4;
-__global__ __launch_bounds__(64) void k_edges(const ViewDev* __restrict__ views, const PairDesc* __restrict__ pairs,
-                                               const uint32_t* __restrict__ gseg_view, const Slot* __restrict__ slots,
-                                               const ListPools lp, uint32_t* __restrict__ seg_of_g) {
-    const uint32_t pool = lp.pool0 + blockIdx.y, lane = lane_id();
+#ifndef L3D_EDGE_BLOCK
+#define L3D_EDGE_BLOCK 256
+#endif
+#ifndef L3D_EDGE_BATCH
+#define L3D_EDGE_BATCH 32
+#endif
+constexpr uint32_t kEdgeBlock = L3D_EDGE_BLOCK;
+constexpr uint32_t kEdgeWaves = kEdgeBlock / 64;
+constexpr uint32_t kEdgeBatch = L3D_EDGE_BATCH;
+constexpr uint32_t kEdgeLds = 8 * kEdgeBlock;
+static_assert(kEdgeBatch < 64 && kEdgeBatch <= kEdgeBlock && kEdgeLds % kEdgeBlock == 0, "k_edges: batch / stage layout");
+constexpr uint32_t kCandAccFresh = 1, kCandAccInv = 2;
+
+__global__ __launch_bounds__(kEdgeBlock) void k_edges(const PairDesc* __restrict__ pairs, const Slot* __restrict__ slots,
+                                                      const ListPools lp, uint32_t* __restrict__ seg_of_g,
+                                                      uint8_t* __restrict__ positive, uint32_t* __restrict__ changed,
+                                                      uint32_t* __restrict__ undecided) {
     if (lp.flags[0] | lp.flags[2]) return;
     __shared__ uint32_t s_ij[kEdgeLds];
-    __shared__ float s_sim[kEdgeLds];
+    __shared__ uint8_t s_st[kEdgeLds];
+    __shared__ uint32_t s_lo[kEdgeBatch + 1];
+    __shared__ uint32_t s_beg[kEdgeBatch], s_g[kEdgeBatch];
+    __shared__ uint32_t s_acc0[kEdgeBatch + 1];
+    __shared__ uint32_t s_first0[kEdgeBatch + 1];
+    __shared__ uint32_t red[8], s_res[3];
+    const uint32_t pool = lp.pool0 + blockIdx.y, t = threadIdx.x, lane = lane_id();
     const uint32_t n_hdr = min(lp.cnt[pool * 16 + 4], lp.scap);
-    for (uint32_t k = blockIdx.x; k < n_hdr; k += gridDim.x) {
-        const uint32_t opool = lp.pool0 + (k + 61u * blockIdx.y) % lp.npools;
-        edges_of_segment(pairs, slots, lp, seg_of_g, lp.chdrs[pool * lp.scap + k], opool, (L3D_LDS uint32_t*)s_ij, (L3D_LDS float*)s_sim, lane);
-        __builtin_amdgcn_fence(__ATOMIC_RELEASE, "workgroup");
-        __builtin_amdgcn_wave_barrier();
+    for (uint32_t b = blockIdx.x; b * kEdgeBatch < n_hdr; b += gridDim.x) {
+        const uint32_t k0 = b * kEdgeBatch, nb = min(kEdgeBatch, n_hdr - k0);
+        group_barrier<kEdgeWaves>();
+        uint32_t c = 0;
+        if (t < nb) {
+            const CandHdr ch = lp.chdrs[pool * lp.scap + k0 + t];
+            c = ch.cnt; s_beg[t] = ch.begin; s_g[t] = ch.g;
+        }
+        uint32_t T;
+        const uint32_t ex = group_scan<kEdgeWaves>(c, T, red);
+        if (t <= nb) s_lo[t] = ex;
+        group_barrier<kEdgeWaves>();
+        if (T == 0) continue;
+        const bool one_tile = T <= kEdgeLds;
+        auto stage = [&](uint32_t t0, uint32_t t1) {
+            for (uint32_t x = t0 + t; x < t1; x += kEdgeBlock) {
+                uint32_t lo = 0, hi = nb;
+                while (hi - lo > 1) { const uint32_t mid = (lo + hi) / 2; if (s_lo[mid] <= x) lo = mid; else hi = mid; }
+                const CandRec* r = lp.cands + s_beg[lo] + (x - s_lo[lo]);
+                const uint32_t st = r->sim >= 0.0f ? ((r->tvj & kHypInv) ? kCandAccInv : kCandAccFresh) : 0u;
+                s_ij[x - t0] = r->ij; s_st[x - t0] = (uint8_t)(st | (lo << 2));
+            }
+            group_barrier<kEdgeWaves>();
+        };
+        auto ij_of = [&](uint32_t y, uint32_t s, uint32_t t0) -> uint32_t {
+            return y - t0 < kEdgeLds ? s_ij[y - t0] : lp.cands[s_beg[s] + (y - s_lo[s])].ij;
+        };
+        auto st_of = [&](uint32_t y, uint32_t s, uint32_t t0) -> uint32_t {
+            if (y - t0 < kEdgeLds) return s_st[y - t0] & 3u;
+            const CandRec* r = lp.cands + s_beg[s] + (y - s_lo[s]);
+            return r->sim >= 0.0f ? ((r->tvj & kHypInv) ? kCandAccInv : kCandAccFresh) : 0u;
+        };
+        uint32_t acc_before = 0, first_before = 0;
+        for (uint32_t t0 = 0; t0 < T; t0 += kEdgeLds) {
+            const uint32_t t1 = min(T, t0 + kEdgeLds);
+            if (t0) group_barrier<kEdgeWaves>();
+            stage(t0, t1);
+            for (uint32_t x0 = t0; x0 < t1; x0 += kEdgeBlock) {
+                const uint32_t x = x0 + t;
+                uint32_t s = 0;
+                bool acc = false, first = false;
+                if (x < t1) {
+                    s = s_st[x - t0] >> 2;
+                    acc = (s_st[x - t0] & 3u) != 0;
+                    if (acc) {
+                        const uint32_t i = s_ij[x - t0] >> 16, lo = s_lo[s];
+                        first = true;
+                        for (uint32_t y = x; y-- > lo;) {
+                            if ((ij_of(y, s, t0) >> 16) != i) break;
+                            if (st_of(y, s, t0)) { first = false; break; }
+                        }
+                    }
+                }
+                uint32_t tot;
+                const uint32_t pre = group_scan<kEdgeWaves>((acc ? 1u : 0u) | (first ? 1u << 16 : 0u), tot, red);
+                if (x < t1 && x == s_lo[s])
+                    for (uint32_t s2 = s;; --s2) {
+                        s_acc0[s2] = acc_before + (pre & 0xFFFFu); s_first0[s2] = first_before + (pre >> 16);
+                        if (s2 == 0 || s_lo[s2 - 1] != x) break;
+                    }
+                acc_before += tot & 0xFFFFu; first_before += tot >> 16;
+            }
+        }
+        const uint32_t n_acc = acc_before, n_h = first_before;
+        if (n_acc == 0) continue;
+        group_barrier<kEdgeWaves>();
+        if (t <= nb && s_lo[t] == T) { s_acc0[t] = n_acc; s_first0[t] = n_h; }
+        group_barrier<kEdgeWaves>();
+        const bool seg_has = t < nb && s_acc0[t + 1] > s_acc0[t];
+        uint32_t n_s;
+        const uint32_t seg_at = group_scan<kEdgeWaves>(seg_has ? 1u : 0u, n_s, red);
+        const uint32_t opool = lp.pool0 + (b + 61u * blockIdx.y) % lp.npools;
+        if (t == 0) {
+            s_res[0] = atomicAdd(&lp.cnt[opool * 16 + 0], n_acc);
+            s_res[1] = atomicAdd(&lp.cnt[opool * 16 + 1], n_h);
+            s_res[2] = atomicAdd(&lp.cnt[opool * 16 + 2], n_s);
+        }
+        group_barrier<kEdgeWaves>();
+        const uint32_t eb = s_res[0], hb = s_res[1], sb = s_res[2];
+        if (eb + n_acc > lp.ecap || hb + n_h > lp.hcap || sb + n_s > lp.scap) {
+            if (t == 0) atomicOr(&lp.flags[0], 1u);
+            continue;
+        }
+        const uint32_t e0 = opool * lp.ecap + eb, h0 = opool * lp.hcap + hb;
+        if (seg_has) {
+            const uint32_t si = opool * lp.scap + sb + seg_at;
+            lp.segs[si] = SegHdr{s_g[t], h0 + s_first0[t], s_first0[t + 1] - s_first0[t], 0u};
+            seg_of_g[s_g[t]] = si;
+        }
+        acc_before = 0; first_before = 0;
+        for (uint32_t t0 = 0; t0 < T; t0 += kEdgeLds) {
+            const uint32_t t1 = min(T, t0 + kEdgeLds);
+            if (!one_tile) { group_barrier<kEdgeWaves>(); stage(t0, t1); }
+            for (uint32_t x0 = t0; x0 < t1; x0 += kEdgeBlock) {
+                const uint32_t x = x0 + t;
+                uint32_t s = 0, ij = 0, rank = 0, earlier = 0, mine = 0, kinds = 0;
+                bool acc = false;
+                if (x < t1) {
+                    s = s_st[x - t0] >> 2;
+                    const uint32_t st = s_st[x - t0] & 3u;
+                    acc = st != 0;
+                    if (acc) {
+                        ij = s_ij[x - t0];
+                        const uint32_t i = ij >> 16, lo = s_lo[s], hi = s_lo[s + 1];
+                        mine = 1; kinds = st;
+                        for (uint32_t y = x; y-- > lo;) {
+                            const uint32_t o = ij_of(y, s, t0);
+                            if ((o >> 16) != i) break;
+                            const uint32_t so = st_of(y, s, t0);
+                            if (so) { ++earlier; ++mine; kinds |= so; rank += o < ij ? 1u : 0u; }
+                        }
+                        for (uint32_t y = x + 1; y < hi; ++y) {
+                            const uint32_t o = ij_of(y, s, t0);
+                            if ((o >> 16) != i) break;
+                            const uint32_t so = st_of(y, s, t0);
+                            if (so) { ++mine; kinds |= so; rank += o < ij ? 1u : 0u; }
+                        }
+                    }
+                }
+                const bool first = acc && earlier == 0;
+                uint32_t tot;
+                const uint32_t pre = group_scan<kEdgeWaves>((acc ? 1u : 0u) | (first ? 1u << 16 : 0u), tot, red);
+                bool positive_now = false, later = false;
+                uint32_t hdr_at = 0;
+                if (acc) {
+                    const CandRec r = lp.cands[s_beg[s] + (x - s_lo[s])];
+                    const uint32_t run0 = acc_before + (pre & 0xFFFFu) - earlier;
+                    EdgeRec e;
+                    e.ref_j = r.ref_j; e.sim = r.sim;
+                    e.j_cam = (r.ij & 0xFFFFu) | ((r.tvj & kHypInv) ? kEdgeInv : 0u);
+                    e.tv_j = r.tvj & 0x7FFFFFFFu;
+                    lp.edges[e0 + run0 + rank] = e;
+                    if (first) {
+                        HypHdr hdr;
+                        hdr.g = s_g[s]; hdr.ref = r.ref_i; hdr.pair_flags = r.pf_i; hdr.canon = r.ij >> 16;
+                        hdr.dp1 = r.a1; hdr.dp2 = r.a2;
+                        hdr.edge_begin = e0 + run0; hdr.edge_cnt = mine; hdr.score3D = 0.0f; hdr.state = 0;
+                        const bool hinv = (r.pf_i & kHypInv) != 0;
+                        {
+                            const Slot hs = slots[r.ref_i];
+                            const PairDesc& hp = pairs[r.pf_i & 0x7FFFFFFFu];
+                            hdr.tgt_seg = !hinv ? hs.tgt_seg : lp.slot_row ? lp.slot_row[r.ref_i] : (uint32_t)((r.ref_i - hp.slot_off) / hp.K);
+                            hdr.overlap = hs.overlap;
+                            hdr.oq1 = hinv ? hs.dp1 : hs.dq1; hdr.oq2 = hinv ? hs.dp2 : hs.dq2;
+                        }
+                        hdr.pad[0] = hdr.pad[1] = 0;
+                        hdr_at = h0 + first_before + (pre >> 16);
+                        lp.hyps[hdr_at] = hdr;
+                        if (positive && !hinv) {
+                            positive_now = (kinds & kCandAccFresh) != 0;
+                            later = !positive_now;
+                            if (positive_now) __hip_atomic_store(&positive[r.ref_i], (uint8_t)1, __ATOMIC_RELAXED, __HIP_MEMORY_SCOPE_AGENT);
+                        }
+                    }
+                }
+                if (positive) {
+                    const uint64_t mp = __builtin_amdgcn_ballot_w64(positive_now), ml = __builtin_amdgcn_ballot_w64(later);
+                    if (mp && lane == (uint32_t)__builtin_ctzll(mp)) changed[0] = 1;
+                    if (ml) {
+                        uint32_t base = 0;
+                        if (lane == (uint32_t)__builtin_ctzll(ml)) base = atomicAdd(&lp.cnt[opool * 16 + 7], (uint32_t)__popcll(ml));
+                        base = __shfl(base, __builtin_ctzll(ml));
+                        if (later) undecided[opool * lp.hcap + base + (uint32_t)__popcll(ml & ((1ull << lane) - 1ull))] = hdr_at;
+                    }
+                }
+                acc_before += tot & 0xFFFFu; first_before += tot >> 16;
+            }
+        }
     }
 }
 
@@ -1176,11 +1243,20 @@
     return hipGetLastError();
 }
 
+hipError_t launch_edges(const PairDesc* pairs, const Slot* slots, ListPools lp, uint32_t* seg_of_g, uint8_t* positive,
+                        uint32_t* changed, uint32_t* undecided, hipStream_t st) {
+    hipLaunchKernelGGL(k_edges, dim3((lp.scap + kEdgeBatch - 1) / kEdgeBatch, lp.npools), dim3(kEdgeBlock), 0, st, pairs, slots, lp,
+                       seg_of_g, positive, changed, undecided);
+    return hipGetLastError();
+}
+void edges_constants(uint32_t out[3]) { out[0] = kEdgeBlock; out[1] = kEdgeBatch; out[2] = kEdgeLds; }
+
 constexpr uint32_t kLists2Grid = 16384;
 hipError_t launch_lists(uint32_t v0, uint32_t nv, uint32_t max_M, const ViewDev* views, const PairDesc* pairs,
                         const ListView* lviews, const OutPair* opairs, const InPair* ipairs, const uint32_t* gseg_view,
                         const uint32_t* poff, const uint32_t* inv, const float2* hyp_p, const float2* hyp_q, const Slot* slots, uint32_t uniform_K,
-                        SimConst sc, ListPools lp, uint32_t* seg_of_g, HugeScratchArgs hsa, hipStream_t st) {
+                        SimConst sc, ListPools lp, uint32_t* seg_of_g, HugeScratchArgs hsa, uint8_t* positive, uint32_t* changed,
+                        uint32_t* undecided, hipStream_t st) {
     if (!nv || !max_M) return hipSuccess;
     const bool wide = hsa.mean_list > 96;
 #define L3D_LISTS(B)                                                                                                       \
@@ -1216,8 +1292,8 @@
         hipLaunchKernelGGL(k_lists_huge, dim3(256), dim3(256), 0, st, views, pairs, lviews, opairs, ipairs, gseg_view, poff,
                            inv, hyp_p, hyp_q, lp, hs);
     hipLaunchKernelGGL(k_cand_exact, dim3((lp.ccap + 255) / 256, lp.npools), dim3(256), 0, st, views, pairs, gseg_view, sc, lp);
-    hipLaunchKernelGGL(k_edges, dim3((lp.scap + kEdgesSplit - 1) / kEdgesSplit, lp.npools), dim3(64), 0, st, views, pairs,
-                       gseg_view, slots, lp, seg_of_g);
+    hipError_t ee = launch_edges(pairs, slots, lp, seg_of_g, positive, changed, undecided, st);
+    if (ee != hipSuccess) return ee;
     if (lp.npools < kListPools) hipLaunchKernelGGL(k_publish_flags, dim3(1), dim3(64), 0, st, lp);
     return hipGetLastError();
 }
diff --git a/line3dpp_amd/csrc/k_selftest.hip b/line3dpp_amd/csrc/k_selftest.hip
--- a/line3dpp_amd/csrc/k_selftest.hip
+++ b/line3dpp_amd/csrc/k_selftest.hip
@@ -104,3 +104,74 @@
     for (size_t i = 0; i < kGuard; ++i) *guard_changed += h_ws[words + i] != kPattern;
     return L3D_OK;
 }
+
+extern "C" int l3d_selftest_edges_constants(uint32_t out[3]) {
+    if (!out) return fail(L3D_ERR_ARG, "null argument");
+    l3d::edges_constants(out);
+    return L3D_OK;
+}
+extern "C" int l3d_selftest_edges(int device, uint32_t npools, uint32_t scap, uint32_t ccap, uint32_t ecap, uint32_t hcap,
+                                  const void* cands, const void* chdrs, const uint32_t* n_cands, const uint32_t* n_chdrs,
+                                  const void* slots, uint32_t n_slots, uint32_t slots_per_row, const uint32_t* slot_row,
+                                  uint32_t n_segments, int fold_sweep0, uint32_t* counters, void* edges, void* hyps, void* segs,
+                                  uint32_t* seg_of_g, uint8_t* positive, uint32_t* undecided) {
+    using namespace l3d;
+    if (!cands || !chdrs || !n_cands || !n_chdrs || !slots || !counters || !edges || !hyps || !segs || !seg_of_g || !positive || !undecided)
+        return fail(L3D_ERR_ARG, "null argument");
+    if (!npools || npools > kListPools || !scap || !ccap || !ecap || !hcap || !n_slots || !n_segments || !slots_per_row)
+        return fail(L3D_ERR_ARG, "l3d_selftest_edges: pools, capacities, slots and segments must not be zero (at most kListPools pools)");
+    if ((uint64_t)npools * std::max(std::max(scap, ccap), std::max(ecap, hcap)) >= (1ull << 31))
+        return fail(L3D_ERR_ARG, "l3d_selftest_edges: pools beyond 2^31 records");
+    const CandHdr* hh = (const CandHdr*)chdrs; const CandRec* hc = (const CandRec*)cands;
+    for (uint32_t p = 0; p < npools; ++p) {
+        if (n_chdrs[p] > scap || n_cands[p] > ccap) return fail(L3D_ERR_ARG, "l3d_selftest_edges: more records than the pool holds");
+        for (uint32_t k = 0; k < n_chdrs[p]; ++k) {
+            const CandHdr& h = hh[(size_t)p * scap + k];
+            if (h.g >= n_segments || h.begin < p * ccap || (uint64_t)h.begin + h.cnt > (uint64_t)p * ccap + n_cands[p])
+                return fail(L3D_ERR_ARG, "l3d_selftest_edges: a candidate header points outside its pool");
+            for (uint32_t x = 0; x < h.cnt; ++x) {
+                const CandRec& r = hc[h.begin + x];
+                if (r.ref_i >= n_slots || (r.pf_i & 0x7FFFFFFFu) != 0) return fail(L3D_ERR_ARG, "l3d_selftest_edges: slot or pair out of range");
+            }
+        }
+    }
+    if (int rc = set_device(device)) return rc;
+    constexpr size_t kHead = (size_t)kListPools * 16 + 32 + 64;
+    DevBuf<uint32_t> d_head, d_seg_of_g, d_und, d_slot_row; DevBuf<uint8_t> d_pos;
+    DevBuf<EdgeRec> d_edges; DevBuf<HypHdr> d_hyps; DevBuf<SegHdr> d_segs; DevBuf<CandRec> d_cands; DevBuf<CandHdr> d_chdrs;
+    DevBuf<Slot> d_slots; DevBuf<PairDesc> d_pair;
+    L3D_HIP_CHECK(d_head.reserve(kHead)); L3D_HIP_CHECK(d_seg_of_g.reserve(n_segments)); L3D_HIP_CHECK(d_und.reserve((size_t)npools * hcap));
+    L3D_HIP_CHECK(d_pos.reserve(n_slots)); L3D_HIP_CHECK(d_edges.reserve((size_t)npools * ecap)); L3D_HIP_CHECK(d_hyps.reserve((size_t)npools * hcap));
+    L3D_HIP_CHECK(d_segs.reserve((size_t)npools * scap)); L3D_HIP_CHECK(d_cands.reserve((size_t)npools * ccap));
+    L3D_HIP_CHECK(d_chdrs.reserve((size_t)npools * scap)); L3D_HIP_CHECK(d_slots.reserve(n_slots)); L3D_HIP_CHECK(d_pair.reserve(1));
+    if (slot_row) L3D_HIP_CHECK(d_slot_row.reserve(n_slots));
+    std::vector<uint32_t> head(kHead, 0);
+    for (uint32_t p = 0; p < npools; ++p) { head[p * 16 + 3] = n_cands[p]; head[p * 16 + 4] = n_chdrs[p]; }
+    PairDesc pd{}; pd.K = slots_per_row; pd.slot_off = 0;
+    L3D_HIP_CHECK(hipMemcpy(d_head.p, head.data(), kHead * 4, hipMemcpyHostToDevice));
+    L3D_HIP_CHECK(hipMemcpy(d_cands.p, cands, (size_t)npools * ccap * sizeof(CandRec), hipMemcpyHostToDevice));
+    L3D_HIP_CHECK(hipMemcpy(d_chdrs.p, chdrs, (size_t)npools * scap * sizeof(CandHdr), hipMemcpyHostToDevice));
+    L3D_HIP_CHECK(hipMemcpy(d_slots.p, slots, (size_t)n_slots * sizeof(Slot), hipMemcpyHostToDevice));
+    L3D_HIP_CHECK(hipMemcpy(d_pair.p, &pd, sizeof(pd), hipMemcpyHostToDevice));
+    if (slot_row) L3D_HIP_CHECK(hipMemcpy(d_slot_row.p, slot_row, (size_t)n_slots * 4, hipMemcpyHostToDevice));
+    L3D_HIP_CHECK(hipMemset(d_edges.p, 0xEE, (size_t)npools * ecap * sizeof(EdgeRec))); L3D_HIP_CHECK(hipMemset(d_hyps.p, 0xEE, (size_t)npools * hcap * sizeof(HypHdr)));
+    L3D_HIP_CHECK(hipMemset(d_segs.p, 0xEE, (size_t)npools * scap * sizeof(SegHdr))); L3D_HIP_CHECK(hipMemset(d_seg_of_g.p, 0xEE, (size_t)n_segments * 4));
+    L3D_HIP_CHECK(hipMemset(d_und.p, 0xEE, (size_t)npools * hcap * 4)); L3D_HIP_CHECK(hipMemset(d_pos.p, 0, n_slots));
+    ListPools lp{};
+    lp.cnt = d_head.p; lp.edges = d_edges.p; lp.hyps = d_hyps.p; lp.segs = d_segs.p; lp.cands = d_cands.p; lp.chdrs = d_chdrs.p;
+    lp.ecap = ecap; lp.hcap = hcap; lp.scap = scap; lp.ccap = ccap; lp.flags = d_head.p + kListPools * 16;
+    lp.pool0 = 0; lp.npools = npools; lp.slot_row = slot_row ? d_slot_row.p : nullptr;
+    L3D_HIP_CHECK(launch_edges(d_pair.p, d_slots.p, lp, d_seg_of_g.p, fold_sweep0 ? d_pos.p : nullptr, d_head.p + kListPools * 16 + 32, d_und.p, 0));
+    L3D_HIP_CHECK(hipDeviceSynchronize());
+    L3D_HIP_CHECK(hipMemcpy(head.data(), d_head.p, kHead * 4, hipMemcpyDeviceToHost));
+    for (uint32_t k = 0; k < npools * 16; ++k) counters[k] = head[k];
+    for (uint32_t k = 0; k < 8; ++k) counters[npools * 16 + k] = head[kListPools * 16 + k];
+    counters[npools * 16 + 8] = head[kListPools * 16 + 32];
+    L3D_HIP_CHECK(hipMemcpy(edges, d_edges.p, (size_t)npools * ecap * sizeof(EdgeRec), hipMemcpyDeviceToHost));
+    L3D_HIP_CHECK(hipMemcpy(hyps, d_hyps.p, (size_t)npools * hcap * sizeof(HypHdr), hipMemcpyDeviceToHost));
+    L3D_HIP_CHECK(hipMemcpy(segs, d_segs.p, (size_t)npools * scap * sizeof(SegHdr), hipMemcpyDeviceToHost));
+    L3D_HIP_CHECK(hipMemcpy(seg_of_g, d_seg_of_g.p, (size_t)n_segments * 4, hipMemcpyDeviceToHost));
+    L3D_HIP_CHECK(hipMemcpy(positive, d_pos.p, n_slots, hipMemcpyDeviceToHost));
+    L3D_HIP_CHECK(hipMemcpy(undecided, d_und.p, (size_t)npools * hcap * 4, hipMemcpyDeviceToHost));
+    return L3D_OK;
+}
diff --git a/line3dpp_amd/csrc/l3d_ctx.h b/line3dpp_amd/csrc/l3d_ctx.h
--- a/line3dpp_amd/csrc/l3d_ctx.h
+++ b/line3dpp_amd/csrc/l3d_ctx.h
@@ -232,6 +232,7 @@
     struct PoolCaps { uint32_t e = 0, h = 0, s = 0, c = 0, huge = 0; bool huge_skip = false, list4_skip = false; } caps_saved[2];
     int caps_mode = 0;
     uint32_t chain_need = 8, chain_enqueued = 10;
+    bool sweep0_folded = false;
     uint32_t chain_hist[4] = {6, 6, 6, 6}, chain_hist_at = 0;
     uint32_t shard_world = 0;
     uint32_t shard_rank = 0, shard_v0 = 0, shard_v1 = 0, shard_pool0 = 0, shard_ppr = 0;
diff --git a/line3dpp_amd/csrc/l3d_kernels.h b/line3dpp_amd/csrc/l3d_kernels.h
--- a/line3dpp_amd/csrc/l3d_kernels.h
+++ b/line3dpp_amd/csrc/l3d_kernels.h
@@ -130,7 +130,12 @@
                         const ListView* lviews, const OutPair* opairs, const InPair* ipairs, const uint32_t* gseg_view,
                         const uint32_t* poff, const uint32_t* inv_refs, const float2* hyp_p, const float2* hyp_q,
                         const Slot* slots, uint32_t uniform_K,
-                        SimConst sc, ListPools lp, uint32_t* seg_of_g, HugeScratchArgs hsa, hipStream_t st);
+                        SimConst sc, ListPools lp, uint32_t* seg_of_g, HugeScratchArgs hsa,
+                        uint8_t* positive, uint32_t* changed, uint32_t* undecided,
+                        hipStream_t st);
+hipError_t launch_edges(const PairDesc* pairs, const Slot* slots, ListPools lp, uint32_t* seg_of_g, uint8_t* positive,
+                        uint32_t* changed, uint32_t* undecided, hipStream_t st);
+void edges_constants(uint32_t out[3]);
 hipError_t launch_chain_sweep(ListPools lp, uint8_t* positive, uint32_t* changed, uint32_t sweep, uint32_t* undecided,
                               hipStream_t st);
 hipError_t launch_hyp_scores(ListPools lp, const uint8_t* positive, const uint32_t* gseg_view, Slot* slots,
diff --git a/line3dpp_amd/csrc/l3d_phase_b.hip b/line3dpp_amd/csrc/l3d_phase_b.hip
--- a/line3dpp_amd/csrc/l3d_phase_b.hip
+++ b/line3dpp_amd/csrc/l3d_phase_b.hip
@@ -5,7 +5,7 @@
 static int match_finish_impl(l3d_ctx* c);
 static int lists_prepare(l3d_ctx* c, int caps_mode);
 static int lists_reserve(l3d_ctx* c);
-static int lists_run(l3d_ctx* c, uint32_t v0, uint32_t nv, uint32_t pool0, uint32_t npools);
+static int lists_run(l3d_ctx* c, uint32_t v0, uint32_t nv, uint32_t pool0, uint32_t npools, bool fold_sweep0);
 
 static int lists_shard_impl(l3d_ctx* c, uint32_t rank, uint32_t world, int64_t view0, int64_t view1, void* slab_ptr[4],
                             uint64_t slab_bytes[4], void* full_ptr[4]) {
@@ -49,7 +49,7 @@
         r2 = lists_reserve(c);
         if (r2) return r2;
         const uint32_t ppr = kListPools / world, pool0 = rank * ppr;
-        r2 = lists_run(c, v0, v1 - v0, pool0, ppr);
+        r2 = lists_run(c, v0, v1 - v0, pool0, ppr, false);
         if (r2) return r2;
         c->shard_rank = rank; c->shard_v0 = v0; c->shard_v1 = v1; c->shard_pool0 = pool0; c->shard_ppr = ppr;
         c->tail_counted = false; c->tail_written = false;
@@ -278,7 +278,7 @@
     return L3D_OK;
 }
 
-static int lists_run(l3d_ctx* c, uint32_t v0, uint32_t nv, uint32_t pool0, uint32_t npools) {
+static int lists_run(l3d_ctx* c, uint32_t v0, uint32_t nv, uint32_t pool0, uint32_t npools, bool fold_sweep0) {
     g_trace.mark("lists_run enter");
     hipStream_t st = c->stream;
     const uint32_t V = (uint32_t)c->order.size(), P = (uint32_t)c->pairs.size(), G = c->G;
@@ -312,7 +312,8 @@
     for (uint32_t vi = v0; vi < v0 + nv; ++vi) max_M = std::max(max_M, c->order[vi]->M);
     L3D_HIP_CHECK(launch_lists(v0, nv, max_M, c->d_views.p, c->d_pairs.p, lviews, opairs, ipairs, c->d_gseg_view.p,
                                c->d_poff.p, c->d_inv_refs.p, c->d_hyp_p.p, c->d_hyp_q.p, c->d_slots.p, c->kNN > 0 ? (uint32_t)c->kNN : 0u, simc, lp,
-                               c->d_seg_of_g.p, hsa, st));
+                               c->d_seg_of_g.p, hsa, fold_sweep0 ? positive_of(c) : nullptr, c->d_lzero.p + z.changed, c->d_surv_tg.p, st));
+    c->sweep0_folded = fold_sweep0;
     if (c->ev_on(9)) L3D_HIP_CHECK(hipEventRecord(c->ev[9], st));
     g_trace.mark("list pass enqueued");
     return L3D_OK;
@@ -338,7 +339,8 @@
     const uint32_t n_sweeps = std::min(kChainSweeps, std::max(4u, need + 3));
     c->chain_enqueued = n_sweeps;
     if (!fresh) L3D_HIP_CHECK(hipMemset2DAsync(c->d_lzero.p + 7, 64, 0, 4, kListPools, st));
-    for (uint32_t s2 = 0; s2 < n_sweeps; ++s2)
+    const uint32_t s_first = fresh && c->sweep0_folded ? 1u : 0u;
+    for (uint32_t s2 = s_first; s2 < n_sweeps; ++s2)
         L3D_HIP_CHECK(launch_chain_sweep(lp, positive_of(c), changed, s2, c->d_surv_tg.p, st));
     g_trace.mark("chain sweeps enqueued");
     const uint8_t* present = nullptr;
@@ -514,7 +516,7 @@
     for (;;) {
         rc = lists_reserve(c);
         if (rc) return rc;
-        rc = lists_run(c, 0, V, 0, kListPools);
+        rc = lists_run(c, 0, V, 0, kListPools, true);
         if (rc) return rc;
         rc = tail_until_converged(c);
         if (rc == kRetry) continue;
```
